# YuanchenBei/ColdRec

Hardware: AMD Instinct MI355X
Metric: ranked items/sec (full-catalogue eval) (higher is better)
Workload: dtype f32; 1 GPU; configs[3] full-catalogue eval: 1000000-row user table x 10000000 items, d=128, k=20, f32 tables, user block 131072 per step, rated CSR (mean ~50) + 20% cold-item bitmap ('warm' setting), item table row-sharded over 1 GPU(s); items=10000000, dim=128, k=20, parallelism=single GPU

## Files before the change

coldrec_amd/_lib.py:

```python
from __future__ import annotations

import ctypes
import os
import subprocess

_HERE = os.path.dirname(os.path.abspath(__file__))
LIB_PATH = os.environ.get("CRH_LIB") or os.path.join(_HERE, "lib", "libcoldrec_hip.so")
CSRC = os.path.join(_HERE, "csrc")

PAD_IDX = 0x7FFFFFFF
MASKED_SCORE = -1.0e9
MAX_K = 128

_lib = None

_vp, _i32, _i64, _sz, _f32 = ctypes.c_void_p, ctypes.c_int, ctypes.c_int64, ctypes.c_size_t, ctypes.c_float
_f64 = ctypes.c_double

SIGNATURES = {
    "crh_last_error": (ctypes.c_char_p, []),
    "crh_version": (_i32, []),
    "crh_score_topk_supports_dim": (_i32, [_i32]),
    "crh_score_topk_workspace_bytes": (_sz, [_i64, _i64, _i32, _i32]),
    "crh_score_topk_min_workspace_bytes": (_sz, [_i64, _i32]),
    "crh_score_topk_route": (_i32, [_i32, _i64, _i64, _i32, _i32, _sz, _i32, _i32, _vp, _vp]),
    "crh_score_topk_route_kernel": (ctypes.c_char_p, [_i32]),
    "crh_score_topk_screened": (_i32, [_i32, _i64, _i64, _i32, _i32, _sz, _i32, _i32]),
    "crh_score_topk_uncertified": (_i64, [_vp, _vp]),
    "crh_score_topk_screen_plan": (_i32, [_i64, _i64, _sz, _i32, _vp, _vp]),
    "crh_score_topk_screen_ordered": (_i32, [_i64, _i64, _sz, _i32]),
    "crh_score_topk_screen_map": (_i32, [_vp, _vp, _i64, _i64, _i64, _i32, _vp, _vp, _vp, _vp]),
    "crh_score_topk_f32": (_i32, [_vp, _vp, _i64, _vp, _i64, _i32, _vp, _vp, _vp, _i32, _i64, _vp, _vp,
                                  _vp, _sz, _vp]),
    "crh_score_topk_f32_ex": (_i32, [_vp, _vp, _i64, _vp, _i64, _i32, _vp, _vp, _vp, _i32, _i64, _vp, _vp,
                                     _vp, _sz, _vp, _i32, _vp, _vp]),
    "crh_score_screen_items_bytes": (_sz, [_i64, _i32]),
    "crh_score_screen_items_prepare": (_i32, [_vp, _i64, _i32, _vp, _i64, _i64, _vp, _sz, _vp, _sz, _vp, _vp]),
    "crh_score_screen_items_destroy": (_i32, [_vp]),
    "crh_score_topk_screen_item_preps": (_i64, []),
    "crh_score_topk_f32_prepared": (_i32, [_vp, _vp, _i64, _vp, _i64, _i32, _vp, _vp, _vp, _i32, _i64, _vp, _vp,
                                           _vp, _sz, _vp, _i32, _vp, _vp, _vp]),
    "crh_score_topk_f16_supports_dim": (_i32, [_i32]),
    "crh_score_topk_f16_workspace_bytes": (_sz, [_i64, _i64, _i32, _i32]),
    "crh_score_topk_f16_ex": (_i32, [_vp, _vp, _i64, _vp, _i64, _i32, _vp, _vp, _vp, _i32, _i64, _vp, _vp,
                                     _vp, _sz, _vp, _i32, _vp, _vp]),
    "crh_mask_topk_f32": (_i32, [_vp, _i64, _i64, _i64, _vp, _vp, _vp, _i32, _i64, _i32, _vp, _vp, _vp]),
    "crh_merge_topk": (_i32, [_vp, _vp, _i32, _i64, _i32, _i32, _vp, _vp, _vp]),
    "crh_bpr_workspace_bytes": (_sz, [_i64]),
    "crh_bpr_plan_ints": (_i64, [_i64]),
    "crh_bpr_heavy_threshold": (_i32, []),
    "crh_bpr_plan_build_host": (_i32, [_vp, _vp, _vp, _i64, _i64, _vp]),
    "crh_bpr_plan_build": (_i32, [_vp, _vp, _vp, _i64, _i64, _vp, _vp]),
    "crh_bpr_plan_build_large_workspace_bytes": (_sz, [_i64, _i64]),
    "crh_bpr_plan_build_large": (_i32, [_vp, _vp, _vp, _i64, _i64, _vp, _vp, _sz, _vp]),
    "crh_bpr_fwd_bwd_f32": (_i32, [_vp, _vp, _vp, _i32, _vp, _vp, _vp, _i64, _f32, _vp, _vp, _vp, _vp, _vp, _vp,
                                   _sz, _vp]),
    "crh_bpr_fwd_f32": (_i32, [_vp, _vp, _vp, _i32, _vp, _vp, _vp, _i64, _vp, _vp, _sz, _vp]),
    "crh_bpr_bwd_f32": (_i32, [_vp, _vp, _vp, _i32, _vp, _vp, _vp, _i64, _i64, _f32, _vp, _vp, _vp, _vp, _vp, _vp,
                               _vp, _sz, _vp]),
    "crh_bpr_bwd_owned_f32": (_i32, [_vp, _vp, _i32, _vp, _vp, _vp, _i64, _f32, _vp, _vp, _vp, _vp, _vp, _i32, _i32, _vp, _sz, _vp]),
    "crh_rows_pack_cap": (_i64, [_i64, _i32]),
    "crh_rows_pack_f32": (_i32, [_vp, _vp, _i64, _i64, _i32, _i32, _i32, _vp, _vp, _vp]),
    "crh_rows_unpack_f32": (_i32, [_vp, _vp, _vp, _i64, _i32, _vp]),
    "crh_adam_dense_f32": (_i32, [_vp, _vp, _vp, _vp, _i64, _vp, _vp, _vp, _vp, _i64, _f64, _f64, _f64, _f64,
                                  _i64, _i32, _vp, _vp]),
    "crh_adam_rows_f32": (_i32, [_vp, _vp, _vp, _vp, _vp, _i64, _i32, _vp, _i64, _i64, _i64, _vp, _f64, _f64, _f64,
                                 _i32, _vp]),
    "crh_adam_step_scalars_host": (None, [_f64, _f64, _f64, _i64, _vp]),
    "crh_adam_step_scalars_range_host": (None, [_f64, _f64, _f64, _i64, _i64, _vp]),
    "crh_spmm_segment_edges": (_i32, []),
    "crh_spmm_lane_group": (_i32, [_i64, _i32, _i64]),
    "crh_spmm_workspace_bytes": (_sz, [_vp, _i32]),
    "crh_spmm_csr_adam_f32": (_i32, [_vp, _vp, _vp, _i64, _vp, _i32, _vp, _f32, _vp, _f32, _vp, _vp, _vp, _vp,
                                     _f64, _f64, _f64, _f64, _i64, _vp, _i32, _vp]),
    "crh_spmm_csr_f32": (_i32, [_vp, _vp, _vp, _i64, _vp, _i32, _vp, _vp, _f32, _vp, _f32, _vp, _vp, _sz, _vp]),
    "crh_bpr_fwd_parts": (_i32, [_i64, _i32]),
    "crh_mf_step_parts": (_i32, [_i64, _i32]),
    "crh_mf_step_tables": (_i32, [_vp, _vp, _vp, _vp, _i64, _i64, _i64, _i64, _vp, _vp, _vp, _vp]),
    "crh_mf_step_f32": (_i32, [_vp, _vp, _vp, _vp, _i64, _i64, _i32, _i64, _f32, _vp, _vp, _vp, _vp,
                               _vp, _i32, _vp, _vp, _i64, _vp, _f64, _f64, _f64, _vp, _vp]),
    "crh_mf_step_finish": (_i32, [_vp, _i32, _i64, _vp, _vp]),
    "crh_mf_step_sgd_f32": (_i32, [_vp, _vp, _i64, _i64, _i32, _i64, _f32, _vp, _vp, _vp, _vp, _vp, _i32, _vp, _vp,
                                   _i64, _vp, _f64, _vp]),
    "crh_sgd_dense_f32": (_i32, [_vp, _vp, _i64, _f64, _i32, _vp]),
    "crh_sgd_rows_f32": (_i32, [_vp, _vp, _i32, _vp, _i64, _i64, _f64, _vp]),
    "crh_spmm_csr_sgd_f32": (_i32, [_vp, _vp, _vp, _i64, _vp, _i32, _vp, _f32, _vp, _f32, _vp, _vp, _f64, _i32, _vp]),
    "crh_l2_workspace_bytes": (_sz, []),
    "crh_l2_norm_f32": (_i32, [_vp, _i64, _vp, _vp, _sz, _vp]),
    "crh_l2_reg_bwd_f32": (_i32, [_vp, _i64, _i64, _f32, _vp, _vp, _vp, _i32, _vp]),
    "crh_infonce_workspace_bytes": (_sz, [_i64, _i32]),
    "crh_infonce_splits": (_i32, [_i64]),
    "crh_infonce_f32": (_i32, [_vp, _vp, _vp, _vp, _vp, _i64, _i32, _f32, _i32, _f32, _i32, _vp, _vp, _vp, _vp, _sz, _vp]),
    "crh_table_nce_workspace_bytes": (_sz, [_i64, _i64, _i32]),
    "crh_table_nce_splits": (_i32, [_i64, _i64, _i32]),
    "crh_table_nce_f32": (_i32, [_vp, _vp, _i64, _vp, _vp, _i64, _i32, _f32, _f32, _i32, _vp, _vp, _vp, _vp, _sz, _vp]),
    "crh_clcrec_max_neg": (_i32, []),
    "crh_clcrec_chunk_rows": (_i32, []),
    "crh_clcrec_workspace_bytes": (_sz, [_i64, _i32, _i32, _i64]),
    "crh_clcrec_f32": (_i32, [_vp] * 12 + [_i64] + [_vp] * 3 + [_i64, _i64, _i32, _i32, _i64, _f32, _f32, _f32, _f32,
                              _vp, _vp, _vp, _vp, _vp, _sz, _vp]),
    "crh_ccfcrec_max_rows": (_i32, []),
    "crh_ccfcrec_chunk_rows": (_i32, []),
    "crh_ccfcrec_workspace_bytes": (_sz, [_i64, _i32, _i32, _i32, _i32, _i64, _i64]),
    "crh_ccfcrec_f32": (_i32, [_vp, _i64, _vp, _i64] + [_vp] * 4 + [_i32] * 4 + [_vp] * 5 + [_i64, _i64] + [_vp] * 5 +
                               [_i64, _i64, _i64, _i32, _i32, _i32, _i32, _f32, _f32, _f32, _vp, _vp, _vp, _vp, _vp, _sz,
                                _vp]),
    "crh_aldi_workspace_bytes": (_sz, [_i64, _i32]),
    "crh_aldi_f32": (_i32, [_vp, _i64, _vp, _i64, _vp, _vp, _vp] + [_i32] * 4 + [_vp] * 4 + [_i64, _i32] + [_f32] * 4 +
                            [_vp] * 5 + [_sz, _vp]),
    "crh_gar_chunk_rows": (_i32, []),
    "crh_gar_workspace_bytes": (_sz, [_i64, _i32, _i64, _i64]),
    "crh_gar_f32": (_i32, [_vp, _i64, _vp, _i64] + [_vp] * 4 + [_i32] * 4 + [_vp] * 5 + [_i64, _i64] + [_vp] * 5 +
                           [_i64, _i64, _i64, _i32, _i32] + [_f32] * 4 + [_vp] * 5 + [_sz, _vp]),
    "crh_mtpr_chunk_rows": (_i32, []),
# ... 91 lines not shown
```

coldrec_amd/csrc/score_screen.hip:

```cpp
#include <math.h>

#include "score_topk_common.h"

#include <hipcub/device/device_radix_sort.hpp>

namespace crh_score {
namespace {

constexpr int SD = 128;
constexpr int FB_SCRATCH_SLICES = 64;

__device__ __forceinline__ float up_float(double x) {
    if (!(x <= 3.0e38)) return __builtin_inff();
    float f = (float)x;
    if ((double)f < x) f = __uint_as_float(__float_as_uint(f) + 1u);
    return f;
}

__device__ __forceinline__ int scale_exp(const unsigned* stats, int word) {
    const float m = __uint_as_float(stats[word]);
    if (!(m > 0.0f) || !(m <= 3.4e38f)) return 0;
    int E;
    frexpf(m, &E);
    return 15 - E;
// ... 73 lines not shown
    const double B = (double)un * R + (double)udn * Nh + gd * (double)un * N + gp * (double)uhn * Nh + 0x1p-126;
    return B * (1.0 + 0x1p-20);
}

__device__ __forceinline__ float up_norm(double s) { return up_float(sqrt(s) * (1.0 + 0x1p-30)); }

constexpr int LIVE_WPB = 256;

__device__ __forceinline__ unsigned live_word(const uint32_t* __restrict__ bitmap, int64_t w, int64_t g0, int64_t g1) {
    const int64_t w0 = g0 >> 5, n_words = ((g1 - 1) >> 5) - w0 + 1;
    if (w >= n_words) return 0u;
    unsigned m = ~bitmap[w0 + w];
    const int64_t lo = (w0 + w) << 5;
    if (lo < g0) m &= ~0u << (int)(g0 - lo);
    if (lo + 32 > g1) m &= ~0u >> (int)(lo + 32 - g1);
    return m;
}

__device__ __forceinline__ unsigned block_excl_sum(unsigned v, unsigned* total) {
    __shared__ unsigned wsum[4];
    const int lane = threadIdx.x & 63, wv = threadIdx.x >> 6;
    unsigned inc = v;
#pragma unroll
    for (int o = 1; o < 64; o <<= 1) {
        const unsigned t = __shfl_up(inc, o);
        if (lane >= o) inc += t;
    }
    if (lane == 63) wsum[wv] = inc;
    __syncthreads();
    unsigned before = 0;
    for (int q = 0; q < wv; ++q) before += wsum[q];
    *total = wsum[0] + wsum[1] + wsum[2] + wsum[3];
    return before + inc - v;
}

__global__ __launch_bounds__(256) void screen_live_count_kernel(const uint32_t* __restrict__ bitmap, int64_t g0, int64_t g1,
                                                                unsigned* __restrict__ blocksum) {
    const unsigned c = __popc(live_word(bitmap, (int64_t)blockIdx.x * LIVE_WPB + threadIdx.x, g0, g1));
    unsigned total;
    block_excl_sum(c, &total);
    if (threadIdx.x == 0) blocksum[blockIdx.x] = total;
}

__global__ __launch_bounds__(256) void screen_live_scan_kernel(unsigned* __restrict__ blocksum, int64_t n_blocks,
                                                               unsigned* __restrict__ n_live) {
    const int64_t per = (n_blocks + 255) / 256;
    const int64_t lo = threadIdx.x * per < n_blocks ? threadIdx.x * per : n_blocks, hi = lo + per < n_blocks ? lo + per : n_blocks;
    unsigned sum = 0;
    for (int64_t q = lo; q < hi; ++q) sum += blocksum[q];
    unsigned total;
    unsigned run = block_excl_sum(sum, &total);
    for (int64_t q = lo; q < hi; ++q) {
        const unsigned c = blocksum[q];
        blocksum[q] = run;
        run += c;
    }
    if (threadIdx.x == 0) *n_live = total;
}

__global__ __launch_bounds__(256) void screen_idmap_kernel(const uint32_t* __restrict__ bitmap, int64_t g0, int64_t g1,
                                                           const unsigned* __restrict__ blocksum, int32_t* __restrict__ idmap) {
    const int64_t w = (int64_t)blockIdx.x * LIVE_WPB + threadIdx.x;
    unsigned m = live_word(bitmap, w, g0, g1);
    unsigned total;
    int64_t pos = (int64_t)blocksum[blockIdx.x] + block_excl_sum(__popc(m), &total);
    const int id0 = (int)(((g0 >> 5) + w) << 5);
    while (m) {
        idmap[pos++] = id0 + __builtin_ctz(m);
        m &= m - 1;
    }
}

__global__ __launch_bounds__(256) void screen_sortkey_kernel(const int32_t* __restrict__ idmap, const uint16_t* __restrict__ rowkeys,
                                                             const unsigned* __restrict__ n_live, int64_t item_base, int64_t n_slots,
                                                             uint16_t* __restrict__ skeys) {
    const int64_t q = (int64_t)blockIdx.x * 256 + threadIdx.x;
    if (q >= n_slots) return;
    skeys[q] = q < (int64_t)*n_live ? (uint16_t)~rowkeys[(int64_t)idmap[q] - item_base] : (uint16_t)0xFFFFu;
}

__global__ __launch_bounds__(256) void screen_mapkeys_kernel(const uint16_t* __restrict__ skeys, int64_t n, int32_t* __restrict__ out) {
    const int64_t q = (int64_t)blockIdx.x * 256 + threadIdx.x;
    if (q < n) out[q] = (int32_t)(uint16_t)~skeys[q];
}

__global__ __launch_bounds__(256) void screen_items_kernel(const float* __restrict__ v, int64_t n_items, const uint32_t* __restrict__ bitmap,
                                                           int64_t item_base, _Float16* __restrict__ packed, unsigned* __restrict__ stats,
                                                           int64_t prefix, const int32_t* __restrict__ idmap) {
    const int e = scale_exp(stats, 0);
    const int64_t TP = prefix >> 5, n_live = idmap ? (int64_t)stats[SCREEN_STAT_LIVE] : 0;
    const int64_t T = idmap ? TP + ((n_live + 31) >> 5) : (n_items + 31) >> 5;
    float mr = 0.0f, mn = 0.0f, mh = 0.0f;
    u32x4* dst = reinterpret_cast<u32x4*>(packed);
    for (int64_t t = blockIdx.x; t < T; t += gridDim.x) {
        for (int p = 0; p < 2; ++p) {
            const int u = threadIdx.x + 256 * p, r = u >> 4, c = u & 15;
            int64_t row = (t << 5) + r;
            bool masked;
            if (idmap != nullptr && t >= TP) {
                const int64_t q = row - prefix;
                masked = q >= n_live;
                row = (int64_t)idmap[masked ? n_live - 1 : q] - item_base;
            } else {
                if (row >= n_items) row = n_items - 1;
                masked = bitmap != nullptr && ((bitmap[(item_base + row) >> 5] >> ((item_base + row) & 31)) & 1u);
            }
            const float* src = v + row * SD + 8 * c;
            const f32x4 x0 = *reinterpret_cast<const f32x4*>(src), x1 = *reinterpret_cast<const f32x4*>(src + 4);
            _Float16 hv[8];
            double sxx, sdd, shh;
            row_sums(x0, x1, hv, e, sxx, sdd, shh);
            u32x4 o = u32x4{0u, 0u, 0u, 0u};
            if (!masked) {
                o = __builtin_bit_cast(u32x4, f16x8{hv[0], hv[1], hv[2], hv[3], hv[4], hv[5], hv[6], hv[7]});
                mr = fmaxf(mr, up_norm(sdd));
                mn = fmaxf(mn, up_norm(sxx));
                mh = fmaxf(mh, up_norm(shh));
                if (sdd != sdd || sxx != sxx) mr = __builtin_inff();
            }
            dst[(t * 8 + (c >> 1)) * 64 + (c & 1) * 32 + r] = o;
        }
    }
    __shared__ float red[3][4];
    mr = wave_max(mr);
    mn = wave_max(mn);
    mh = wave_max(mh);
    if ((threadIdx.x & 63) == 0) {
        red[0][threadIdx.x >> 6] = mr;
        red[1][threadIdx.x >> 6] = mn;
        red[2][threadIdx.x >> 6] = mh;
    }
    __syncthreads();
    if (threadIdx.x < 3) {
        const float b = fmaxf(fmaxf(red[threadIdx.x][0], red[threadIdx.x][1]), fmaxf(red[threadIdx.x][2], red[threadIdx.x][3]));
        if (b > 0.0f) atomicMax(stats + 2 + threadIdx.x, __float_as_uint(b));
    }
}

__global__ __launch_bounds__(256) void screen_users_kernel(const float* __restrict__ uemb, const int32_t* __restrict__ users,
                                                           int64_t n_users, _Float16* __restrict__ uh, float* __restrict__ ustat,
                                                           unsigned* __restrict__ stats) {
    const int e = scale_exp(stats, 1);
    const float R = __uint_as_float(stats[2]), N = __uint_as_float(stats[3]), Nh = __uint_as_float(stats[4]);
    float mb = 0.0f;
    const int64_t n_units = n_users * 16;
    for (int64_t w = (int64_t)blockIdx.x * 256 + threadIdx.x; w < ((n_units + 255) & ~(int64_t)255); w += (int64_t)gridDim.x * 256) {
        const int64_t j = (w < n_units ? w : n_units - 1) >> 4;
        const int c = (int)(w & 15);
        const int64_t row = users ? (int64_t)users[j] : j;
        const float* src = uemb + row * SD + 8 * c;
        const f32x4 x0 = *reinterpret_cast<const f32x4*>(src), x1 = *reinterpret_cast<const f32x4*>(src + 4);
        _Float16 hv[8];
        double sxx, sdd, shh;
        row_sums(x0, x1, hv, e, sxx, sdd, shh);
        if (w < n_units) {
            reinterpret_cast<u32x4*>(uh)[j * 16 + c] = __builtin_bit_cast(u32x4, f16x8{hv[0], hv[1], hv[2], hv[3], hv[4], hv[5], hv[6], hv[7]});
            if (c == 0) {
                const bool bad = sxx != sxx || sdd != sdd;
                const float un = bad ? __builtin_inff() : up_norm(sxx), uhn = bad ? __builtin_inff() : up_norm(shh);
                const float udn = bad ? __builtin_inff() : up_norm(sdd);
                ustat[3 * j + 0] = un;
                ustat[3 * j + 1] = uhn;
                ustat[3 * j + 2] = udn;
                mb = fmaxf(mb, up_float(screen_bound(un, uhn, udn, R, N, Nh)));
            }
        }
// ... 181 lines not shown
    __shared__ int cnth[4];
    const int lane = threadIdx.x & 63, wv = threadIdx.x >> 6;
    const int K = s.k;
    const int64_t count = s.stats[5];
    const int S = fb_slices(s, count);
    const int last = S <= FB_FANIN ? 0 : 1;
    if (level > last) return;
    const int stride = level == 0 ? 1 : FB_FANIN;
    const int span = stride * FB_FANIN;
    const int G = (S + span - 1) / span;
    float* ls = lsh[wv];
    int* li = lih[wv];
    int* cnt = &cnth[wv];
    for (int64_t w = (int64_t)blockIdx.x * 4 + wv; w < count * G; w += (int64_t)gridDim.x * 4) {
        const int64_t f = w / G;
        const int z0 = (int)(w % G) * span;
        if (lane == 0) *cnt = 0;
        for (int z = z0; z < z0 + span && z < S; z += stride) {
            const int64_t o = (f * S + z) * K;
            const float es = lane < K ? s.part_score[o + lane] : CRH_NEG_INF;
            const int ei = lane < K ? s.part_idx[o + lane] : CRH_PAD_IDX;
            unsigned long long m = __ballot(lane < K && ei != CRH_PAD_IDX);
            while (m) {
                const int L = __builtin_ctzll(m);
                m &= m - 1;
                const float sc = __shfl(es, L);
                const int g = __shfl(ei, L);
                const int n = __builtin_amdgcn_readfirstlane(*cnt);
                if (n >= K && !crh_better(sc, g, ls[K - 1], li[K - 1])) break;
                wave_list_insert(ls, li, cnt, K, sc, g, lane);
            }
        }
        const int n = __builtin_amdgcn_readfirstlane(*cnt);
        if (level == last) {
            const int64_t slot = s.fail_list[f];
            wave_list_store(ls, li, n, K, s.out_score + slot * K, s.out_idx + slot * K, lane);
        } else {
            const int64_t o = (f * S + z0) * K;
            wave_list_store(ls, li, n, K, s.part_score + o, s.part_idx + o, lane);
        }
    }
}

}

int screen_fallback_slices(int64_t n_items) {
    const int64_t s = n_items / 4096;
    return (int)(s < 1 ? 1 : (s > FB_SCRATCH_SLICES ? FB_SCRATCH_SLICES : s));
}

size_t screen_scan_bytes(int64_t n_main) { return (size_t)((n_main + 31) / 32 / LIVE_WPB + 2) * sizeof(unsigned); }

int64_t screen_map_slots(int64_t n_main) { return ((n_main + 31) / 32 + 1) * 32; }

size_t screen_sort_bytes(int64_t n_slots) { return (size_t)n_slots * 8 + ((size_t)1 << 20); }

int launch_screen_map(const uint32_t* bitmap, int64_t item_base, int64_t n_items, int64_t prefix, unsigned* n_live, unsigned* scan,
                      int32_t* idmap, const ScreenOrder* ord, hipStream_t st) {
    const int64_t g0 = item_base + prefix, g1 = item_base + n_items;
    const int64_t n_words = ((g1 - 1) >> 5) - (g0 >> 5) + 1, nb = (n_words + LIVE_WPB - 1) / LIVE_WPB;
    hipLaunchKernelGGL(screen_live_count_kernel, dim3((unsigned)nb), dim3(256), 0, st, bitmap, g0, g1, scan);
    CRH_HIP(hipGetLastError());
    hipLaunchKernelGGL(screen_live_scan_kernel, dim3(1), dim3(256), 0, st, scan, nb, n_live);
    CRH_HIP(hipGetLastError());
    hipLaunchKernelGGL(screen_idmap_kernel, dim3((unsigned)nb), dim3(256), 0, st, bitmap, g0, g1, scan, idmap);
    CRH_HIP(hipGetLastError());
    if (ord == nullptr) return CRH_OK;
    const int64_t n_slots = screen_map_slots(n_items - prefix);
    hipLaunchKernelGGL(screen_sortkey_kernel, dim3((unsigned)((n_slots + 255) / 256)), dim3(256), 0, st, idmap, ord->rowkeys, n_live,
                       item_base, n_slots, ord->skeys_in);
    CRH_HIP(hipGetLastError());
    size_t need = 0;
    CRH_HIP(hipcub::DeviceRadixSort::SortPairs(nullptr, need, ord->skeys_in, ord->skeys_out, idmap, ord->idmap, (int)n_slots, 0, 16, st));
    if (need > ord->sort_tmp_bytes) {
        crh_set_error("screened route: the ordered map's sort asks for %zu bytes of temporary storage, %zu are reserved", need,
                      ord->sort_tmp_bytes);
        return CRH_ERR_WS;
    }
    need = ord->sort_tmp_bytes;
    CRH_HIP(hipcub::DeviceRadixSort::SortPairs(ord->sort_tmp, need, ord->skeys_in, ord->skeys_out, idmap, ord->idmap, (int)n_slots, 0, 16, st));
    return CRH_OK;
}

int launch_screen_prep_items(const ScreenArgs& s, unsigned* stats, _Float16* packed, int64_t prefix, int32_t* idmap, unsigned* scan,
                             const ScreenOrder* ord, hipStream_t st) {
    const int64_t T = (s.n_items + 31) / 32;
    if (ord != nullptr)
        hipLaunchKernelGGL(screen_maxabs_kernel<true>, dim3(2048), dim3(256), 0, st, s.item_emb, nullptr, s.n_items, stats, 0, ord->rowkeys);
    else
        hipLaunchKernelGGL(screen_maxabs_kernel<false>, dim3(2048), dim3(256), 0, st, s.item_emb, nullptr, s.n_items, stats, 0, nullptr);
    CRH_HIP(hipGetLastError());
    if (idmap != nullptr) {
        const int rc = launch_screen_map(s.bitmap, s.item_base, s.n_items, prefix, stats + SCREEN_STAT_LIVE, scan, idmap, ord, st);
        if (rc != CRH_OK) return rc;
        if (ord != nullptr) idmap = ord->idmap;
    }
    hipLaunchKernelGGL(screen_items_kernel, dim3((unsigned)(T < 4096 ? T : 4096)), dim3(256), 0, st, s.item_emb, s.n_items, s.bitmap,
                       s.item_base, packed, stats, prefix, idmap);
    CRH_HIP(hipGetLastError());
    return CRH_OK;
}

int launch_screen_prep_users(const ScreenArgs& s, _Float16* uh, int margin_on, hipStream_t st) {
    hipLaunchKernelGGL(screen_maxabs_kernel<false>, dim3(256), dim3(256), 0, st, s.user_emb, s.users, s.n_users, s.stats, 1, nullptr);
    CRH_HIP(hipGetLastError());
    const int64_t ub = (s.n_users * 16 + 255) / 256;
    hipLaunchKernelGGL(screen_users_kernel, dim3((unsigned)(ub < 2048 ? ub : 2048)), dim3(256), 0, st, s.user_emb, s.users, s.n_users,
                       uh, s.ustat, s.stats);
    CRH_HIP(hipGetLastError());
    hipLaunchKernelGGL(screen_margin_kernel, dim3(1), dim3(1), 0, st, s.stats, margin_on);
    CRH_HIP(hipGetLastError());
    return CRH_OK;
}

int screen_map_only(const uint32_t* bitmap, const float* item_emb, int64_t n_items, int64_t item_base, int64_t prefix, int ordered,
                    int32_t* map_out, int32_t* keys_out, int64_t* count, hipStream_t st) {
    auto al = [](size_t x) { return (x + 255) & ~(size_t)255; };
    const int64_t n_main = n_items - prefix, n_slots = screen_map_slots(n_main);
    const size_t o_scan = 256, o_map = o_scan + al(screen_scan_bytes(n_main)), o_rk = o_map + al((size_t)n_slots * 4),
                 o_k0 = o_rk + al((size_t)n_items * 2), o_k1 = o_k0 + al((size_t)n_slots * 2), o_m1 = o_k1 + al((size_t)n_slots * 2),
                 o_tmp = o_m1 + al((size_t)n_slots * 4), total = o_tmp + screen_sort_bytes(n_slots);
    char* buf = nullptr;
    CRH_HIP(hipMalloc(reinterpret_cast<void**>(&buf), total));
    ScreenOrder ord;
    ord.rowkeys = reinterpret_cast<uint16_t*>(buf + o_rk);
    ord.skeys_in = reinterpret_cast<uint16_t*>(buf + o_k0);
    ord.skeys_out = reinterpret_cast<uint16_t*>(buf + o_k1);
    ord.idmap = reinterpret_cast<int32_t*>(buf + o_m1);
    ord.sort_tmp = buf + o_tmp;
    ord.sort_tmp_bytes = screen_sort_bytes(n_slots);
    unsigned* stats = reinterpret_cast<unsigned*>(buf);
    int32_t* idmap = reinterpret_cast<int32_t*>(buf + o_map);
    int rc = CRH_OK;
    unsigned live = 0;
    hipError_t e = hipMemsetAsync(buf, 0, 256, st);
    if (e == hipSuccess) {
        hipLaunchKernelGGL(screen_maxabs_kernel<true>, dim3(2048), dim3(256), 0, st, item_emb, nullptr, n_items, stats, 0, ord.rowkeys);
        e = hipGetLastError();
    }
    if (e == hipSuccess) rc = launch_screen_map(bitmap, item_base, n_items, prefix, stats + SCREEN_STAT_LIVE, reinterpret_cast<unsigned*>(buf + o_scan), idmap, &ord, st);
    if (e == hipSuccess && rc == CRH_OK) {
        hipLaunchKernelGGL(screen_mapkeys_kernel, dim3((unsigned)((n_main + 255) / 256)), dim3(256), 0, st,
                           ordered ? ord.skeys_out : ord.skeys_in, n_main, keys_out);
        e = hipGetLastError();
    }
    if (e == hipSuccess && rc == CRH_OK)
        e = hipMemcpyAsync(map_out, ordered ? ord.idmap : idmap, (size_t)n_main * 4, hipMemcpyDeviceToDevice, st);
    if (e == hipSuccess && rc == CRH_OK) e = hipMemcpyAsync(&live, stats + SCREEN_STAT_LIVE, 4, hipMemcpyDeviceToHost, st);
    if (e == hipSuccess) e = hipStreamSynchronize(st);
    (void)hipFree(buf);
    CRH_HIP(e);
    if (rc == CRH_OK) *count = (int64_t)live;
    return rc;
}

int launch_screen_certify(const ScreenArgs& s, hipStream_t st) {
    hipLaunchKernelGGL(screen_certify_kernel, dim3((unsigned)((s.n_users + 3) / 4)), dim3(256), 0, st, s);
    CRH_HIP(hipGetLastError());
    hipLaunchKernelGGL(screen_fallback_kernel, dim3((unsigned)(FB_WAVES / 4)), dim3(256), 0, st, s);
    CRH_HIP(hipGetLastError());
    for (int level = 0; level < 2; ++level) {
        hipLaunchKernelGGL(screen_fallback_merge_kernel, dim3(512), dim3(256), 0, st, s, level);
        CRH_HIP(hipGetLastError());
    }
    return CRH_OK;
}

}
```

coldrec_amd/csrc/score_topk.hip:

```cpp
#include <math.h>
#include <stdarg.h>
#include <stdlib.h>

#include <algorithm>
#include <atomic>
#include <vector>

#include "score_topk_common.h"

using namespace crh_score;

namespace {

__device__ __forceinline__ bool pack_row_masked(const uint32_t* bitmap, int64_t gid) {
    return bitmap != nullptr && ((bitmap[gid >> 5] >> (gid & 31)) & 1u);
}

template <int D>
__global__ __launch_bounds__(256) void pack_items_kernel(const float* __restrict__ v, int64_t n_items,
                                                         float* __restrict__ packed, const uint32_t* __restrict__ bitmap,
                                                         int64_t item_base) {
    constexpr int NCH = D / 8;
    __shared__ float tile[32][D + 4];
    const int64_t t = blockIdx.x;
// ... 674 lines not shown
    const int dma_mode = getenv("CRH_SCORE_DMA") ? atoi(getenv("CRH_SCORE_DMA")) : 1;
    const size_t tb_off = lists_bytes(n_users, k) + packed_bytes(n_items, d, esz) + sync_bytes(n_items);
    const bool dma_rows = esz == 2 ? d == 256 : (d == 128 || d == 64);
    const int dma_form = dma_mode == 2 || dma_mode == 3 ? dma_mode : (esz == 4 && d == 128 && n_items < FP32_DMA_FLAG_MAX_ITEMS ? 2 : 3);
    const bool dma_shape = dma_mode && dma_rows && score_dma_ring_slots(esz, d, k, dma_form) > 0 &&
                           (!has_bitmap || workspace_bytes >= tb_off + tbits_bytes(n_items));
    const bool wg_shape = esz == 2 ? (d == 64 || d == 128 || d == 256) : ((d == 128 && wg_waves == 8) || (d == 64 && dma_shape));
    const int64_t n_wg64 = ((n_users + 63) / 64 + wg_waves - 1) / wg_waves;
    const int64_t fp32_min_items = !dma_shape ? FP32_WG_MIN_ITEMS : (d == 64 ? FP32_DMA_MIN_ITEMS_D64 : FP32_DMA_MIN_ITEMS_D128);
    const bool fp32_wg_ok = n_items >= fp32_min_items && (double)n_wg64 / (double)(((n_wg64 + 255) / 256) * 256) >= 0.9;
    const bool use_wg = wg_mode && can_pack && wg_shape && (dma_shape || wg_waves == 8 || 2 * wg4_lds <= 160 * 1024) &&
                        (n_users + 63) / 64 >= 512 && (esz == 2 || fp32_wg_ok || wg_mode == 2);
    const bool use_dma = use_wg && dma_shape;
    const int wg_waves_l = use_dma ? 4 : wg_waves;
    const int wg_slots_l = use_dma ? 256 : wg_slots;
    const int upw = use_dma ? 128 : (use_wg ? wg_upw : users_per_wave(esz, d));
    static const int variant = CRH_TUNE_ENV("CRH_SCORE_OCC") ? atoi(CRH_TUNE_ENV("CRH_SCORE_OCC")) : 2;
    const int occ = esz == 2 ? 2 : ((variant == 2 && d == 128) ? 2 : 1);
    static const int dense_mode = CRH_TUNE_ENV("CRH_SCORE_DENSE") ? atoi(CRH_TUNE_ENV("CRH_SCORE_DENSE")) : 1;
    const size_t dense_b = dense_block_bytes(n_users, n_items);
    r.dense = dense_mode && n_splits == 0 && !seeded && dense_b && has_workspace && workspace_bytes >= dense_b;
    r.use_wg = use_wg;
    r.use_dma = use_dma;
    r.dma_mode = dma_form;
    r.can_pack = can_pack;
    r.wg_waves_l = wg_waves_l;
    r.wg_slots_l = wg_slots_l;
    r.upw = upw;
    r.occ = occ;
    r.dense_b = dense_b;
    r.tb_off = tb_off;
    r.no_pack = no_pack;
    return r;
}

int plan_splits(const RoutePlan& r, int esz, int64_t n_users, int64_t n_items, int k, int n_splits, bool seeded) {
    const int64_t T = (n_items + 31) / 32;
    const int64_t n_ug = (n_users + r.upw - 1) / r.upw;
    int s = n_splits > 0 ? n_splits
            : seeded     ? pick_splits_seeded(r.use_wg ? (n_ug + r.wg_waves_l - 1) / r.wg_waves_l : n_ug, n_items,
                                              r.use_wg ? (double)r.wg_slots_l : 1024.0 * r.occ)
            : r.use_wg   ? pick_splits_wg((n_ug + r.wg_waves_l - 1) / r.wg_waves_l, n_items, k, r.wg_slots_l,
                                          esz == 2 ? 18750.0 : 5700.0)
                         : pick_splits(n_ug, n_items, r.occ);
    if (s > T) s = (int)T;
    return s;
}

int score_topk_impl(int esz, const void* user_emb, const int32_t* users, int64_t n_users, const void* item_emb,
                    int64_t n_items, int d, const int64_t* rated_rowptr, const int32_t* rated_col,
                    const uint32_t* cand_bitmap, int k, int64_t item_base, float* out_score, int32_t* out_idx,
                    void* workspace, size_t workspace_bytes, void* stream, int n_splits, void* ev_kernel_start,
                    void* ev_kernel_stop, const char* who, const float* seed_score, const int32_t* seed_idx);

int64_t seed_route(int esz, int64_t n_users, int64_t n_items, int d) {
    const char* sm = getenv("CRH_SCORE_SEED");
    const int seed_mode = sm ? atoi(sm) : 1;
    int64_t P = seed_prefix_items(n_items, n_users);
    if (!seed_mode || P <= 0 || n_users <= 0) return 0;
    const int upw = users_per_wave(esz, d);
    const int64_t n_ug = (n_users + upw - 1) / upw;
    const int occ_pw = esz == 2 || d == 128 ? 2 : 1;
    const bool cuts = pick_splits(n_ug, n_items, occ_pw) > 1;
    const char* smi = getenv("CRH_SCORE_SEED_MAX_ITEMS");
    const int64_t f32_stream_min = d == 64 ? FP32_DMA_MIN_ITEMS_D64 : FP32_WG_MIN_ITEMS;
    const bool small_cat = !cuts && esz == 4 && n_items <= (smi ? atoll(smi) : f32_stream_min - 1);
    const bool f16_stream = !cuts && esz == 2 && d == 256 && n_users >= 32768 && n_items >= ((int64_t)1 << 20);
    const bool f32_stream = !cuts && esz == 4 && (d == 128 || d == 64) && n_users >= 32768 && n_items >= f32_stream_min;
    if ((small_cat || f16_stream) && !CRH_TUNE_ENV("CRH_SCORE_SEED_ITEMS") && P > 4096) P = 4096;
    if (f32_stream && !small_cat && !CRH_TUNE_ENV("CRH_SCORE_SEED_ITEMS") && P > 8192) P = 8192;
    if (!(cuts || small_cat || f16_stream || f32_stream || seed_mode == 2) || dense_block_bytes(n_users, P) == 0) return 0;
    return P;
}

constexpr int64_t SCREEN_SEED_ITEMS = 8192;
int64_t screen_prefix(int64_t n_items) { return n_items >= 8 * SCREEN_SEED_ITEMS ? SCREEN_SEED_ITEMS : 0; }
int screen_splits(int64_t n_users, int64_t n_main, bool seeded) {
    const int64_t n_wg = ((n_users + 127) / 128 + 3) / 4, T = (n_main + 31) / 32;
    int s = seeded ? pick_splits_seeded(n_wg, n_main, 256.0) : pick_splits_wg(n_wg, n_main, SCREEN_KP, 256, 18750.0);
    if (s > T) s = (int)T;
    return s;
}
struct ScreenLayout {
    size_t stats, ustat, fail, uh, seed, cand, packed, tbits, sync, idmap, scan, rowkeys, skeys, idmap2, sorttmp, scratch, need;
};
ScreenLayout screen_layout(int64_t n_users, int64_t n_items, int64_t P, bool compact = false, bool ordered = false) {
    auto al = [](size_t x) { return (x + 255) & ~(size_t)255; };
    ScreenLayout L;
    L.stats = 0;
    L.ustat = 256;
    L.fail = L.ustat + al((size_t)n_users * 3 * sizeof(float));
    L.uh = L.fail + al((size_t)n_users * sizeof(int32_t));
    L.seed = L.uh + al((size_t)n_users * 128 * 2);
    L.cand = L.seed + al((size_t)n_users * SCREEN_KP * 8);
    L.packed = L.cand + al((size_t)n_users * SCREEN_KP * 8);
    L.tbits = L.packed + packed_bytes(n_items, 128, 2);
    L.sync = L.tbits + tbits_bytes(n_items);
    L.idmap = L.sync + sync_bytes(n_items);
    const size_t slots = (size_t)screen_map_slots(n_items - P);
    L.scan = L.idmap + (compact ? al(slots * sizeof(int32_t)) : 0);
    L.rowkeys = L.scan + (compact ? al(screen_scan_bytes(n_items - P)) : 0);
    ordered = ordered && compact;
    L.skeys = L.rowkeys + (ordered ? al((size_t)n_items * sizeof(uint16_t)) : 0);
    L.idmap2 = L.skeys + (ordered ? 2 * al(slots * sizeof(uint16_t)) : 0);
    L.sorttmp = L.idmap2 + (ordered ? al(slots * sizeof(int32_t)) : 0);
    L.scratch = L.sorttmp + (ordered ? al(screen_sort_bytes((int64_t)slots)) : 0);
    const int S = screen_splits(n_users, n_items - P, P > 0);
    const size_t lists = S > 1 ? (size_t)S * n_users * SCREEN_KP * 8 : 0;
    const size_t dense = P > 0 ? (size_t)64 * (size_t)P * sizeof(float) : 0;
    const size_t part = (size_t)n_users * screen_fallback_slices(n_items) * 20 * 8;
    L.need = L.scratch + std::max(lists, std::max(dense, part));
    return L;
}

int screen_mode() {
    const char* e = getenv("CRH_SCORE_SCREEN");
    return e ? atoi(e) : 1;
}
bool screen_compact(int64_t n_users, int64_t n_items, size_t workspace_bytes, bool has_bitmap) {
    const char* e = getenv("CRH_SCORE_SCREEN_COMPACT");
    if (!has_bitmap || (e && atoi(e) == 0)) return false;
    return workspace_bytes >= screen_layout(n_users, n_items, screen_prefix(n_items), true).need;
}
bool screen_ordered(int64_t n_users, int64_t n_items, size_t workspace_bytes, bool has_bitmap) {
    const char* e = getenv("CRH_SCORE_SCREEN_ORDER");
    if ((e && atoi(e) == 0) || !screen_compact(n_users, n_items, workspace_bytes, has_bitmap)) return false;
    const int64_t P = screen_prefix(n_items);
    if (screen_splits(n_users, n_items - P, P > 0) != 1) return false;
    return workspace_bytes >= screen_layout(n_users, n_items, P, true, true).need;
}
bool screen_route(int esz, int64_t n_users, int64_t n_items, int d, int k, size_t workspace_bytes, bool has_bitmap, int n_splits) {
    const int mode = screen_mode();
    if (mode <= 0 || mode > 3 || esz != 4 || d != 128 || k < 1 || k > 20 || n_splits != 0 || n_users <= 0 || n_items <= 0 ||
        workspace_bytes == 0)
        return false;
    if (workspace_bytes < screen_layout(n_users, n_items, screen_prefix(n_items)).need) return false;
    if (mode >= 2) return true;
    if (n_items < FP32_DMA_FLAG_MAX_ITEMS) return false;
    int64_t P = seed_route(esz, n_users, n_items, d);
    size_t ws = workspace_bytes;
    if (P > 0) {
        const size_t sb = seed_bytes(n_users, k);
        const size_t stage1 = dense_block_bytes(n_users, P) + packed_bytes(P, d, esz);
        const size_t stage2 = lists_bytes(n_users, k) + packed_bytes(n_items - P, d, esz);
        if (workspace_bytes >= sb + std::max(stage1, stage2)) ws = workspace_bytes - sb;
        else P = 0;
    }
    const RoutePlan r = plan_route(esz, n_users, n_items - P, d, k, true, ws, has_bitmap, 0, P > 0);
    return !r.dense && r.use_dma && r.dma_mode == 3;
}

constexpr uint32_t SCREEN_ITEMS_MAGIC = 0x43524849u;
struct ScreenItems {
    uint32_t magic;
    const float* item_emb;
    int64_t n_items, item_base, prefix;
    int d;
    const uint32_t* bitmap;
    bool compact, ordered;
    hipStream_t stream;
    char* buf;
};
struct ScreenItemsLayout {
    size_t stats, packed, tbits, map, need;
};
ScreenItemsLayout screen_items_layout(int64_t n_items, bool has_bitmap) {
    ScreenItemsLayout L;
    L.stats = 0;
    L.packed = 256;
    L.tbits = L.packed + packed_bytes(n_items, 128, 2);
    L.map = L.tbits + (has_bitmap ? tbits_bytes(n_items) : 0);
    const size_t slots = (size_t)screen_map_slots(n_items);
    L.need = L.map + (has_bitmap ? (slots * sizeof(int32_t) + 255) & ~(size_t)255 : 0);
    return L;
}
bool screen_items_match(const ScreenItems* p, const float* item_emb, int64_t n_items, int64_t item_base, const uint32_t* bitmap,
                        int64_t prefix, bool compact, bool ordered, hipStream_t st) {
    if (p == nullptr || p->magic != SCREEN_ITEMS_MAGIC) return false;
    const char* e = getenv("CRH_SCORE_SCREEN_PREPARED");
    if (e && atoi(e) == 0) return false;
    return p->item_emb == item_emb && p->n_items == n_items && p->d == 128 && p->item_base == item_base && p->bitmap == bitmap &&
           p->prefix == prefix && p->compact == compact && p->ordered == ordered && p->stream == st;
}
std::atomic<int64_t> screen_item_preps{0};

int score_topk_screened(const float* user_emb, const int32_t* users, int64_t n_users, const float* item_emb, int64_t n_items,
                        const int64_t* rated_rowptr, const int32_t* rated_col, const uint32_t* cand_bitmap, int k, int64_t item_base,
                        float* out_score, int32_t* out_idx, void* workspace, size_t workspace_bytes, void* stream,
                        void* ev_kernel_start, void* ev_kernel_stop, const char* who, const ScreenItems* prepared);

int score_topk_any(int esz, const void* user_emb, const int32_t* users, int64_t n_users, const void* item_emb,
                   int64_t n_items, int d, const int64_t* rated_rowptr, const int32_t* rated_col,
                   const uint32_t* cand_bitmap, int k, int64_t item_base, float* out_score, int32_t* out_idx,
                   void* workspace, size_t workspace_bytes, void* stream, int n_splits, void* ev_kernel_start,
                   void* ev_kernel_stop, const char* who, const ScreenItems* prepared = nullptr) {
    if (user_emb && item_emb && out_score && out_idx && workspace &&
        screen_route(esz, n_users, n_items, d, k, workspace_bytes, cand_bitmap != nullptr, n_splits))
        return score_topk_screened(reinterpret_cast<const float*>(user_emb), users, n_users, reinterpret_cast<const float*>(item_emb),
                                   n_items, rated_rowptr, rated_col, cand_bitmap, k, item_base, out_score, out_idx, workspace,
                                   workspace_bytes, stream, ev_kernel_start, ev_kernel_stop, who, prepared);
    const int64_t P = n_splits == 0 ? seed_route(esz, n_users, n_items, d) : 0;
    if (P > 0 && user_emb && item_emb && out_score && out_idx && n_users > 0 && k >= 1 && k <= CRH_MAX_K && workspace) {
        const size_t sb = seed_bytes(n_users, k);
        const size_t stage1 = dense_block_bytes(n_users, P) + packed_bytes(P, d, esz);
        const size_t stage2 = lists_bytes(n_users, k) + packed_bytes(n_items - P, d, esz);
        if (workspace_bytes >= sb + std::max(stage1, stage2)) {
            float* seed_s = reinterpret_cast<float*>(workspace);
            int32_t* seed_i = reinterpret_cast<int32_t*>(seed_s + (size_t)n_users * k);
            void* ws2 = reinterpret_cast<char*>(workspace) + sb;
            hipStream_t st = reinterpret_cast<hipStream_t>(stream);
            if (ev_kernel_start) CRH_HIP(hipEventRecord(reinterpret_cast<hipEvent_t>(ev_kernel_start), st));
            int rc = score_topk_impl(esz, user_emb, users, n_users, item_emb, P, d, rated_rowptr, rated_col, cand_bitmap, k,
                                     item_base, seed_s, seed_i, ws2, workspace_bytes - sb, stream, 0, nullptr, nullptr, who,
                                     nullptr, nullptr);
            if (rc != CRH_OK) return rc;
            rc = score_topk_impl(esz, user_emb, users, n_users,
                                 reinterpret_cast<const char*>(item_emb) + (size_t)P * d * esz, n_items - P, d, rated_rowptr,
                                 rated_col, cand_bitmap, k, item_base + P, out_score, out_idx, ws2, workspace_bytes - sb, stream,
                                 0, nullptr, nullptr, who, seed_s, seed_i);
            if (rc != CRH_OK) return rc;
            if (ev_kernel_stop) CRH_HIP(hipEventRecord(reinterpret_cast<hipEvent_t>(ev_kernel_stop), st));
            return CRH_OK;
        }
    }
    return score_topk_impl(esz, user_emb, users, n_users, item_emb, n_items, d, rated_rowptr, rated_col, cand_bitmap, k,
                           item_base, out_score, out_idx, workspace, workspace_bytes, stream, n_splits, ev_kernel_start,
                           ev_kernel_stop, who, nullptr, nullptr);
}

#ifdef CRH_PROFILE
int print_wave_timing(unsigned long long* dev, int64_t n_waves, int timing, hipStream_t st) {
        CRH_HIP(hipStreamSynchronize(st));
        std::vector<unsigned long long> h((size_t)n_waves * 6);
        CRH_HIP(hipMemcpy(h.data(), dev, h.size() * 8, hipMemcpyDeviceToHost));
        CRH_HIP(hipFree(dev));
        if (timing == 2)
            if (FILE* f = fopen("/tmp/crh_wave_clock.bin", "wb")) { fwrite(h.data(), 8, h.size(), f); fclose(f); }
        unsigned long long t0 = ~0ull, t1 = 0;
        for (int64_t wv = 0; wv < n_waves; ++wv) { t0 = std::min(t0, h[2 * wv]); t1 = std::max(t1, h[2 * wv + 1]); }
        std::vector<double> st_(n_waves), en_(n_waves);
        for (int64_t wv = 0; wv < n_waves; ++wv) { st_[wv] = (double)(h[2 * wv] - t0); en_[wv] = (double)(h[2 * wv + 1] - t0); }
        std::sort(st_.begin(), st_.end());
        std::sort(en_.begin(), en_.end());
        const double tot = (double)(t1 - t0);
        fprintf(stderr, "[crh timing] waves=%lld span=%.0f ticks; start quantiles 0/25/50/75/100%%: %.3f %.3f %.3f %.3f %.3f; "
                        "end quantiles 0/10/25/50/75/90/100%%: %.3f %.3f %.3f %.3f %.3f %.3f %.3f (fraction of span)\n",
                (long long)n_waves, tot, st_[0] / tot, st_[n_waves / 4] / tot, st_[n_waves / 2] / tot,
                st_[3 * n_waves / 4] / tot, st_[n_waves - 1] / tot, en_[0] / tot, en_[n_waves / 10] / tot,
                en_[n_waves / 4] / tot, en_[n_waves / 2] / tot, en_[3 * n_waves / 4] / tot, en_[9 * n_waves / 10] / tot,
                en_[n_waves - 1] / tot);
        std::vector<double> in_(n_waves), lp_(n_waves), so_(n_waves);
        double ev_ticks = 0, ev = 0, lp_sum = 0;
        for (int64_t wv = 0; wv < n_waves; ++wv) {
            in_[wv] = (double)(h[2 * n_waves + 2 * wv] - h[2 * wv]);
            lp_[wv] = (double)(h[2 * n_waves + 2 * wv + 1] - h[2 * n_waves + 2 * wv]);
            so_[wv] = (double)(h[2 * wv + 1] - h[2 * n_waves + 2 * wv + 1]);
            ev_ticks += (double)h[4 * n_waves + 2 * wv];
            ev += (double)h[4 * n_waves + 2 * wv + 1];
            lp_sum += lp_[wv];
        }
        std::sort(in_.begin(), in_.end());
        std::sort(lp_.begin(), lp_.end());
        std::sort(so_.begin(), so_.end());
        fprintf(stderr, "[crh timing] median ticks: list setup %.0f, tile loop %.0f, list store %.0f; %.0f slow-path events per wave, "
                        "%.0f ticks each = %.3f of the loop\n",
                in_[n_waves / 2], lp_[n_waves / 2], so_[n_waves / 2], ev / (double)n_waves, ev > 0 ? ev_ticks / ev : 0.0,
                lp_sum > 0 ? ev_ticks / lp_sum : 0.0);
    return CRH_OK;
}
int dma_timing_begin(ScoreArgs& a, hipStream_t st) {
    CRH_HIP(hipMalloc(&a.wave_clock, (size_t)16 * 4 * 66 * 8));
    CRH_HIP(hipMemsetAsync(a.wave_clock, 0, (size_t)16 * 4 * 66 * 8, st));
    return CRH_OK;
}
int dma_timing_report(ScoreArgs& a, int esz, int d, hipStream_t st) {
    CRH_HIP(hipStreamSynchronize(st));
    std::vector<unsigned long long> h((size_t)16 * 4 * 66);
    CRH_HIP(hipMemcpy(h.data(), a.wave_clock, h.size() * 8, hipMemcpyDeviceToHost));
    CRH_HIP(hipFree(a.wave_clock));
    {
        unsigned long long tk = 0, ne = 0;
        for (int q = 0; q < 64; ++q) { tk += h[(size_t)16 * 4 * 64 + 2 * q]; ne += h[(size_t)16 * 4 * 64 + 2 * q + 1]; }
        fprintf(stderr, "[crh dma timing] events: %.0f per wave, %.0f cycles each (tiles with at least one candidate; 64 waves)\n",
                (double)ne / 64.0, ne ? (double)tk / (double)ne : 0.0);
    }
    for (int wv = 0; wv < 4; ++wv) {
        unsigned long long tot = 0, wsum = 0;
        std::vector<unsigned long long> b(64, 0);
        for (int blk = 0; blk < 16; ++blk)
            for (int q = 0; q < 64; ++q) b[q] += h[((size_t)blk * 4 + wv) * 64 + q];
        const unsigned long long bw = (esz == 4 ? 512 : 128) >> (d * esz == 256 ? 1 : 0);
        for (int q = 0; q < 64; ++q) { tot += b[q]; wsum += b[q] * (q * bw + bw / 2); }
        fprintf(stderr, "[crh dma timing] wave %d: %llu tiles, mean %.0f cycles; histogram (%llu-cycle buckets from 0):", wv, tot,
                tot ? (double)wsum / (double)tot : 0.0, bw);
        for (int q = 0; q < 64; ++q) fprintf(stderr, " %llu", b[q]);
        fprintf(stderr, "\n");
    }
    a.wave_clock = nullptr;
    return CRH_OK;
}
#endif

int score_topk_impl(int esz, const void* user_emb, const int32_t* users, int64_t n_users, const void* item_emb,
                    int64_t n_items, int d, const int64_t* rated_rowptr, const int32_t* rated_col,
                    const uint32_t* cand_bitmap, int k, int64_t item_base, float* out_score, int32_t* out_idx,
                    void* workspace, size_t workspace_bytes, void* stream, int n_splits, void* ev_kernel_start,
                    void* ev_kernel_stop, const char* who, const float* seed_score, const int32_t* seed_idx) {
    CRH_CHECK_ARG(user_emb && item_emb && out_score && out_idx, "%s: NULL table/output pointer", who);
    CRH_CHECK_ARG(n_users > 0 && n_items > 0, "%s: empty block (n_users=%lld, n_items=%lld)", who,
                  (long long)n_users, (long long)n_items);
    CRH_CHECK_ARG(k >= 1 && k <= CRH_MAX_K, "%s: k=%d outside 1..%d", who, k, CRH_MAX_K);
    CRH_CHECK_ARG(esz == 4 ? crh_score_topk_supports_dim(d) : crh_score_topk_f16_supports_dim(d),
                  "%s: d=%d unsupported (pad the tables to %s16/32/64/128/256)", who, d, esz == 4 ? "8/" : "");
    CRH_CHECK_ARG(((uintptr_t)user_emb & 15) == 0 && ((uintptr_t)item_emb & 15) == 0,
                  "%s: tables must be 16-byte aligned", who);
    CRH_CHECK_ARG((rated_rowptr == nullptr) == (rated_col == nullptr) || rated_rowptr != nullptr,
                  "%s: rated_col given without rated_rowptr", who);
    CRH_CHECK_ARG(item_base >= 0 && item_base + n_items < (int64_t)CRH_PAD_IDX, "%s: item ids exceed int32", who);
    CRH_CHECK_ARG(n_splits >= 0 && n_splits <= 64, "%s: n_splits=%d outside 0..64", who, n_splits);

    const RoutePlan rp = plan_route(esz, n_users, n_items, d, k, workspace != nullptr, workspace_bytes, cand_bitmap != nullptr,
                                    n_splits, seed_score != nullptr);
    const bool use_wg = rp.use_wg, use_dma = rp.use_dma, can_pack = rp.can_pack;
    const int wg_waves_l = rp.wg_waves_l, upw = rp.upw, occ = rp.occ, no_pack = rp.no_pack;
    const size_t tb_off = rp.tb_off, dense_b = rp.dense_b;
    ScoreArgs a;
    a.user_emb = user_emb;
    a.users = users;
    a.n_users = n_users;
    a.item_emb = item_emb;
    a.n_items = n_items;
    a.rated_rowptr = rated_rowptr;
    a.rated_col = rated_col;
    a.bitmap = cand_bitmap;
    a.k = k;
    a.item_base = item_base;
    a.n_ugroups = (n_users + upw - 1) / upw;
    static const int ablate = CRH_PROFILE_ENV("CRH_SCORE_ABLATE");
    a.ablate = ablate;
    a.dense = nullptr;
    a.dense_stride = 0;
    a.user_base = 0;
    a.seed_score = seed_score;
    a.seed_idx = seed_idx;
    a.margin = nullptr;
    a.screen_k = 0;
    const int64_t T = (n_items + 31) / 32;
    hipStream_t st = reinterpret_cast<hipStream_t>(stream);

    if (rp.dense) {
        const int64_t stride = T * 32;
        const int upw_pw = users_per_wave(esz, d);
        int64_t chunk = (int64_t)(dense_b / ((size_t)stride * sizeof(float)));
        if (chunk > n_users) chunk = n_users;
        a.packed = nullptr;
        if (!no_pack && workspace_bytes >= dense_b + packed_bytes(n_items, d, esz)) {
            void* pk = reinterpret_cast<char*>(workspace) + dense_b;
            const int prc = pack_items(esz, item_emb, n_items, d, pk, st, cand_bitmap, item_base);
            if (prc != CRH_OK) return prc;
            a.packed = pk;
        }
        a.n_splits = 1;
        a.xcd_sync = nullptr;
        a.sync_window = 0;
        a.sync_stride = 0;
        a.wave_clock = nullptr;
#ifdef CRH_PROFILE
        static const int timing_d = CRH_PROFILE_ENV("CRH_SCORE_TIMING");
#endif
        a.out_score = out_score;
        a.out_idx = out_idx;
        a.dense = reinterpret_cast<float*>(workspace);
        CRH_CHECK_ARG(stride < ((int64_t)1 << 25), "%s: dense block rows of %lld scores exceed the kernel's 32-bit lane offsets", who, (long long)stride);
        a.dense_stride = stride;
        if (ev_kernel_start) CRH_HIP(hipEventRecord(reinterpret_cast<hipEvent_t>(ev_kernel_start), st));
        for (int64_t u0 = 0; u0 < n_users; u0 += chunk) {
            const int64_t cu = std::min(chunk, n_users - u0);
            a.users = users ? users + u0 : nullptr;
            a.user_base = u0;
            a.n_users = cu;
            a.n_ugroups = (cu + upw_pw - 1) / upw_pw;
            a.n_splits = (int)std::max<int64_t>(1, std::min<int64_t>(T, (1024 * occ) / a.n_ugroups));
            a.rated_rowptr = rated_rowptr ? rated_rowptr + u0 : nullptr;
#ifdef CRH_PROFILE
            if (timing_d) {
                CRH_HIP(hipMalloc(&a.wave_clock, (size_t)a.n_ugroups * a.n_splits * 48));
                CRH_HIP(hipMemsetAsync(a.wave_clock, 0, (size_t)a.n_ugroups * a.n_splits * 48, st));
            }
#endif
            const int rc1 = launch_score_per_wave(esz, d, occ, a, st);
            if (rc1 != CRH_OK) return rc1;
#ifdef CRH_PROFILE
            if (timing_d) {
                const int trc = print_wave_timing(a.wave_clock, a.n_ugroups * a.n_splits, timing_d, st);
                if (trc != CRH_OK) return trc;
            }
#endif
            const int rc2 = crh_mask_topk_f32(a.dense, cu, n_items, stride, a.rated_rowptr, rated_col, cand_bitmap, k,
                                              item_base, 0, out_score + u0 * k, out_idx + u0 * k, stream);
            if (rc2 != CRH_OK) return rc2;
        }
        if (ev_kernel_stop) CRH_HIP(hipEventRecord(reinterpret_cast<hipEvent_t>(ev_kernel_stop), st));
        return CRH_OK;
    }

    a.n_splits = plan_splits(rp, esz, n_users, n_items, k, n_splits, seed_score != nullptr);

    if (a.n_splits == 1) {
        a.out_score = out_score;
        a.out_idx = out_idx;
    } else {
        const size_t need = (size_t)a.n_splits * n_users * k * 8;
        if (!workspace || workspace_bytes < need) {
            crh_set_error("%s: workspace %zu < %zu bytes", who, workspace_bytes, need);
            return CRH_ERR_WS;
        }
        a.out_score = reinterpret_cast<float*>(workspace);
        a.out_idx = reinterpret_cast<int32_t*>(a.out_score + (size_t)a.n_splits * n_users * k);
    }
    a.packed = nullptr;
    if (can_pack) {
        void* pk = reinterpret_cast<char*>(workspace) + lists_bytes(n_users, k);
        const int prc = pack_items(esz, item_emb, n_items, d, pk, st, cand_bitmap, item_base);
        if (prc != CRH_OK) return prc;
        a.packed = pk;
    }
    int rc;
    static const int sync_win_raw = CRH_TUNE_ENV("CRH_SCORE_SYNC_WINDOW") ? atoi(CRH_TUNE_ENV("CRH_SCORE_SYNC_WINDOW")) : 128;
    static const int sync_win = sync_win_raw <= 0 ? 0 : std::max(2, sync_win_raw & ~1);
// ... 8 lines not shown
        const int64_t n_win = (T / a.n_splits + 1 + sync_win - 1) / sync_win + 1;
        const size_t need = lists_bytes(n_users, k) + packed_bytes(n_items, d, esz) + sync_bytes(n_items);
        if (workspace_bytes >= need && (size_t)(n_win + 1) * 8 * sizeof(unsigned) <= sync_bytes(n_items)) {
            a.sync_stride = n_win + 1;
            a.xcd_sync = reinterpret_cast<unsigned*>(reinterpret_cast<char*>(workspace) + lists_bytes(n_users, k) +
                                                     packed_bytes(n_items, d, esz));
            CRH_HIP(hipMemsetAsync(a.xcd_sync, 0, (size_t)a.sync_stride * 8 * sizeof(unsigned), st));
        }
    }
    a.tile_bits = reinterpret_cast<const uint32_t*>(a.packed);
    a.idmap = nullptr;
    a.n_live = nullptr;
    if (use_dma && cand_bitmap) {
        uint32_t* tb = reinterpret_cast<uint32_t*>(reinterpret_cast<char*>(workspace) + tb_off);
        hipLaunchKernelGGL(tile_bits_kernel, dim3((unsigned)((T + 255) / 256)), dim3(256), 0, st, cand_bitmap, item_base, n_items, T, tb);
        CRH_HIP(hipGetLastError());
        a.tile_bits = tb;
    }
    a.wave_clock = nullptr;
#ifdef CRH_PROFILE
    static const int timing = CRH_PROFILE_ENV("CRH_SCORE_TIMING");
    const int64_t n_waves = a.n_ugroups * a.n_splits;
    if (timing && !use_wg) CRH_HIP(hipMalloc(&a.wave_clock, (size_t)n_waves * 48));
    if (timing && use_dma) {
        rc = dma_timing_begin(a, st);
        if (rc != CRH_OK) return rc;
    }
#endif
    if (ev_kernel_start) CRH_HIP(hipEventRecord(reinterpret_cast<hipEvent_t>(ev_kernel_start), st));
    if (use_dma) {
        rc = launch_score_dma(esz, d, rp.dma_mode, a, st);
    } else if (esz == 4 && use_wg) {
        rc = launch_score_wg<float, 128, 2, 8>(a, st);
    } else if (use_wg) {
        switch (d) {
            case 64: rc = wg_waves_l == 4 ? launch_score_wg<_Float16, 64, 2, 4>(a, st) : launch_score_wg<_Float16, 64, 2, 8>(a, st); break;
            case 128: rc = wg_waves_l == 4 ? launch_score_wg<_Float16, 128, 2, 4>(a, st) : launch_score_wg<_Float16, 128, 2, 8>(a, st); break;
            default: rc = wg_waves_l == 4 ? launch_score_wg<_Float16, 256, 2, 4>(a, st) : launch_score_wg<_Float16, 256, 2, 8>(a, st); break;
        }
    } else {
        rc = launch_score_per_wave(esz, d, occ, a, st);
    }
    if (rc != CRH_OK) return rc;
    if (ev_kernel_stop) CRH_HIP(hipEventRecord(reinterpret_cast<hipEvent_t>(ev_kernel_stop), st));
#ifdef CRH_PROFILE
    if (timing && use_dma) {
        rc = dma_timing_report(a, esz, d, st);
        if (rc != CRH_OK) return rc;
    }
    if (timing && !use_wg) {
        const int trc = print_wave_timing(a.wave_clock, n_waves, timing, st);
        if (trc != CRH_OK) return trc;
    }
#endif
    if (a.n_splits > 1)
        return crh_merge_topk(a.out_score, a.out_idx, a.n_splits, n_users, k, k, out_score, out_idx, stream);
    return CRH_OK;
}

int screen_items_build(const ScreenArgs& s, unsigned* stats, _Float16* pk, int64_t P, int32_t* idmap, unsigned* scan,
                       const ScreenOrder* ord, uint32_t* tbits, hipStream_t st) {
    screen_item_preps.fetch_add(1, std::memory_order_relaxed);
    const int rc = launch_screen_prep_items(s, stats, pk, P, idmap, scan, ord, st);
    if (rc != CRH_OK) return rc;
    if (tbits != nullptr) {
        const int64_t n_main = s.n_items - P, T = (n_main + 31) / 32;
        hipLaunchKernelGGL(tile_bits_kernel, dim3((unsigned)((T + 255) / 256)), dim3(256), 0, st, s.bitmap, s.item_base + P, n_main, T, tbits);
        CRH_HIP(hipGetLastError());
    }
    return CRH_OK;
}

int score_topk_screened(const float* user_emb, const int32_t* users, int64_t n_users, const float* item_emb, int64_t n_items,
                        const int64_t* rated_rowptr, const int32_t* rated_col, const uint32_t* cand_bitmap, int k, int64_t item_base,
                        float* out_score, int32_t* out_idx, void* workspace, size_t workspace_bytes, void* stream,
                        void* ev_kernel_start, void* ev_kernel_stop, const char* who, const ScreenItems* prepared) {
    CRH_CHECK_ARG(((uintptr_t)user_emb & 15) == 0 && ((uintptr_t)item_emb & 15) == 0, "%s: tables must be 16-byte aligned", who);
    CRH_CHECK_ARG(rated_rowptr != nullptr || rated_col == nullptr, "%s: rated_col given without rated_rowptr", who);
    CRH_CHECK_ARG(item_base >= 0 && item_base + n_items < (int64_t)CRH_PAD_IDX, "%s: item ids exceed int32", who);
    constexpr int KP = SCREEN_KP, D = 128;
    const int64_t P = screen_prefix(n_items);
    const bool compact = screen_compact(n_users, n_items, workspace_bytes, cand_bitmap != nullptr);
    const bool ordered = screen_ordered(n_users, n_items, workspace_bytes, cand_bitmap != nullptr);
    const ScreenLayout L = screen_layout(n_users, n_items, P, compact, ordered);
    CRH_CHECK_ARG(workspace_bytes >= L.need, "%s: workspace %zu < %zu bytes (screened route)", who, workspace_bytes, L.need);
    int32_t* idmap = compact ? reinterpret_cast<int32_t*>(reinterpret_cast<char*>(workspace) + L.idmap) : nullptr;
    hipStream_t st = reinterpret_cast<hipStream_t>(stream);
    char* ws = reinterpret_cast<char*>(workspace);
    ScreenOrder ord;
    if (ordered) {
        const size_t slots = (size_t)screen_map_slots(n_items - P);
        ord.rowkeys = reinterpret_cast<uint16_t*>(ws + L.rowkeys);
        ord.skeys_in = reinterpret_cast<uint16_t*>(ws + L.skeys);
        ord.skeys_out = reinterpret_cast<uint16_t*>(ws + L.skeys + (L.idmap2 - L.skeys) / 2);
        ord.idmap = reinterpret_cast<int32_t*>(ws + L.idmap2);
        ord.sort_tmp = ws + L.sorttmp;
        ord.sort_tmp_bytes = screen_sort_bytes((int64_t)slots);
    }
    const bool reuse = screen_items_match(prepared, item_emb, n_items, item_base, cand_bitmap, P, compact, ordered, st);
    const ScreenItemsLayout PL = screen_items_layout(n_items, cand_bitmap != nullptr);
    _Float16* pk = reinterpret_cast<_Float16*>(reuse ? prepared->buf + PL.packed : ws + L.packed);
    uint32_t* tbits = cand_bitmap && !compact ? reinterpret_cast<uint32_t*>(reuse ? prepared->buf + PL.tbits : ws + L.tbits) : nullptr;
    const int32_t* stream_map = nullptr;
    if (compact) stream_map = reuse ? reinterpret_cast<const int32_t*>(prepared->buf + PL.map) : (ordered ? ord.idmap : idmap);
    _Float16* uh = reinterpret_cast<_Float16*>(ws + L.uh);
    float* seed_s = reinterpret_cast<float*>(ws + L.seed);
    int32_t* seed_i = reinterpret_cast<int32_t*>(seed_s + (size_t)n_users * KP);
    float* cand_s = reinterpret_cast<float*>(ws + L.cand);
    int32_t* cand_i = reinterpret_cast<int32_t*>(cand_s + (size_t)n_users * KP);
    char* scratch = ws + L.scratch;
    const size_t scratch_b = workspace_bytes - L.scratch;

    ScreenArgs s;
    s.user_emb = user_emb;
    s.users = users;
    s.n_users = n_users;
    s.item_emb = item_emb;
    s.n_items = n_items;
    s.item_base = item_base;
    s.rated_rowptr = rated_rowptr;
    s.rated_col = rated_col;
    s.bitmap = cand_bitmap;
    s.k = k;
    s.kp = KP;
    s.mode = screen_mode();
    s.cand_score = cand_s;
    s.cand_idx = cand_i;
    s.stats = reinterpret_cast<unsigned*>(ws + L.stats);
    s.ustat = reinterpret_cast<float*>(ws + L.ustat);
    s.fail_list = reinterpret_cast<int32_t*>(ws + L.fail);
    s.n_slices = screen_fallback_slices(n_items);
    s.part_score = reinterpret_cast<float*>(scratch);
    s.part_idx = reinterpret_cast<int32_t*>(s.part_score + (size_t)n_users * s.n_slices * k);
    s.out_score = out_score;
    s.out_idx = out_idx;

    int rc = CRH_OK;
    if (reuse) {
        CRH_HIP(hipMemcpyAsync(s.stats, prepared->buf + PL.stats, 256, hipMemcpyDeviceToDevice, st));
    } else {
        CRH_HIP(hipMemsetAsync(s.stats, 0, 256, st));
        rc = screen_items_build(s, s.stats, pk, P, idmap, reinterpret_cast<unsigned*>(ws + L.scan), ordered ? &ord : nullptr, tbits, st);
        if (rc != CRH_OK) return rc;
    }
    const char* margin_env = getenv("CRH_SCORE_SCREEN_MARGIN");
    rc = launch_screen_prep_users(s, uh, !(margin_env && atoi(margin_env) == 0), st);
    if (rc != CRH_OK) return rc;
    if (ev_kernel_start) CRH_HIP(hipEventRecord(reinterpret_cast<hipEvent_t>(ev_kernel_start), st));

    ScoreArgs a;
    a.user_emb = uh;
    a.users = nullptr;
    a.n_users = n_users;
    a.item_emb = nullptr;
    a.rated_rowptr = rated_rowptr;
    a.rated_col = rated_col;
    a.bitmap = cand_bitmap;
    a.k = KP;
    a.ablate = 0;
    a.wave_clock = nullptr;
    a.xcd_sync = nullptr;
    a.sync_window = 0;
    a.sync_stride = 0;
    a.dense = nullptr;
    a.dense_stride = 0;
    a.user_base = 0;
    a.seed_score = nullptr;
    a.seed_idx = nullptr;
    a.tile_bits = reinterpret_cast<const uint32_t*>(pk);
    a.idmap = nullptr;
    a.n_live = nullptr;
    a.margin = nullptr;
    a.screen_k = 0;
    if (P > 0) {
        const int64_t stride = P;
        const int upw_pw = users_per_wave(2, D);
        int64_t chunk = (int64_t)(scratch_b / ((size_t)stride * sizeof(float))) & ~(int64_t)63;
        if (chunk > n_users) chunk = n_users;
        a.packed = pk;
        a.n_items = P;
        a.item_base = item_base;
        a.dense = reinterpret_cast<float*>(scratch);
        a.dense_stride = stride;
        for (int64_t u0 = 0; u0 < n_users; u0 += chunk) {
            const int64_t cu = std::min(chunk, n_users - u0);
            a.user_base = u0;
            a.n_users = cu;
            a.n_ugroups = (cu + upw_pw - 1) / upw_pw;
            a.n_splits = (int)std::max<int64_t>(1, std::min<int64_t>(P / 32, 2048 / a.n_ugroups));
            a.rated_rowptr = rated_rowptr ? rated_rowptr + u0 : nullptr;
            rc = launch_score_per_wave(2, D, 2, a, st);
            if (rc != CRH_OK) return rc;
            rc = crh_mask_topk_f32(a.dense, cu, P, stride, a.rated_rowptr, rated_col, cand_bitmap, KP, item_base, 0,
                                   seed_s + u0 * KP, seed_i + u0 * KP, stream);
            if (rc != CRH_OK) return rc;
        }
        a.dense = nullptr;
        a.dense_stride = 0;
        a.user_base = 0;
        a.n_users = n_users;
        a.rated_rowptr = rated_rowptr;
        a.seed_score = seed_s;
        a.seed_idx = seed_i;
    }
    const int64_t n_main = n_items - P, T = (n_main + 31) / 32;
    a.packed = reinterpret_cast<const char*>(pk) + (size_t)(P / 32) * 32 * D * 2;
    a.n_items = n_main;
    a.item_base = item_base + P;
    a.n_ugroups = (n_users + 127) / 128;
    const int64_t n_wg = (a.n_ugroups + 3) / 4;
    a.n_splits = screen_splits(n_users, n_main, P > 0);
    a.margin = reinterpret_cast<const float*>(s.stats + SCREEN_STAT_MARGIN);
    a.screen_k = k;
    if (a.n_splits == 1) {
        a.out_score = cand_s;
        a.out_idx = cand_i;
    } else {
        a.out_score = reinterpret_cast<float*>(scratch);
        a.out_idx = reinterpret_cast<int32_t*>(a.out_score + (size_t)a.n_splits * n_users * KP);
    }
    static const int sync_win_raw = CRH_TUNE_ENV("CRH_SCORE_SYNC_WINDOW") ? atoi(CRH_TUNE_ENV("CRH_SCORE_SYNC_WINDOW")) : 128;
    static const int sync_win = sync_win_raw <= 0 ? 0 : std::max(2, sync_win_raw & ~1);
    if (sync_win > 0 && a.n_splits == 1 && n_wg <= 256 && n_wg > 8) {
        const int64_t n_win = (T + 1 + sync_win - 1) / sync_win + 1;
        if ((size_t)(n_win + 1) * 8 * sizeof(unsigned) <= sync_bytes(n_items)) {
            a.sync_window = sync_win;
            a.sync_stride = n_win + 1;
            a.xcd_sync = reinterpret_cast<unsigned*>(ws + L.sync);
            CRH_HIP(hipMemsetAsync(a.xcd_sync, 0, (size_t)a.sync_stride * 8 * sizeof(unsigned), st));
        }
    }
    if (compact) {
        a.idmap = stream_map;
        a.n_live = s.stats + SCREEN_STAT_LIVE;
    } else if (cand_bitmap) {
        a.tile_bits = tbits;
    }
#ifdef CRH_PROFILE
    static const int timing = CRH_PROFILE_ENV("CRH_SCORE_TIMING");
    if (timing) {
        rc = dma_timing_begin(a, st);
        if (rc != CRH_OK) return rc;
    }
#endif
    rc = launch_score_dma(2, D, 3, a, st);
    if (rc != CRH_OK) return rc;
#ifdef CRH_PROFILE
    if (timing) {
        rc = dma_timing_report(a, 2, D, st);
        if (rc != CRH_OK) return rc;
    }
#endif
    if (a.n_splits > 1) {
        rc = crh_merge_topk(a.out_score, a.out_idx, a.n_splits, n_users, KP, KP, cand_s, cand_i, stream);
        if (rc != CRH_OK) return rc;
    }

    rc = launch_screen_certify(s, st);
    if (rc != CRH_OK) return rc;
    if (ev_kernel_stop) CRH_HIP(hipEventRecord(reinterpret_cast<hipEvent_t>(ev_kernel_stop), st));
    return CRH_OK;
}
}

namespace {
size_t full_workspace_bytes(int64_t n_users, int64_t n_items, int d, int k, int esz, bool dim_ok) {
    if (n_users <= 0 || k <= 0) return 0;
    const size_t tail = dim_ok && n_items > 0 ? packed_bytes(n_items, d, esz) + sync_bytes(n_items) + tbits_bytes(n_items) : 0;
    size_t need = std::max(lists_bytes(n_users, k), dense_block_bytes(n_users, n_items)) + tail;
    const int64_t P = dim_ok ? seed_route(esz, n_users, n_items, d) : 0;
    if (P > 0)
        need = std::max(need, std::max(dense_block_bytes(n_users, P) + packed_bytes(P, d, esz), lists_bytes(n_users, k) + tail)) +
               seed_bytes(n_users, k);
    return need;
}
}

extern "C" size_t crh_score_topk_workspace_bytes(int64_t n_users, int64_t n_items, int d, int k) {
    return full_workspace_bytes(n_users, n_items, d, k, 4, crh_score_topk_supports_dim(d) != 0);
}

extern "C" size_t crh_score_topk_f16_workspace_bytes(int64_t n_users, int64_t n_items, int d, int k) {
    return full_workspace_bytes(n_users, n_items, d, k, 2, crh_score_topk_f16_supports_dim(d) != 0);
}

extern "C" size_t crh_score_topk_min_workspace_bytes(int64_t n_users, int k) {
    if (n_users <= 0 || k <= 0) return 0;
    return lists_bytes(n_users, k);
}

extern "C" int crh_score_topk_route(int elem_bytes, int64_t n_users, int64_t n_items, int d, int k, size_t workspace_bytes,
                                    int has_bitmap, int n_splits, int64_t* prefix_items, int* picked_splits) {
    CRH_CHECK_ARG(elem_bytes == 4 || elem_bytes == 2, "crh_score_topk_route: elem_bytes=%d (4 = fp32 tables, 2 = fp16)", elem_bytes);
    CRH_CHECK_ARG(n_users > 0 && n_items > 0 && k >= 1 && k <= CRH_MAX_K, "crh_score_topk_route: empty block or k outside 1..%d",
                  CRH_MAX_K);
    CRH_CHECK_ARG(elem_bytes == 4 ? crh_score_topk_supports_dim(d) : crh_score_topk_f16_supports_dim(d),
                  "crh_score_topk_route: d=%d unsupported", d);
    CRH_CHECK_ARG(n_splits >= 0 && n_splits <= 64, "crh_score_topk_route: n_splits=%d outside 0..64", n_splits);
    const bool has_ws = workspace_bytes > 0;
    int64_t P = n_splits == 0 && has_ws ? seed_route(elem_bytes, n_users, n_items, d) : 0;
    size_t ws = workspace_bytes;
    if (P > 0) {
        const size_t sb = seed_bytes(n_users, k);
        const size_t stage1 = dense_block_bytes(n_users, P) + packed_bytes(P, d, elem_bytes);
        const size_t stage2 = lists_bytes(n_users, k) + packed_bytes(n_items - P, d, elem_bytes);
        if (workspace_bytes >= sb + std::max(stage1, stage2)) ws = workspace_bytes - sb;
        else P = 0;
    }
    const int64_t n_main = n_items - P;
    const RoutePlan r = plan_route(elem_bytes, n_users, n_main, d, k, has_ws, ws, has_bitmap != 0, n_splits, P > 0);
    int route = r.dense ? CRH_ROUTE_DENSE : (r.use_dma ? CRH_ROUTE_FUSED_DMA : (r.use_wg ? CRH_ROUTE_FUSED_WG : CRH_ROUTE_FUSED_WAVE));
    if (P > 0) route |= CRH_ROUTE_SEEDED;
    if (r.use_dma && !r.dense && r.dma_mode == 2) route |= CRH_ROUTE_DMA_FLAGS;
    if (prefix_items) *prefix_items = P;
    if (picked_splits) *picked_splits = r.dense ? 1 : plan_splits(r, elem_bytes, n_users, n_main, k, n_splits, P > 0);
    return route;
}

extern "C" int crh_score_topk_screened(int elem_bytes, int64_t n_users, int64_t n_items, int d, int k, size_t workspace_bytes,
                                       int has_bitmap, int n_splits) {
    return screen_route(elem_bytes, n_users, n_items, d, k, workspace_bytes, has_bitmap != 0, n_splits) ? 1 : 0;
}

extern "C" int crh_score_topk_screen_plan(int64_t n_users, int64_t n_items, size_t workspace_bytes, int has_bitmap, int* cuts,
                                          int* compact) {
    CRH_CHECK_ARG(n_users > 0 && n_items > 0, "crh_score_topk_screen_plan: empty block");
    const int64_t P = screen_prefix(n_items);
    if (cuts) *cuts = screen_splits(n_users, n_items - P, P > 0);
    if (compact) *compact = screen_compact(n_users, n_items, workspace_bytes, has_bitmap != 0) ? 1 : 0;
    return CRH_OK;
}

extern "C" int crh_score_topk_screen_ordered(int64_t n_users, int64_t n_items, size_t workspace_bytes, int has_bitmap) {
    if (n_users <= 0 || n_items <= 0) return 0;
    return screen_ordered(n_users, n_items, workspace_bytes, has_bitmap != 0) ? 1 : 0;
}

extern "C" int crh_score_topk_screen_map(const uint32_t* bitmap, const float* item_emb, int64_t n_items, int64_t item_base,
                                         int64_t prefix, int ordered, int32_t* map_out, int32_t* keys_out, int64_t* count,
                                         void* stream) {
    CRH_CHECK_ARG(bitmap && item_emb && map_out && keys_out && count, "crh_score_topk_screen_map: NULL argument");
    CRH_CHECK_ARG(prefix >= 0 && (prefix & 31) == 0 && n_items > prefix, "crh_score_topk_screen_map: prefix %lld of %lld items",
                  (long long)prefix, (long long)n_items);
    CRH_CHECK_ARG(((uintptr_t)item_emb & 15) == 0, "crh_score_topk_screen_map: table must be 16-byte aligned");
    CRH_CHECK_ARG(item_base >= 0 && item_base + n_items < (int64_t)CRH_PAD_IDX, "crh_score_topk_screen_map: item ids exceed int32");
    return screen_map_only(bitmap, item_emb, n_items, item_base, prefix, ordered, map_out, keys_out, count,
                           reinterpret_cast<hipStream_t>(stream));
}

extern "C" size_t crh_score_screen_items_bytes(int64_t n_items, int has_bitmap) {
    if (n_items <= 0) return 0;
    return screen_items_layout(n_items, has_bitmap != 0).need;
}

extern "C" int crh_score_screen_items_prepare(const float* item_emb, int64_t n_items, int d, const uint32_t* cand_bitmap,
                                              int64_t item_base, int64_t n_users, void* items_buf, size_t items_bytes,
                                              void* workspace, size_t workspace_bytes, void* stream, void** handle) {
    const char* who = "crh_score_screen_items_prepare";
    CRH_CHECK_ARG(item_emb && items_buf && workspace && handle, "%s: NULL argument", who);
    CRH_CHECK_ARG(d == 128, "%s: d=%d (the screened route ranks d=128 tables)", who, d);
    CRH_CHECK_ARG(n_users > 0 && n_items > 0, "%s: empty block", who);
    CRH_CHECK_ARG(((uintptr_t)item_emb & 15) == 0 && ((uintptr_t)items_buf & 255) == 0, "%s: table must be 16-byte, buffer 256-byte aligned", who);
    CRH_CHECK_ARG(item_base >= 0 && item_base + n_items < (int64_t)CRH_PAD_IDX, "%s: item ids exceed int32", who);
    const bool has_bitmap = cand_bitmap != nullptr;
    const ScreenItemsLayout PL = screen_items_layout(n_items, has_bitmap);
    CRH_CHECK_ARG(items_bytes >= PL.need, "%s: buffer %zu < %zu bytes", who, items_bytes, PL.need);
    const int64_t P = screen_prefix(n_items);
    const bool compact = screen_compact(n_users, n_items, workspace_bytes, has_bitmap);
    const bool ordered = screen_ordered(n_users, n_items, workspace_bytes, has_bitmap);
    const ScreenLayout L = screen_layout(n_users, n_items, P, compact, ordered);
    CRH_CHECK_ARG(workspace_bytes >= L.need, "%s: workspace %zu < %zu bytes (screened route)", who, workspace_bytes, L.need);
    hipStream_t st = reinterpret_cast<hipStream_t>(stream);
    char* ws = reinterpret_cast<char*>(workspace);
    char* buf = reinterpret_cast<char*>(items_buf);
    int32_t* own_map = reinterpret_cast<int32_t*>(buf + PL.map);
    ScreenOrder ord;
    if (ordered) {
        const size_t slots = (size_t)screen_map_slots(n_items - P);
        ord.rowkeys = reinterpret_cast<uint16_t*>(ws + L.rowkeys);
        ord.skeys_in = reinterpret_cast<uint16_t*>(ws + L.skeys);
        ord.skeys_out = reinterpret_cast<uint16_t*>(ws + L.skeys + (L.idmap2 - L.skeys) / 2);
        ord.idmap = own_map;
        ord.sort_tmp = ws + L.sorttmp;
        ord.sort_tmp_bytes = screen_sort_bytes((int64_t)slots);
    }
    int32_t* idmap = compact ? (ordered ? reinterpret_cast<int32_t*>(ws + L.idmap) : own_map) : nullptr;
    ScreenArgs s = {};
    s.item_emb = item_emb;
    s.n_items = n_items;
    s.item_base = item_base;
    s.bitmap = cand_bitmap;
    unsigned* stats = reinterpret_cast<unsigned*>(buf + PL.stats);
    CRH_HIP(hipMemsetAsync(stats, 0, 256, st));
    const int rc = screen_items_build(s, stats, reinterpret_cast<_Float16*>(buf + PL.packed), P, idmap, reinterpret_cast<unsigned*>(ws + L.scan),
                                      ordered ? &ord : nullptr, has_bitmap && !compact ? reinterpret_cast<uint32_t*>(buf + PL.tbits) : nullptr, st);
    if (rc != CRH_OK) return rc;
    ScreenItems* p = new ScreenItems;
    p->magic = SCREEN_ITEMS_MAGIC;
    p->item_emb = item_emb;
    p->n_items = n_items;
    p->item_base = item_base;
    p->prefix = P;
    p->d = d;
    p->bitmap = cand_bitmap;
    p->compact = compact;
    p->ordered = ordered;
    p->stream = st;
    p->buf = buf;
    *handle = p;
    return CRH_OK;
}

extern "C" int crh_score_screen_items_destroy(void* handle) {
    if (handle == nullptr) return CRH_OK;
    ScreenItems* p = reinterpret_cast<ScreenItems*>(handle);
    CRH_CHECK_ARG(p->magic == SCREEN_ITEMS_MAGIC, "crh_score_screen_items_destroy: not a prepared-items handle");
    p->magic = 0;
    delete p;
// ... 71 lines not shown
```

coldrec_amd/csrc/score_topk_common.h:

```cpp
#pragma once
#include <math.h>

#include "crh_common.h"
#include "topk_list.h"

namespace crh_score {

struct ScoreArgs {
    const void* user_emb;
    const int32_t* users;
    int64_t n_users;
    const void* item_emb;
    const void* packed;
    int64_t n_items;
    const int64_t* rated_rowptr;
    const int32_t* rated_col;
    const uint32_t* bitmap;
    int k;
    int64_t item_base;
    int n_splits;
    int64_t n_ugroups;
    float* out_score;
    int32_t* out_idx;
    int ablate;
    unsigned long long* wave_clock;
    unsigned* xcd_sync;
    int sync_window;
    int64_t sync_stride;
    float* dense;
    int64_t dense_stride;
    int64_t user_base;
    const float* seed_score;
    const int32_t* seed_idx;
    const uint32_t* tile_bits;
    const int32_t* idmap;
    const unsigned* n_live;
    const float* margin;
    int screen_k;
};

__device__ __forceinline__ void chunk_swap(f32x4& cf) {
    u32x4 c = __builtin_bit_cast(u32x4, cf);
    const u32x2 r0 = __builtin_amdgcn_permlane32_swap(c.x, c.y, false, false);
    const u32x2 r1 = __builtin_amdgcn_permlane32_swap(c.z, c.w, false, false);
    u32x4 o;
    o.x = r0[0];
    o.y = r0[1];
    o.z = r1[0];
    o.w = r1[1];
    cf = __builtin_bit_cast(f32x4, o);
}

__device__ __forceinline__ f32x4 load16(const char* p) { return *reinterpret_cast<const f32x4*>(p); }

typedef _Float16 f16x8 __attribute__((ext_vector_type(8)));

template <typename T>
struct Elem;
template <>
struct Elem<float> {
    static constexpr bool kSwap = true;
    template <int UW>
    static __device__ __forceinline__ void mma(f32x16 (&acc)[UW], const f32x4& c, const f32x4 (&b)[UW]) {
#pragma unroll
        for (int u = 0; u < UW; ++u) acc[u] = __builtin_amdgcn_mfma_f32_32x32x2f32(c.x, b[u].x, acc[u], 0, 0, 0);
#pragma unroll
        for (int u = 0; u < UW; ++u) acc[u] = __builtin_amdgcn_mfma_f32_32x32x2f32(c.z, b[u].z, acc[u], 0, 0, 0);
#pragma unroll
        for (int u = 0; u < UW; ++u) acc[u] = __builtin_amdgcn_mfma_f32_32x32x2f32(c.y, b[u].y, acc[u], 0, 0, 0);
#pragma unroll
        for (int u = 0; u < UW; ++u) acc[u] = __builtin_amdgcn_mfma_f32_32x32x2f32(c.w, b[u].w, acc[u], 0, 0, 0);
    }
};
template <>
struct Elem<_Float16> {
    static constexpr bool kSwap = false;
    template <int UW>
    static __device__ __forceinline__ void mma(f32x16 (&acc)[UW], const f32x4& c, const f32x4 (&b)[UW]) {
        const f16x8 ca = __builtin_bit_cast(f16x8, c);
#pragma unroll
        for (int u = 0; u < UW; ++u)
            acc[u] = __builtin_amdgcn_mfma_f32_32x32x16_f16(ca, __builtin_bit_cast(f16x8, b[u]), acc[u], 0, 0, 0);
    }
};

template <int UPW>
struct WaveLds {
    float* ls;
    int* li;
    int* cnt;
    int64_t* rlo;
    int64_t* rhi;
    unsigned* rfilter;
};

template <int UPW>
__host__ __device__ constexpr size_t wave_lds_bytes(int K) {
    return (size_t)UPW * K * 8 + (size_t)UPW * 4 + (size_t)UPW * 16 + (size_t)UPW * 32;
}

template <int UPW>
__device__ __forceinline__ void wave_lds_carve(WaveLds<UPW>& w, char* base, int K) {
    w.ls = reinterpret_cast<float*>(base);
    w.li = reinterpret_cast<int*>(w.ls + UPW * K);
    w.cnt = w.li + UPW * K;
    w.rlo = reinterpret_cast<int64_t*>(w.cnt + UPW);
    w.rhi = w.rlo + UPW;
    w.rfilter = reinterpret_cast<unsigned*>(w.rhi + UPW);
}

__device__ __forceinline__ unsigned rated_hash(int gi) { return ((unsigned)gi * 2654435761u) >> 24; }

template <int UPW>
__device__ __forceinline__ void wave_lds_init(const WaveLds<UPW>& w, const ScoreArgs& a, int64_t slot0, int id0, int id1,
                                              bool filter, int lane) {
    for (int j = lane; j < UPW; j += 64) {
        w.cnt[j] = 0;
        const int64_t slot = slot0 + j;
        const bool has = a.rated_rowptr && slot < a.n_users;
        w.rlo[j] = has ? a.rated_rowptr[slot] : 0;
        w.rhi[j] = has ? a.rated_rowptr[slot + 1] : 0;
    }
// ... 162 lines not shown
                    lsu[p] = sc;
                    liu[p] = gi;
                    w.cnt[ul] = n2;
                }
                if (n2 >= K) {
                    const int q = K >= 2 ? K - 2 : 0;
                    const float prev = __builtin_bit_cast(float, q < 64 ? __builtin_amdgcn_readlane(__builtin_bit_cast(int, es), q)
                                                                        : __builtin_amdgcn_readlane(__builtin_bit_cast(int, es2), q - 64));
                    const float kth = (p == K - 1) ? sc : prev;
                    if ((lane & 31) == jl) tau_reg = kth >= CRH_MASKED_SCORE ? kth : CRH_NEG_INF;
                }
            }
        }
    }
}

__device__ __forceinline__ bool xcd_window_sync(unsigned* cnt, int64_t win, int lane) {
    bool ok = true;
    if (lane == 0) {
        if (win >= 1) __hip_atomic_fetch_add(cnt + 1 + (win - 1), 1u, __ATOMIC_RELAXED, __HIP_MEMORY_SCOPE_AGENT);
        if (win >= 2) {
            int spins = 0;
            while (__hip_atomic_load(cnt + 1 + (win - 2), __ATOMIC_RELAXED, __HIP_MEMORY_SCOPE_AGENT) <
                   __hip_atomic_load(cnt, __ATOMIC_RELAXED, __HIP_MEMORY_SCOPE_AGENT)) {
                __builtin_amdgcn_s_sleep(32);
                if (++spins > 200000) { ok = false; break; }
            }
        }
    }
    return __builtin_amdgcn_readfirstlane((int)ok) != 0;
}

constexpr int WG_RING = 3;

constexpr int SCREEN_KP = 28;
__attribute__((visibility("hidden"))) int launch_score_dma(int esz, int d, int mode, const ScoreArgs& a, hipStream_t stream);
__attribute__((visibility("hidden"))) size_t score_dma_lds_bytes(int row_bytes, int k, int ring_slots, bool flags, bool compact = false);
__attribute__((visibility("hidden"))) int score_dma_ring_slots(int esz, int d, int k, int mode);

struct ScreenArgs {
    const float* user_emb;
    const int32_t* users;
    int64_t n_users;
    const float* item_emb;
    int64_t n_items;
    int64_t item_base;
    const int64_t* rated_rowptr;
    const int32_t* rated_col;
    const uint32_t* bitmap;
    int k;
    int kp;
    int mode;
    const float* cand_score;
    const int32_t* cand_idx;
    unsigned* stats;
    float* ustat;
    int32_t* fail_list;
    float* part_score;
    int32_t* part_idx;
    int n_slices;
    float* out_score;
    int32_t* out_idx;
};
__attribute__((visibility("hidden"))) int screen_fallback_slices(int64_t n_items);
constexpr int SCREEN_STAT_LIVE = 6;
constexpr int SCREEN_STAT_MAXB = 7;
constexpr int SCREEN_STAT_MARGIN = 8;
__attribute__((visibility("hidden"))) size_t screen_scan_bytes(int64_t n_main);
struct ScreenOrder {
    uint16_t* rowkeys;
    uint16_t* skeys_in;
    uint16_t* skeys_out;
    int32_t* idmap;
    void* sort_tmp;
    size_t sort_tmp_bytes;
};
__attribute__((visibility("hidden"))) int64_t screen_map_slots(int64_t n_main);
__attribute__((visibility("hidden"))) size_t screen_sort_bytes(int64_t n_slots);
__attribute__((visibility("hidden"))) int launch_screen_prep_items(const ScreenArgs& s, unsigned* stats, _Float16* packed, int64_t prefix,
                                                                   int32_t* idmap, unsigned* scan, const ScreenOrder* ord, hipStream_t st);
__attribute__((visibility("hidden"))) int launch_screen_prep_users(const ScreenArgs& s, _Float16* uh, int margin_on, hipStream_t st);
__attribute__((visibility("hidden"))) int screen_map_only(const uint32_t* bitmap, const float* item_emb, int64_t n_items,
                                                          int64_t item_base, int64_t prefix, int ordered, int32_t* map_out,
                                                          int32_t* keys_out, int64_t* count, hipStream_t st);
__attribute__((visibility("hidden"))) int launch_screen_certify(const ScreenArgs& s, hipStream_t st);

}
```

coldrec_amd/csrc/score_topk_dma.hip:

```cpp
#include <type_traits>
#include <utility>

#include "score_topk_common.h"

namespace crh_score {
namespace {

constexpr int DMA_NW = 4;
constexpr int DMA_UPW = 128;
constexpr int TBITS_B = 2 * 64 * 4;
constexpr int FLAGS_B = 64;
constexpr int IDS_SLOTS = 8;
constexpr int IDS_B = (IDS_SLOTS + 1) * 32 * 4;

constexpr int DMA_FW = 6;
__host__ __device__ constexpr size_t dma_wave_lds_bytes(int K) {
    return (size_t)DMA_UPW * K * 8 + (size_t)DMA_UPW * 4 + (size_t)DMA_UPW * DMA_FW * 4;
}
__device__ __forceinline__ unsigned rated_hash192(int gi) { return ((((unsigned)gi * 2654435761u) >> 16) * (32u * DMA_FW)) >> 16; }

template <int K>
__device__ __forceinline__ float f4_comp(const f32x4& v) {
    if constexpr (K == 0) return v.x;
    else if constexpr (K == 1) return v.z;
    else if constexpr (K == 2) return v.y;
    else return v.w;
}
template <int UW, int BASE, typename H>
__device__ __forceinline__ void mma_f32_hooked(f32x16 (&acc)[UW], const f32x4& c, const f32x4 (&b)[UW], H&& hook) {
    [&]<int... I>(std::integer_sequence<int, I...>) __attribute__((always_inline)) {
        ((acc[I % UW] = __builtin_amdgcn_mfma_f32_32x32x2f32(f4_comp<I / UW>(c), f4_comp<I / UW>(b[I % UW]), acc[I % UW], 0, 0, 0),
          hook(std::integral_constant<int, BASE + I>{})),
         ...);
    }(std::make_integer_sequence<int, 4 * UW>{});
}

#ifdef CRH_DMA_TWO_TRIP
constexpr bool DMA_ONE_TRIP_F32 = false;
#else
constexpr bool DMA_ONE_TRIP_F32 = true;
#endif
template <bool MG>
__device__ __forceinline__ float dma_new_tau(float tail, float es, float sc, int kc, float m) {
    float t = tail >= CRH_MASKED_SCORE ? tail : CRH_NEG_INF;
    if constexpr (MG) {
        const float e1 = __builtin_bit_cast(float, __builtin_amdgcn_readlane(__builtin_bit_cast(int, es), kc - 1));
        const float e2 = __builtin_bit_cast(float, __builtin_amdgcn_readlane(__builtin_bit_cast(int, es), kc - 2));
        const float lk = __builtin_amdgcn_fmed3f(sc, e1, e2);
        t = __builtin_amdgcn_fmed3f(t, tail > CRH_MASKED_SCORE ? lk - m : CRH_NEG_INF, __builtin_inff());
    }
    return t;
}

template <bool ONE_TRIP, bool LANE_READ = false, bool MG = false>
__device__ __forceinline__ void dma_candidate(float sc, int gi, bool bm_masked, int ul, int64_t slot, float* ls, int* li, int* cnt, int K,
                                              const ScoreArgs& a, int lane, const unsigned* rfilter, bool mine, float& tau_reg,
                                              float margin = 0.0f) {
    float* lsu = ls + ul * K;
    int* liu = li + ul * K;
    const unsigned hsh = rated_hash192(gi);
    const int n_raw = cnt[ul];
    const int le = ONE_TRIP ? (LANE_READ ? lane : (lane < K ? lane : K - 1)) : K - 1;
    const float ks_raw = lsu[le];
    const int ki_raw = liu[le];
    const unsigned fw_raw = a.rated_rowptr ? rfilter[ul * DMA_FW + (hsh >> 5)] : 0u;
    const int n = __builtin_amdgcn_readfirstlane(n_raw);
    if (n >= K) {
        const float ks = ONE_TRIP ? __builtin_bit_cast(float, __builtin_amdgcn_readlane(__builtin_bit_cast(int, ks_raw), K - 1))
                                  : __builtin_bit_cast(float, __builtin_amdgcn_readfirstlane(__builtin_bit_cast(int, ks_raw)));
        const int ki = ONE_TRIP ? __builtin_amdgcn_readlane(ki_raw, K - 1) : __builtin_amdgcn_readfirstlane(ki_raw);
        if (!crh_better(fmaxf(sc, CRH_MASKED_SCORE), gi, ks, ki)) return;
    }
    bool masked = bm_masked;
    if (!masked && ((__builtin_amdgcn_readfirstlane(fw_raw) >> (hsh & 31)) & 1u)) {
        const int64_t lo = a.rated_rowptr[slot], hi = a.rated_rowptr[slot + 1];
        masked = wave_is_masked_at(gi, lo, hi, a.rated_col, nullptr, lane);
        __builtin_amdgcn_s_waitcnt(0x0f70);
    }
    if (masked) sc = CRH_MASKED_SCORE;
    float es = CRH_NEG_INF;
    int ei = CRH_PAD_IDX;
    if constexpr (ONE_TRIP && LANE_READ) {
        es = ks_raw;
        ei = ki_raw;
    } else if constexpr (ONE_TRIP) {
        if (lane < n) {
            es = ks_raw;
            ei = ki_raw;
        }
    } else {
        if (lane < n) {
            es = lsu[lane];
            ei = liu[lane];
        }
    }
    const int p = __popcll(__ballot(lane < n && crh_better(es, ei, sc, gi)));
    if (p < K) {
        if (lane >= p && lane < n && lane + 1 < K) {
            lsu[lane + 1] = es;
            liu[lane + 1] = ei;
        }
        const int n2 = n < K ? n + 1 : K;
        if (lane == 0) {
            lsu[p] = sc;
            liu[p] = gi;
            cnt[ul] = n2;
        }
        if (n2 >= K) {
            const float prev = __builtin_bit_cast(float, __builtin_amdgcn_readlane(__builtin_bit_cast(int, es), K >= 2 ? K - 2 : 0));
            const float kth = (p == K - 1) ? sc : prev;
            const float t = dma_new_tau<MG>(kth, es, sc, a.screen_k < 2 ? 2 : a.screen_k, margin);
            if (mine) tau_reg = t;
        }
    }
}

#ifdef CRH_DMA_EVENT_REBALLOT
constexpr bool DMA_EVENT_REBALLOT = true;
#else
constexpr bool DMA_EVENT_REBALLOT = false;
#endif
#ifdef CRH_DMA_SCREEN_TWO_TRIP
constexpr bool DMA_SCREEN_ONE_TRIP = false;
#else
constexpr bool DMA_SCREEN_ONE_TRIP = true;
#endif
#ifdef CRH_DMA_SCREEN_MFMA32
constexpr bool DMA_SCREEN_M16 = false;
#else
constexpr bool DMA_SCREEN_M16 = true;
#endif
#ifdef CRH_DMA_M16_BODY_OLD
constexpr bool DMA_M16_HOOKED = false;
#else
constexpr bool DMA_M16_HOOKED = true;
#endif
#ifdef CRH_DMA_EVENT_RUNTIME_K
constexpr int DMA_EVENT_KC = 0;
#else
constexpr int DMA_EVENT_KC = SCREEN_KP;
#endif
#ifdef CRH_DMA_EVENT_SLOT_TEST
constexpr bool DMA_EVENT_SLOT_TEST = true;
#else
constexpr bool DMA_EVENT_SLOT_TEST = false;
#endif
#ifdef CRH_DMA_EVENT_TAIL64
constexpr bool DMA_EVENT_TAIL64 = true;
#else
constexpr bool DMA_EVENT_TAIL64 = false;
#endif
#ifdef CRH_DMA_EVENT_MASK8_SPLIT
[[maybe_unused]] constexpr bool DMA_EVENT_MASK8_SPLIT = true;
#else
[[maybe_unused]] constexpr bool DMA_EVENT_MASK8_SPLIT = false;
#endif
#ifdef CRH_DMA_EVENT_NO_FULL
constexpr bool DMA_EVENT_FULL = false;
#else
constexpr bool DMA_EVENT_FULL = DMA_EVENT_KC != 0 && DMA_SCREEN_ONE_TRIP;
#endif
#ifdef CRH_DMA_EVENT_NO_STRAIGHT
constexpr bool DMA_EVENT_STRAIGHT = false;
#else
constexpr bool DMA_EVENT_STRAIGHT = true;
#endif
template <int K>
__device__ __forceinline__ void dma_candidate_full(float sc, int gi, bool bm_masked, int ul, int64_t slot, float* ls, int* li,
                                                   const ScoreArgs& a, int lane, const unsigned* rfilter, bool mine, float& tau_reg,
                                                   float margin) {
    static_assert(K >= 2 && K < 64, "one entry per lane");
    constexpr unsigned long long LIST = (1ull << K) - 1ull;
    float* lsu = ls + ul * K;
    int* liu = li + ul * K;
    const unsigned hsh = rated_hash192(gi);
    const float es = lsu[lane];
    const int ei = liu[lane];
    const unsigned fw_raw = a.rated_rowptr ? rfilter[ul * DMA_FW + (hsh >> 5)] : 0u;
    const float ks = __builtin_bit_cast(float, __builtin_amdgcn_readlane(__builtin_bit_cast(int, es), K - 1));
    const int ki = __builtin_amdgcn_readlane(ei, K - 1);
    if (!crh_better(fmaxf(sc, CRH_MASKED_SCORE), gi, ks, ki)) return;
    bool masked = bm_masked;
    if (!masked && ((__builtin_amdgcn_readfirstlane(fw_raw) >> (hsh & 31)) & 1u)) {
        const int64_t lo = a.rated_rowptr[slot], hi = a.rated_rowptr[slot + 1];
        masked = wave_is_masked_at(gi, lo, hi, a.rated_col, nullptr, lane);
        __builtin_amdgcn_s_waitcnt(0x0f70);
    }
    if (masked) sc = CRH_MASKED_SCORE;
    const int p = __popcll(__ballot(crh_better(es, ei, sc, gi)) & LIST);
    if (p < K) {
        if (lane >= p && lane + 1 < K) {
            lsu[lane + 1] = es;
            liu[lane + 1] = ei;
        }
        if (lane == 0) {
            lsu[p] = sc;
            liu[p] = gi;
        }
        const float prev = __builtin_bit_cast(float, __builtin_amdgcn_readlane(__builtin_bit_cast(int, es), K - 2));
        const float kth = (p == K - 1) ? sc : prev;
        const float t = dma_new_tau<true>(kth, es, sc, a.screen_k < 2 ? 2 : a.screen_k, margin);
        if (mine) tau_reg = t;
    }
}

template <bool ONE_TRIP, bool CM, bool MG = false>
__device__ __forceinline__ void tile_slow_path_dma(const f32x16& acc, float& tau_reg, float* ls, int* li, int* cnt, int K,
                                                   int ucol0, int64_t slot0, const ScoreArgs& a, int64_t item0,
                                                   int64_t split_end, int lane, unsigned tb, const unsigned* rfilter, int idv,
                                                   float margin = 0.0f) {
    unsigned cm = gt_mask16(acc, tau_reg);
    unsigned m16 = 0u;
    if (tb != 0u && __ballot(tau_reg < 0.0f) != 0ull) {
        const unsigned x = tb >> (4 * (lane >> 5));
        m16 = (x & 0xFu) | ((x >> 4) & 0xF0u) | ((x >> 8) & 0xF00u) | ((x >> 12) & 0xF000u);
        if (tau_reg > CRH_NEG_INF) cm &= ~m16;
    }
    const unsigned bm = cm & m16;
    unsigned long long lanes = __ballot(cm != 0u);
    while (lanes) {
        const int L = __builtin_ctzll(lanes);
        lanes &= lanes - 1;
        unsigned cmL = __builtin_amdgcn_readlane(cm, L);
        const unsigned bmL = __builtin_amdgcn_readlane(bm, L);
        const int jl = L & 31, hh = L >> 5;
        const int64_t slot = slot0 + jl;
        if (slot >= a.n_users) continue;
        const int ul = ucol0 + jl;
        while (cmL) {
            const int r = __builtin_ctz(cmL);
            cmL &= cmL - 1;
            const int64_t il = item0 + (r & 3) + 8 * (r >> 2) + 4 * hh;
            if (il >= split_end) continue;
            const float sc = __builtin_bit_cast(float, __builtin_amdgcn_readlane(__builtin_bit_cast(int, pick16u(acc, r)), L));
            int gi;
            if constexpr (CM) gi = __builtin_amdgcn_readlane(idv, (r & 3) + 8 * (r >> 2) + 4 * hh);
            else gi = (int)(a.item_base + il);
            dma_candidate<ONE_TRIP, false, MG>(sc, gi, (bmL >> r) & 1u, ul, slot, ls, li, cnt, K, a, lane, rfilter, (lane & 31) == jl, tau_reg, margin);
        }
    }
}

typedef float f32x8 __attribute__((ext_vector_type(8)));
__device__ __forceinline__ float max8(const f32x8& v) {
#if defined(__HIP_DEVICE_COMPILE__)
    float a0, a1, a2, r;
    asm("v_max3_f32 %0, %1, %2, %3" : "=v"(a0) : "v"(v[0]), "v"(v[1]), "v"(v[2]));
    asm("v_max3_f32 %0, %1, %2, %3" : "=v"(a1) : "v"(v[3]), "v"(v[4]), "v"(v[5]));
    asm("v_max3_f32 %0, %1, %2, %3" : "=v"(a2) : "v"(v[6]), "v"(v[7]), "v"(a0));
    asm("v_max_f32 %0, %1, %2" : "=v"(r) : "v"(a1), "v"(a2));
    return r;
#else
    return fmaxf(fmaxf(fmaxf(v[0], v[1]), fmaxf(v[2], v[3])), fmaxf(fmaxf(v[4], v[5]), fmaxf(v[6], v[7])));
#endif
}
__device__ __forceinline__ float acc_max(const f32x8& v) { return max8(v); }
__device__ __forceinline__ float acc_max(const f32x16& v) { return max16(v); }
__device__ __forceinline__ unsigned gt_mask8(const f32x8& v, float t) {
    unsigned m = 0;
#if defined(__HIP_DEVICE_COMPILE__)
    if constexpr (DMA_EVENT_MASK8_SPLIT) {
#pragma unroll
        for (int r = 7; r >= 0; --r)
            asm("v_cmp_gt_f32 vcc, %1, %2\n\tv_addc_co_u32 %0, vcc, %0, %0, vcc" : "+v"(m) : "v"(v[r]), "v"(t) : "vcc");
    } else {
#define CRH_GT8(R) "v_cmp_gt_f32 vcc, %" #R ", %9\n\tv_addc_co_u32 %0, vcc, %0, %0, vcc\n\t"
        asm(CRH_GT8(8) CRH_GT8(7) CRH_GT8(6) CRH_GT8(5) CRH_GT8(4) CRH_GT8(3) CRH_GT8(2) "v_cmp_gt_f32 vcc, %1, %9\n\tv_addc_co_u32 %0, vcc, %0, %0, vcc"
            : "+v"(m)
            : "v"(v[0]), "v"(v[1]), "v"(v[2]), "v"(v[3]), "v"(v[4]), "v"(v[5]), "v"(v[6]), "v"(v[7]), "v"(t)
            : "vcc");
#undef CRH_GT8
    }
#endif
    return m;
}
__device__ __forceinline__ float pick8u(const f32x8& v, int r) {
    const bool b0 = r & 1, b1 = r & 2, b2 = r & 4;
    const float p0 = b0 ? v[1] : v[0], p1 = b0 ? v[3] : v[2], p2 = b0 ? v[5] : v[4], p3 = b0 ? v[7] : v[6];
    const float q0 = b1 ? p1 : p0, q1 = b1 ? p3 : p2;
    return b2 ? q1 : q0;
}
template <bool CM, int KC, bool FULL = false>
__device__ __forceinline__ void tile_slow_path_dma16(const f32x8& acc, float& tau_reg, float* ls, int* li, int* cnt, int Krt, int ucol0,
                                                     int64_t slot0, const ScoreArgs& a, int64_t item0, int64_t split_end, int rows_left,
                                                     int gi0, int lane, unsigned tb, const unsigned* rfilter, int idv, float margin) {
    static_assert(!FULL || KC != 0, "the full-list form is compiled for K'");
    const int K = KC ? KC : Krt;
    unsigned cm = gt_mask8(acc, tau_reg);
    unsigned m8 = 0u;
    if (tb != 0u && __ballot(tau_reg < 0.0f) != 0ull) {
        const int g4 = 4 * (lane >> 4);
        m8 = ((tb >> g4) & 0xFu) | (((tb >> (16 + g4)) & 0xFu) << 4);
        if (tau_reg > CRH_NEG_INF) cm &= ~m8;
    }
    const unsigned bm = cm & m8;
    unsigned long long lanes = __ballot(cm != 0u);
    auto candidate = [&](int L, int r, unsigned bmL) __attribute__((always_inline)) {
        const int jl = L & 15, g = L >> 4;
        const int64_t slot = slot0 + jl;
        const int ul = ucol0 + jl;
        const int row = 16 * (r >> 2) + 4 * g + (r & 3);
        const int64_t il = item0 + row;
        if constexpr (DMA_EVENT_TAIL64) {
            if (il >= split_end) return;
        } else {
            if (row >= rows_left) return;
        }
        const float sc = __builtin_bit_cast(float, __builtin_amdgcn_readlane(__builtin_bit_cast(int, pick8u(acc, r)), L));
        int gi;
        if constexpr (CM) gi = __builtin_amdgcn_readlane(idv, row);
        else if constexpr (DMA_EVENT_TAIL64) gi = (int)(a.item_base + il);
        else gi = gi0 + row;
        if constexpr (FULL)
            dma_candidate_full<KC>(sc, gi, (bmL >> r) & 1u, ul, slot, ls, li, a, lane, rfilter, (lane & 15) == jl, tau_reg, margin);
        else
            dma_candidate<DMA_SCREEN_ONE_TRIP, true, true>(sc, gi, (bmL >> r) & 1u, ul, slot, ls, li, cnt, K, a, lane, rfilter, (lane & 15) == jl, tau_reg, margin);
    };
    if constexpr (FULL && DMA_EVENT_STRAIGHT && !DMA_EVENT_SLOT_TEST) {
        if (__popcll(lanes) == 1) {
            const int L = __builtin_ctzll(lanes);
            const unsigned cmL = __builtin_amdgcn_readlane(cm, L);
            if ((cmL & (cmL - 1)) == 0u) {
                candidate(L, __builtin_ctz(cmL), __builtin_amdgcn_readlane(bm, L));
                return;
            }
        }
    }
    while (lanes) {
        const int L = __builtin_ctzll(lanes);
        lanes &= lanes - 1;
        unsigned cmL = __builtin_amdgcn_readlane(cm, L);
        const unsigned bmL = __builtin_amdgcn_readlane(bm, L);
        if constexpr (DMA_EVENT_SLOT_TEST) {
            if (slot0 + (L & 15) >= a.n_users) continue;
        }
        while (cmL) {
            const int r = __builtin_ctz(cmL);
            cmL &= cmL - 1;
            candidate(L, r, bmL);
        }
    }
}


template <typename T, int D, int R, bool FL, bool CM = false, bool M16 = false>
__global__ __launch_bounds__(256, 1) void score_topk_dma_kernel(ScoreArgs a) {
    constexpr int NW = DMA_NW, UW = 4, UPW = DMA_UPW;
    static_assert(!M16 || (std::is_same<T, _Float16>::value && D == 128 && !FL), "the 16x16x32 form is the fp16 d=128 screen's");
    constexpr int UB = M16 ? 16 : 32, NU = UPW / UB, NR = M16 ? 8 : 16;
    using AccT = std::conditional_t<M16, f32x8, f32x16>;
    constexpr int PF = FL ? 2 : 3;
    static_assert(R == 4 && (!FL || sizeof(T) == 4) && !(CM && FL), "ring shape");
    constexpr int SIDE_B = CM ? IDS_B : TBITS_B;
    constexpr int ROWB = D * (int)sizeof(T);
    constexpr int NCH = ROWB / 32;
    constexpr int TILE_B = NCH * 1024;
    constexpr int CPW = NCH / NW;
    constexpr int GR = 2, NG = NCH / GR;
    constexpr int BG = NG / 2 - 1;
    constexpr int TG = M16 ? 2 : 1;
    static_assert(NCH % NW == 0 && NG % 4 == 0 && BG + 2 < NG, "row width not supported by the DMA kernel");
    extern __shared__ __attribute__((aligned(16))) char smem[];

    const int lane = threadIdx.x & 63;
    const int wave = __builtin_amdgcn_readfirstlane((int)(threadIdx.x >> 6));
    const int S = a.n_splits;
    const int split = (int)(blockIdx.x % S);
    const int64_t ug_raw = (int64_t)(blockIdx.x / S) * NW + wave;
    const bool live = ug_raw < a.n_ugroups;
    const int64_t ug = live ? ug_raw : a.n_ugroups - 1;
    constexpr int KC = M16 ? DMA_EVENT_KC : 0;
    const int K = KC ? KC : a.k;
    const int i = lane & (M16 ? 15 : 31), h = lane >> (M16 ? 4 : 5);
    constexpr bool MG = std::is_same<T, _Float16>::value && D == 128;

    char* ring = smem;
    unsigned* tbits = reinterpret_cast<unsigned*>(smem + R * TILE_B);
    unsigned* flags = tbits + SIDE_B / 4;
    if constexpr (FL) {
        if (threadIdx.x < 16) flags[threadIdx.x] = threadIdx.x < PF - 1 ? (unsigned)NW : 0u;
    }
    int64_t n_rows = a.n_items;
    if constexpr (CM) n_rows = (int64_t)__builtin_amdgcn_readfirstlane((int)*a.n_live);
    const int64_t NT = (n_rows + 31) >> 5;
    const int64_t t0 = NT * split / S, t1 = NT * (split + 1) / S;
    const int64_t split_end = (t1 << 5) < n_rows ? (t1 << 5) : n_rows;
    const int64_t slot0w = ug * UPW;
    auto cut_ids = [&](int& lo, int& hi) __attribute__((always_inline)) {
        if constexpr (CM) {
            const int id_end = (int)(a.item_base + a.n_items);
            if (S == 1) {
                lo = (int)a.item_base;
                hi = id_end;
            } else {
                lo = (t0 << 5) < n_rows ? a.idmap[t0 << 5] : id_end;
                hi = (t1 << 5) < n_rows ? a.idmap[t1 << 5] : id_end;
            }
        } else {
            lo = (int)(a.item_base + (t0 << 5));
            hi = (int)(a.item_base + split_end);
        }
    };

    char* wl = smem + R * TILE_B + SIDE_B + (FL ? FLAGS_B : 0) + (size_t)wave * dma_wave_lds_bytes(K);
    float* ls = reinterpret_cast<float*>(wl);
    int* li = reinterpret_cast<int*>(ls + UPW * K);
    int* cnt = li + UPW * K;
    for (int j = lane; j < UPW; j += 64) cnt[j] = 0;
    [[maybe_unused]] float margin = __builtin_inff();
    if constexpr (MG) {
        if (a.margin != nullptr) margin = *a.margin;
    }
    constexpr bool FULL_FORM = M16 && KC != 0 && DMA_EVENT_FULL;
    [[maybe_unused]] int lists_full = FULL_FORM && a.seed_score != nullptr ? 1 : 0;
    if (a.seed_score) {
        for (int j = 0; j < UPW; ++j) {
            const int64_t slot = slot0w + j;
            if (slot >= a.n_users) break;
            int n = 0;
            for (int e0 = 0; e0 < K; e0 += 64) {
                const int e = e0 + lane;
                int gi = CRH_PAD_IDX;
                if (e < K) {
                    gi = a.seed_idx[slot * K + e];
                    ls[j * K + e] = a.seed_score[slot * K + e];
                    li[j * K + e] = gi;
                }
                n += __popcll(__ballot(gi != CRH_PAD_IDX));
            }
            if (lane == 0) cnt[j] = n;
            if constexpr (FULL_FORM) lists_full &= n == K ? 1 : 0;
        }
    }
    unsigned* rfilter = reinterpret_cast<unsigned*>(cnt + UPW);
    for (int j = lane; j < UPW * DMA_FW; j += 64) rfilter[j] = 0u;
    if (live && a.rated_rowptr) {
        int id0, id1;
        cut_ids(id0, id1);
        const int64_t s1 = slot0w + UPW < a.n_users ? slot0w + UPW : a.n_users;
        const int64_t e0 = a.rated_rowptr[slot0w], e1 = a.rated_rowptr[s1];
        int64_t nxt = a.rated_rowptr[slot0w + 1];
        int u = 0;
        for (int64_t base = e0; base < e1; base += 64) {
            const int64_t e = base + lane;
            if (e < e1) {
                const int v = a.rated_col[e];
                while (e >= nxt) { ++u; nxt = a.rated_rowptr[slot0w + u + 1]; }
                if (v >= id0 && v < id1) {
                    const unsigned hsh = rated_hash192(v);
                    atomicOr(&rfilter[u * DMA_FW + (hsh >> 5)], 1u << (hsh & 31));
                }
            }
        }
    }

    constexpr int BQ = M16 ? ROWB / 64 : NCH;
    f32x4 b[BQ][NU];
    float tau[NU];
#pragma unroll
    for (int u = 0; u < NU; ++u) {
        int64_t slot = slot0w + UB * u + i;
        tau[u] = slot < a.n_users ? CRH_NEG_INF : __builtin_inff();
        if (a.seed_score && slot < a.n_users) {
            tau[u] = wave_list_tau(ls + (UB * u + i) * K, cnt[UB * u + i], K);
            if constexpr (MG) {
                if (cnt[UB * u + i] >= K && ls[(UB * u + i) * K + K - 1] > CRH_MASKED_SCORE)
                    tau[u] = fmaxf(tau[u], ls[(UB * u + i) * K + (a.screen_k < 2 ? 2 : a.screen_k) - 1] - margin);
            }
        }
        if (slot >= a.n_users) slot = a.n_users - 1;
        const int64_t row = a.users ? (int64_t)a.users[slot] : a.user_base + slot;
        const char* up = reinterpret_cast<const char*>(a.user_emb) + row * ROWB + 16 * h;
#pragma unroll
        for (int q = 0; q < BQ; ++q) {
            b[q][u] = load16(up + (M16 ? 64 : 32) * q);
            if constexpr (Elem<T>::kSwap) chunk_swap(b[q][u]);
        }
    }
    if constexpr (M16 && DMA_M16_HOOKED) {
        if (!live) {
#pragma unroll
            for (int u = 0; u < NU; ++u) tau[u] = __builtin_inff();
        }
    }
#if defined(__HIP_DEVICE_COMPILE__)
#pragma unroll
    for (int q = 0; q < BQ; ++q)
#pragma unroll
        for (int u = 0; u < NU; ++u) {
            if constexpr (sizeof(T) == 4) {
                asm volatile("" : "+a"(b[q][u].x));
                asm volatile("" : "+a"(b[q][u].y));
                asm volatile("" : "+a"(b[q][u].z));
                asm volatile("" : "+a"(b[q][u].w));
            } else {
                asm volatile("" : "+a"(b[q][u]));
            }
        }
#endif

    const char* packed = reinterpret_cast<const char*>(a.packed);
    const int n_steps = (int)(t1 - t0);
    const char* my_pieces = packed + (wave * CPW) * 1024 + lane * 16;
    const int n_tiles32 = (int)NT;
    auto dma_tile = [&](int j, int slot) __attribute__((always_inline)) {
        int t = (int)t0 + j;
        t = t < n_tiles32 ? t : n_tiles32 - 1;
        if (CRH_ABLATE(a.ablate) & 2) t = 0;
        const char* g = my_pieces + (int64_t)t * TILE_B;
        char* l = ring + slot * TILE_B + (wave * CPW) * 1024;
#define CRH_DMA_PIECE(CQ)                                                                                              \
    if constexpr (CQ < CPW)                                                                                            \
        __builtin_amdgcn_global_load_lds((const __attribute__((address_space(1))) void*)g,                             \
                                         (__attribute__((address_space(3))) void*)l, 16, (CQ) * 1024, 0)
        CRH_DMA_PIECE(0); CRH_DMA_PIECE(1); CRH_DMA_PIECE(2); CRH_DMA_PIECE(3);
#undef CRH_DMA_PIECE
        static_assert(CPW <= 4, "pieces beyond the immediate offset range");
    };
    auto dma_tbits = [&](int64_t blk) __attribute__((always_inline)) {
        int t = ((int)blk << 6) + lane;
        t = t < n_tiles32 ? t : n_tiles32 - 1;
        __builtin_amdgcn_global_load_lds((const __attribute__((address_space(1))) void*)(a.tile_bits + (unsigned)t),
                                         (__attribute__((address_space(3))) void*)(tbits + (blk & 1) * 64), 4, 0, 0);
    };
    auto dma_ids = [&](int j) __attribute__((always_inline)) {
        int t = (int)t0 + j;
        t = t < n_tiles32 ? t : n_tiles32 - 1;
        unsigned e = ((unsigned)t << 5) + (unsigned)lane;
        const unsigned e_max = ((unsigned)n_tiles32 << 5) - 1u;
        e = e < e_max ? e : e_max;
        __builtin_amdgcn_global_load_lds((const __attribute__((address_space(1))) void*)(a.idmap + e),
                                         (__attribute__((address_space(3))) void*)(tbits + (j & (IDS_SLOTS - 1)) * 32), 4, 0, 0);
    };
    const bool has_bits = !CM && a.bitmap != nullptr;
    auto dma_wait_all = [&]() __attribute__((always_inline)) {
#if defined(__HIP_DEVICE_COMPILE__)
        asm volatile("s_waitcnt vmcnt(0)" ::: "memory");
#endif
    };
    auto dma_wait_but_newest_tile = [&]() __attribute__((always_inline)) {
#if defined(__HIP_DEVICE_COMPILE__)
        if (CRH_ABLATE(a.ablate) & 16) return;
        asm volatile("s_waitcnt vmcnt(%0)" ::"i"(CPW + 1) : "memory");
#endif
    };

    AccT acc[2][NU];
#pragma unroll
    for (int p = 0; p < 2; ++p)
#pragma unroll
        for (int u = 0; u < NU; ++u)
#pragma unroll
            for (int r = 0; r < NR; ++r) acc[p][u][r] = 0.0f;
    f32x4 c[4][GR];
    const uint32_t ring_lds = (uint32_t)(uintptr_t)(__attribute__((address_space(3))) char*)ring +
                              (M16 ? (lane >> 5) * 1024 + ((lane >> 4) & 1) * 512 + (lane & 15) * 16 : lane * 16);
    auto lds_group = [&](f32x4(&dst)[GR], uint32_t addr, auto Gc) __attribute__((always_inline)) {
#if defined(__HIP_DEVICE_COMPILE__)
        asm volatile("ds_read_b128 %0, %1 offset:%2" : "=v"(dst[0]) : "v"(addr), "i"((decltype(Gc)::value * GR + 0) * 1024));
        asm volatile("ds_read_b128 %0, %1 offset:%2" : "=v"(dst[1]) : "v"(addr), "i"(M16 ? decltype(Gc)::value * GR * 1024 + 256 : (decltype(Gc)::value * GR + 1) * 1024));
#endif
    };
    auto lds_wait = [&](f32x4(&x)[GR], auto Nc) __attribute__((always_inline)) {
#if defined(__HIP_DEVICE_COMPILE__)
        if (CRH_ABLATE(a.ablate) & 8) {
            asm volatile("" : "+v"(x[0]), "+v"(x[1]));
            return;
        }
        asm volatile("s_waitcnt lgkmcnt(%2)" : "+v"(x[0]), "+v"(x[1]) : "i"(decltype(Nc)::value));
#endif
    };
    static_assert(GR == 2, "lds_group / lds_wait are written for two chunks per group");
    const uint32_t flags_lds = (uint32_t)(uintptr_t)(__attribute__((address_space(3))) unsigned*)flags;
    unsigned rflag = 0, dflag = 0;
    auto flag_read = [&](unsigned& dst, int word) __attribute__((always_inline)) {
#if defined(__HIP_DEVICE_COMPILE__)
        asm volatile("ds_read_b32 %0, %1" : "=v"(dst) : "v"(flags_lds + 4u * (unsigned)word));
#endif
    };
    const unsigned bump_val = lane == 0 ? 1u : 0u;
    auto flag_bump = [&](int word) __attribute__((always_inline)) {
#if defined(__HIP_DEVICE_COMPILE__)
        asm volatile("ds_add_u32 %0, %1" ::"v"(flags_lds + 4u * (unsigned)word), "v"(bump_val) : "memory");
#endif
    };
    auto flag_land = [&](unsigned& f) __attribute__((always_inline)) {
#if defined(__HIP_DEVICE_COMPILE__)
        asm volatile("s_waitcnt lgkmcnt(0)" : "+v"(f));
#endif
    };
    auto lds_wait_fl = [&](f32x4(&x)[GR], unsigned& f0, unsigned& f1) __attribute__((always_inline)) {
#if defined(__HIP_DEVICE_COMPILE__)
        asm volatile("s_waitcnt lgkmcnt(%4)" : "+v"(x[0]), "+v"(x[1]), "+v"(f0), "+v"(f1) : "i"(GR));
#endif
    };
    auto flag_spin = [&](unsigned have, int word, unsigned want) __attribute__((always_inline)) {
        unsigned v = __builtin_amdgcn_readfirstlane(have);
        if (__builtin_expect(v >= want, 1) || (CRH_ABLATE(a.ablate) & 4)) return;
        unsigned spins = 0;
        do {
            __builtin_amdgcn_s_sleep(1);
            unsigned t;
#if defined(__HIP_DEVICE_COMPILE__)
            asm volatile("ds_read_b32 %0, %1\n\ts_waitcnt lgkmcnt(0)" : "=v"(t) : "v"(flags_lds + 4u * (unsigned)word) : "memory");
#endif
            v = __builtin_amdgcn_readfirstlane(t);
            if (++spins > (1u << 24)) __builtin_trap();
        } while (v < want);
    };

#ifdef CRH_PROFILE
    unsigned long long ev_ticks = 0, ev_count = 0;
#endif
    auto event16 = [&](const AccT& v, float& tau_u, int u, int64_t ts, int rows_left, int gi0, unsigned tb, int idv) __attribute__((always_inline)) {
        if constexpr (M16) {
            if constexpr (FULL_FORM) {
                if (lists_full) {
                    tile_slow_path_dma16<CM, KC, true>(v, tau_u, ls, li, cnt, K, UB * u, slot0w + UB * u, a, ts << 5, split_end, rows_left, gi0,
                                                       lane, tb, rfilter, idv, margin);
                    return;
                }
            }
            tile_slow_path_dma16<CM, KC>(v, tau_u, ls, li, cnt, K, UB * u, slot0w + UB * u, a, ts << 5, split_end, rows_left, gi0, lane, tb,
                                         rfilter, idv, margin);
        }
    };
    auto body = [&](auto Pc, int j, int s_cur, int s_nxt, int s_fill) __attribute__((always_inline)) {
        constexpr int P = decltype(Pc)::value, Q = 1 - P;
        const uint32_t src = ring_lds + s_cur * TILE_B, srcn = ring_lds + s_nxt * TILE_B;
        float m[NU];
        auto group = [&](auto Gc) __attribute__((always_inline)) {
            constexpr int g = decltype(Gc)::value;
            if constexpr (g + 2 < NG) lds_group(c[(g + 2) & 3], src, std::integral_constant<int, g + 2>{});
            else lds_group(c[(g + 2) & 3], srcn, std::integral_constant<int, g + 2 - NG>{});
            if constexpr (!FL && g == BG) {
                dma_wait_but_newest_tile();
                if (!(CRH_ABLATE(a.ablate) & 4)) __builtin_amdgcn_s_barrier();
            }
            __builtin_amdgcn_sched_barrier(0);
            if constexpr (FL) {
                lds_wait_fl(c[g & 3], rflag, dflag);
            } else {
                lds_wait(c[g & 3], std::integral_constant<int, 2 * GR>{});
            }
            if constexpr (!FL && g == BG) {
                if constexpr (CM) dma_ids(j + 3);
                else dma_tbits((t0 + j + 32) >> 6);
                dma_tile(j + 3, s_fill);
#pragma unroll
                for (int q = 0; q < (M16 ? 16 : 8); ++q) {
                    __builtin_amdgcn_sched_group_barrier(0x008, 1, 0);
                    __builtin_amdgcn_sched_group_barrier(0x004, M16 ? 1 : 2, 0);
                    __builtin_amdgcn_sched_group_barrier(0x002, 1, 0);
                    if constexpr (!M16) __builtin_amdgcn_sched_group_barrier(0x020, 1, 0);
                }
            }
            if constexpr (FL) {
                auto hook = [&](auto Nc) __attribute__((always_inline)) {
                    constexpr int n = decltype(Nc)::value;
                    constexpr bool any = (g == 0 && n <= 3) || (g == NG - 3 && (n == 0 || n == 8 || n == 9)) || (g == NG - 2 && n == 0) ||
                                         (g == NG - 1 && (n == 0 || n == 8));
                    if constexpr (any) __builtin_amdgcn_sched_barrier(0);
                    if constexpr (g == 0 && n == 0) {
                        dma_wait_all();
                        flag_bump((j + PF - 1) & (R - 1));
                    }
                    if constexpr (g == 0 && n == 1) flag_spin(dflag, 8 + s_fill, (unsigned)NW * (unsigned)((j + PF) / R));
                    if constexpr (g == 0 && n == 2) dma_tbits((t0 + j + 32) >> 6);
                    if constexpr (g == 0 && n == 3) dma_tile(j + PF, s_fill);
                    if constexpr (g == NG - 3 && n == 0) flag_read(rflag, s_nxt);
                    if constexpr (g == NG - 3 && n == 8) flag_land(rflag);
                    if constexpr (g == NG - 3 && n == 9) flag_spin(rflag, s_nxt, (unsigned)NW * (unsigned)((j + 1) / R + 1));
                    if constexpr (g == NG - 2 && n == 0) flag_bump(8 + s_cur);
                    if constexpr (g == NG - 1 && n == 0) flag_read(dflag, 8 + ((j + 1 + PF) & (R - 1)));
                    if constexpr (g == NG - 1 && n == 8) flag_land(dflag);
                    if constexpr (any) __builtin_amdgcn_sched_barrier(0);
                };
                if constexpr (g == 0) {
#pragma unroll
                    for (int u = 0; u < UW; ++u)
#pragma unroll
                        for (int r = 0; r < 16; ++r) acc[P][u][r] = 0.0f;
                }
                if constexpr (sizeof(T) == 4) {
                    [&]<int... JJ>(std::integer_sequence<int, JJ...>) __attribute__((always_inline)) {
                        (mma_f32_hooked<UW, JJ * 4 * UW>(acc[P], c[g & 3][JJ], b[g * GR + JJ], hook), ...);
                    }(std::make_integer_sequence<int, GR>{});
                }
            } else if constexpr (M16) {
                if constexpr (g == 0) {
#pragma unroll
                    for (int u = 0; u < NU; ++u)
#pragma unroll
                        for (int r = 0; r < NR; ++r) acc[P][u][r] = 0.0f;
                }
#pragma unroll
                for (int mb = 0; mb < 2; ++mb) {
                    const f16x8 ca = __builtin_bit_cast(f16x8, c[g & 3][mb]);
#pragma unroll
                    for (int u = 0; u < NU; ++u) {
                        AccT& x = acc[P][u];
                        f32x4 t = mb ? f32x4{x[4], x[5], x[6], x[7]} : f32x4{x[0], x[1], x[2], x[3]};
                        t = __builtin_amdgcn_mfma_f32_16x16x32_f16(ca, __builtin_bit_cast(f16x8, b[g][u]), t, 0, 0, 0);
#pragma unroll
                        for (int r = 0; r < 4; ++r) x[4 * mb + r] = t[r];
                    }
                }
            } else {
#pragma unroll
                for (int jj = 0; jj < GR; ++jj) {
                    if constexpr (g == 0) {
                        if (jj == 0) {
#pragma unroll
                            for (int u = 0; u < UW; ++u)
#pragma unroll
                                for (int r = 0; r < 16; ++r) acc[P][u][r] = 0.0f;
                        }
                    }
                    Elem<T>::template mma<UW>(acc[P], c[g & 3][jj], b[g * GR + jj]);
                }
            }
            if constexpr (M16 && g == 0) {
#pragma unroll
                for (int u = 0; u < NU; ++u) m[u] = acc_max(acc[Q][u]);
#pragma unroll
                for (int q = 0; q < 16; ++q) {
                    __builtin_amdgcn_sched_group_barrier(0x008, 1, 0);
                    __builtin_amdgcn_sched_group_barrier(0x002, 2, 0);
                }
            }
            if constexpr (!M16 && g == 1) {
#pragma unroll
                for (int u = 0; u < UW; ++u) m[u] = acc_max(acc[Q][u]);
            }
            unsigned long long hitm = 0ull;
            unsigned long long hitb[NU];
            if constexpr (M16 && g == TG) {
#pragma unroll
                for (int u = 0; u < NU; ++u) {
                    hitb[u] = __ballot(m[u] > tau[u]);
                    hitm |= hitb[u];
                }
#pragma unroll
                for (int q = 0; q < NU; ++q) {
                    __builtin_amdgcn_sched_group_barrier(0x008, 1, 0);
                    __builtin_amdgcn_sched_group_barrier(0x002, 1, 0);
                    __builtin_amdgcn_sched_group_barrier(0x004, 1, 0);
                }
            }
            __builtin_amdgcn_sched_barrier(0);
            if constexpr (g == TG) {
                if constexpr (!M16) {
#pragma unroll
                    for (int u = 0; u < UW; ++u) hitm |= __ballot(m[u] > tau[u]);
                }
                if (hitm != 0ull && live && j > 0 && !(CRH_ABLATE(a.ablate) & 1)) {
#ifdef CRH_PROFILE
                    const unsigned long long ev_t0 = a.wave_clock != nullptr ? __builtin_amdgcn_s_memtime() : 0ull;
#endif
                    const int64_t ts = t0 + j - 1;
                    const unsigned tb = has_bits ? tbits[((ts >> 6) & 1) * 64 + (ts & 63)] : 0u;
                    int idv = 0;
                    if constexpr (CM) idv = (int)tbits[((j - 1) & (IDS_SLOTS - 1)) * 32 + (lane & 31)];
                    const int64_t rl64 = split_end - (ts << 5);
                    const int rows_left = rl64 < 32 ? (int)rl64 : 32;
                    const int gi0 = (int)(a.item_base + (ts << 5));
#pragma unroll
                    for (int u = 0; u < NU; ++u)
                        if ((M16 && !DMA_EVENT_REBALLOT) ? hitb[u] != 0ull : __ballot(m[u] > tau[u]) != 0ull) {
                            if constexpr (M16)
                                event16(acc[Q][u], tau[u], u, ts, rows_left, gi0, tb, idv);
                            else
                                tile_slow_path_dma<sizeof(T) == 4 && DMA_ONE_TRIP_F32, CM, MG>(acc[Q][u], tau[u], ls, li, cnt, K, 32 * u, slot0w + 32 * u, a,
                                                                                                ts << 5, split_end, lane, tb, rfilter, idv, margin);
                        }
                    __builtin_amdgcn_s_waitcnt(0xc07f);
#ifdef CRH_PROFILE
                    if (a.wave_clock != nullptr) {
                        ev_ticks += __builtin_amdgcn_s_memtime() - ev_t0;
                        ev_count += 1;
                    }
#endif
                }
            }
        };
        [&]<int... Gs>(std::integer_sequence<int, Gs...>) __attribute__((always_inline)) {
            (group(std::integral_constant<int, Gs>{}), ...);
        }(std::make_integer_sequence<int, NG>{});
    };

    uint32_t ring_a = ring_lds;
    int next_sync = 0;
    bool sync_due = false;
    auto lds_read1 = [&](f32x4& dst, uint32_t addr, auto Oc) __attribute__((always_inline)) {
#if defined(__HIP_DEVICE_COMPILE__)
        asm volatile("ds_read_b128 %0, %1 offset:%2" : "=v"(dst) : "v"(addr), "i"(decltype(Oc)::value));
#endif
    };
    auto body16 = [&](auto Pc, auto Fc, int j) __attribute__((always_inline)) {
        constexpr int P = decltype(Pc)::value, Q = 1 - P;
        constexpr bool FIRST = decltype(Fc)::value;
        constexpr int LA = P ? 0 : TILE_B;
        static_assert(CPW == 2 || !M16, "two pieces per wave");
        float m[NU], a0[NU], a1[NU], a2[NU];
        unsigned long long hitm = 0ull;
        unsigned long long hitb[NU];
        int tc = 0, tf = 0;
        const unsigned* side = nullptr;
        const char* gt = nullptr;
        auto hook = [&](auto Gc, auto Nc) __attribute__((always_inline)) {
            constexpr int g = decltype(Gc)::value, n = decltype(Nc)::value;
            if constexpr (g == 0 && !FIRST) {
#if defined(__HIP_DEVICE_COMPILE__)
                constexpr int u = n >> 1;
                const AccT& v = acc[Q][u];
                if constexpr ((n & 1) == 0) {
                    asm volatile("v_max3_f32 %0, %1, %2, %3" : "=v"(a0[u]) : "v"(v[0]), "v"(v[1]), "v"(v[2]));
                    asm volatile("v_max3_f32 %0, %1, %2, %3" : "=v"(a1[u]) : "v"(v[3]), "v"(v[4]), "v"(v[5]));
                } else {
                    asm volatile("v_max3_f32 %0, %1, %2, %3" : "=v"(a2[u]) : "v"(v[6]), "v"(v[7]), "v"(a0[u]));
                    asm volatile("v_max_f32 %0, %1, %2" : "=v"(m[u]) : "v"(a1[u]), "v"(a2[u]));
                }
#endif
            }
            if constexpr (g == BG) {
                if constexpr (n == 0) {
                    tc = (int)t0 + j + 3;
                    tc = tc < n_tiles32 ? tc : n_tiles32 - 1;
                    tf = (CRH_ABLATE(a.ablate) & 2) ? 0 : tc;
                }
                if constexpr (n == 1) {
                    if constexpr (CM) {
                        unsigned e = ((unsigned)tc << 5) + (unsigned)lane;
                        const unsigned e_max = ((unsigned)n_tiles32 << 5) - 1u;
                        e = e < e_max ? e : e_max;
                        side = reinterpret_cast<const unsigned*>(a.idmap) + e;
                    } else {
                        int t = ((int)((t0 + j + 32) >> 6) << 6) + lane;
                        t = t < n_tiles32 ? t : n_tiles32 - 1;
                        side = reinterpret_cast<const unsigned*>(a.tile_bits) + (unsigned)t;
                    }
                }
                if constexpr (n == 2) {
                    unsigned* dst = CM ? tbits + ((j + 3) & (IDS_SLOTS - 1)) * 32 : tbits + (((t0 + j + 32) >> 6) & 1) * 64;
                    __builtin_amdgcn_global_load_lds((const __attribute__((address_space(1))) void*)side,
                                                     (__attribute__((address_space(3))) void*)dst, 4, 0, 0);
                }
                if constexpr (n == 3) gt = my_pieces + (int64_t)tf * TILE_B;
                if constexpr (n == 4 || n == 5) {
                    char* l = ring + ((j + 3) & (R - 1)) * TILE_B + (wave * CPW) * 1024;
                    __builtin_amdgcn_global_load_lds((const __attribute__((address_space(1))) void*)gt,
                                                     (__attribute__((address_space(3))) void*)l, 16, (n - 4) * 1024, 0);
                }
                if constexpr (n == 8) lds_read1(c[3][0], ring_a, std::integral_constant<int, P * TILE_B + 3 * 2048>{});
                if constexpr (n == 9) lds_read1(c[3][1], ring_a, std::integral_constant<int, P * TILE_B + 3 * 2048 + 256>{});
                if constexpr (n == 10 && P == 1) ring_a = ring_lds + (unsigned)((j + 1) & 2) * TILE_B;
            }
            if constexpr (g == TG) {
                if constexpr (n < NU && !FIRST) {
                    hitb[n] = __ballot(m[n] > tau[n]);
                    hitm |= hitb[n];
                }
                if constexpr (n == 8) lds_read1(c[0][0], ring_a, std::integral_constant<int, LA>{});
                if constexpr (n == 9) lds_read1(c[0][1], ring_a, std::integral_constant<int, LA + 256>{});
            }
            if constexpr (g == 3) {
                if constexpr (n == 0) lds_read1(c[1][0], ring_a, std::integral_constant<int, LA + 2048>{});
                if constexpr (n == 1) lds_read1(c[1][1], ring_a, std::integral_constant<int, LA + 2048 + 256>{});
                if constexpr (n == 6) lds_read1(c[2][0], ring_a, std::integral_constant<int, LA + 2 * 2048>{});
                if constexpr (n == 7) lds_read1(c[2][1], ring_a, std::integral_constant<int, LA + 2 * 2048 + 256>{});
                if constexpr (n == 8 && P == 1) sync_due = (j + 1 >= next_sync) & (j + 1 < n_steps);
            }
        };
        auto group = [&](auto Gc) __attribute__((always_inline)) {
            constexpr int g = decltype(Gc)::value;
            if constexpr (g == BG) {
                dma_wait_but_newest_tile();
                if (!(CRH_ABLATE(a.ablate) & 4)) __builtin_amdgcn_s_barrier();
            }
            __builtin_amdgcn_sched_barrier(0);
            if constexpr (g == 0) lds_wait(c[g], std::integral_constant<int, 4>{});
            else lds_wait(c[g], std::integral_constant<int, 2>{});
            __builtin_amdgcn_sched_barrier(0);
            [&]<int... N>(std::integer_sequence<int, N...>) __attribute__((always_inline)) {
                (([&]() __attribute__((always_inline)) {
                     constexpr int mb = N >> 3, u = N & 7;
                     AccT& x = acc[P][u];
                     f32x4 t = mb ? f32x4{x[4], x[5], x[6], x[7]} : f32x4{x[0], x[1], x[2], x[3]};
                     if constexpr (g == 0) t = f32x4{0.0f, 0.0f, 0.0f, 0.0f};
                     t = __builtin_amdgcn_mfma_f32_16x16x32_f16(__builtin_bit_cast(f16x8, c[g][mb]), __builtin_bit_cast(f16x8, b[g][u]), t, 0, 0, 0);
#pragma unroll
                     for (int r = 0; r < 4; ++r) x[4 * mb + r] = t[r];
                     __builtin_amdgcn_sched_barrier(0);
                     hook(Gc, std::integral_constant<int, N>{});
                     __builtin_amdgcn_sched_barrier(0);
                 }()),
                 ...);
            }(std::make_integer_sequence<int, 16>{});
            if constexpr (g == TG && !FIRST) {
                if (hitm != 0ull && !(CRH_ABLATE(a.ablate) & 1)) {
#ifdef CRH_PROFILE
                    const unsigned long long ev_t0 = a.wave_clock != nullptr ? __builtin_amdgcn_s_memtime() : 0ull;
#endif
                    const int64_t ts = t0 + j - 1;
                    const unsigned tb = has_bits ? tbits[((ts >> 6) & 1) * 64 + (ts & 63)] : 0u;
                    int idv = 0;
                    if constexpr (CM) idv = (int)tbits[((j - 1) & (IDS_SLOTS - 1)) * 32 + (lane & 31)];
                    const int64_t rl64 = split_end - (ts << 5);
                    const int rows_left = rl64 < 32 ? (int)rl64 : 32;
                    const int gi0 = (int)(a.item_base + (ts << 5));
#pragma unroll
                    for (int u = 0; u < NU; ++u)
                        if (!DMA_EVENT_REBALLOT ? hitb[u] != 0ull : __ballot(m[u] > tau[u]) != 0ull)
                            if constexpr (M16)
                                event16(acc[Q][u], tau[u], u, ts, rows_left, gi0, tb, idv);
                    __builtin_amdgcn_s_waitcnt(0xc07f);
#ifdef CRH_PROFILE
                    if (a.wave_clock != nullptr) {
                        ev_ticks += __builtin_amdgcn_s_memtime() - ev_t0;
                        ev_count += 1;
                    }
#endif
                }
            }
        };
        [&]<int... Gs>(std::integer_sequence<int, Gs...>) __attribute__((always_inline)) {
            (group(std::integral_constant<int, Gs>{}), ...);
        }(std::make_integer_sequence<int, NG>{});
    };

    if (n_steps > 0) {
        if constexpr (CM) {
            dma_ids(0);
            dma_ids(2);
        } else {
            dma_tbits(t0 >> 6);
            dma_tbits((t0 >> 6) + 1);
        }
#pragma unroll
        for (int p = 0; p < PF; ++p) dma_tile(p, p);
        dma_wait_all();
        __builtin_amdgcn_s_barrier();
        lds_group(c[0], ring_lds, std::integral_constant<int, 0>{});
        lds_group(c[1], ring_lds, std::integral_constant<int, 1>{});
        if constexpr (FL) flag_read(dflag, 8 + (PF & (R - 1)));
        int s0 = 0;
        unsigned* sync_cnt = nullptr;
        int win_steps = 0;
        next_sync = n_steps + 4;
        if (a.xcd_sync && wave == 0) {
            const unsigned xcc = __builtin_amdgcn_s_getreg(20 | (0 << 6) | (3 << 11)) & 7u;
            sync_cnt = a.xcd_sync + (int64_t)xcc * a.sync_stride;
            if (lane == 0) __hip_atomic_fetch_add(sync_cnt, 1u, __ATOMIC_RELAXED, __HIP_MEMORY_SCOPE_AGENT);
            win_steps = a.sync_window & ~1;
            if (win_steps < 2) win_steps = 2;
            next_sync = 0;
        }
#ifdef CRH_PROFILE
        unsigned long long t_prev = 0;
#endif
        auto trip_head = [&](int j, bool due) __attribute__((always_inline)) {
#ifdef CRH_PROFILE
            if (a.wave_clock != nullptr && blockIdx.x < 16) {
                const unsigned long long t_now = __builtin_amdgcn_s_memtime();
                if (j >= 64 && lane == 0) {
                    unsigned long long dt = (t_now - t_prev) >> ((sizeof(T) == 4 ? 10 : 8) - (ROWB == 256 ? 1 : 0));
                    if (dt > 63) dt = 63;
                    atomicAdd(&a.wave_clock[((size_t)blockIdx.x * 4 + wave) * 64 + dt], 1ull);
                }
                t_prev = t_now;
            }
#endif
            if (due) {
                const int win = j / win_steps;
                if (xcd_window_sync(sync_cnt, win, lane)) {
                    next_sync += win_steps;
                } else {
                    next_sync = n_steps + 4;
                    const int n_win = (n_steps + win_steps - 1) / win_steps;
                    if (lane == 0)
                        for (int wdw = win; wdw < n_win; ++wdw)
                            __hip_atomic_fetch_add(sync_cnt + 1 + wdw, 1u, __ATOMIC_RELAXED, __HIP_MEMORY_SCOPE_AGENT);
                }
            }
        };
        if constexpr (M16 && DMA_M16_HOOKED) {
            lds_group(c[2], ring_lds, std::integral_constant<int, 2>{});
            trip_head(0, 0 >= next_sync);
            body16(std::integral_constant<int, 0>{}, std::true_type{}, 0);
            for (int j = 1;; j += 2) {
                body16(std::integral_constant<int, 1>{}, std::false_type{}, j);
                if (j + 1 > n_steps) break;
                trip_head(j + 1, sync_due);
                body16(std::integral_constant<int, 0>{}, std::false_type{}, j + 1);
                if (j + 2 > n_steps) break;
            }
        } else {
            for (int j = 0; j <= n_steps; j += 2) {
                trip_head(j, j >= next_sync && j < n_steps);
                const int s1 = (s0 + 1) & (R - 1), s2 = (s0 + 2) & (R - 1);
                body(std::integral_constant<int, 0>{}, j, s0, s1, (s0 + PF) & (R - 1));
                if (j + 1 > n_steps) break;
                body(std::integral_constant<int, 1>{}, j + 1, s1, s2, (s1 + PF) & (R - 1));
                s0 = s2;
            }
        }
        dma_wait_all();
#if defined(__HIP_DEVICE_COMPILE__)
        asm volatile("s_waitcnt lgkmcnt(0)" : "+v"(c[0][0]), "+v"(c[0][1]), "+v"(c[1][0]), "+v"(c[1][1]), "+v"(c[2][0]), "+v"(c[2][1]),
                     "+v"(c[3][0]), "+v"(c[3][1]), "+v"(rflag), "+v"(dflag));
#endif
    }

#ifdef CRH_PROFILE
    if (a.wave_clock != nullptr && blockIdx.x < 16 && lane == 0) {
        a.wave_clock[(size_t)16 * 4 * 64 + ((size_t)blockIdx.x * 4 + wave) * 2] = ev_ticks;
        a.wave_clock[(size_t)16 * 4 * 64 + ((size_t)blockIdx.x * 4 + wave) * 2 + 1] = ev_count;
    }
#endif
    if (live) {
        int id_lo, id_hi;
        cut_ids(id_lo, id_hi);
        for (int j = 0; j < UPW; ++j) {
            const int64_t slot = slot0w + j;
            if (slot >= a.n_users) break;
            const int n = __builtin_amdgcn_readfirstlane(cnt[j]);
            const int64_t o = ((int64_t)split * a.n_users + slot) * K;
            if (a.seed_score && S > 1)
                wave_list_store_range(ls + j * K, li + j * K, n, K, a.out_score + o, a.out_idx + o, lane,
                                      split == 0 ? INT32_MIN : id_lo, id_hi);
            else
                wave_list_store(ls + j * K, li + j * K, n, K, a.out_score + o, a.out_idx + o, lane);
        }
    }
}

template <typename T, int D, int R, bool FL, bool CM = false, bool M16 = false>
int launch_score_dma_t(const ScoreArgs& a, hipStream_t stream) {
    const size_t lds = score_dma_lds_bytes(D * (int)sizeof(T), a.k, R, FL, CM);
    auto kern = score_topk_dma_kernel<T, D, R, FL, CM, M16>;
    CRH_HIP(hipFuncSetAttribute(reinterpret_cast<const void*>(kern), hipFuncAttributeMaxDynamicSharedMemorySize,
                                (int)lds));
    const int64_t blocks = ((a.n_ugroups + DMA_NW - 1) / DMA_NW) * a.n_splits;
    hipLaunchKernelGGL(kern, dim3((unsigned)blocks), dim3(64 * DMA_NW), lds, stream, a);
    CRH_HIP(hipGetLastError());
    return CRH_OK;
}

}

size_t score_dma_lds_bytes(int row_bytes, int k, int ring_slots, bool flags, bool compact) {
    return (size_t)ring_slots * (row_bytes / 32) * 1024 + (compact ? IDS_B : TBITS_B) + (flags ? FLAGS_B : 0) + DMA_NW * dma_wave_lds_bytes(k);
}

int score_dma_ring_slots(int esz, int d, int k, int mode) {
    const bool fl = esz == 4 && d == 128 && mode == 2;
    return score_dma_lds_bytes(d * esz, k, 4, fl) <= 160 * 1024 ? 4 : 0;
}

int launch_score_dma(int esz, int d, int mode, const ScoreArgs& a, hipStream_t stream) {
    if (esz == 2 && d == 128 && DMA_SCREEN_M16 && DMA_EVENT_KC != 0 && a.k != DMA_EVENT_KC) return CRH_ERR_ARG;
    if (esz == 2 && d == 128 && (a.margin == nullptr || a.screen_k < 1 || a.screen_k > a.k)) return CRH_ERR_ARG;
    if (esz == 2 && d == 128 && a.idmap != nullptr) {
        if (score_dma_lds_bytes(d * esz, a.k, 4, false, true) > 160 * 1024) return CRH_ERR_ARG;
        return launch_score_dma_t<_Float16, 128, 4, false, true, DMA_SCREEN_M16>(a, stream);
    }
    if (esz == 2) return d == 128 ? launch_score_dma_t<_Float16, 128, 4, false, false, DMA_SCREEN_M16>(a, stream) : launch_score_dma_t<_Float16, 256, 4, false>(a, stream);
    if (d == 64) return launch_score_dma_t<float, 64, 4, false>(a, stream);
    return mode == 2 ? launch_score_dma_t<float, 128, 4, true>(a, stream) : launch_score_dma_t<float, 128, 4, false>(a, stream);
}

}
```

coldrec_amd/ops.py:

```python
from __future__ import annotations

import ctypes
import weakref
import os
from typing import Optional, Tuple

import numpy as np
import torch

from . import _lib

SUPPORTED_DIMS = (8, 16, 32, 64, 128, 256)
SUPPORTED_DIMS_F16 = (16, 32, 64, 128, 256)


def _need_cuda(*ts):
    for t in ts:
        if t is not None and not t.is_cuda:
            raise RuntimeError("coldrec_amd ops need tensors on the MI355X (cuda device); there is no CPU path")


def pad_dim(table: torch.Tensor) -> torch.Tensor:
    d = table.shape[1]
    dims = SUPPORTED_DIMS_F16 if table.dtype == torch.float16 else SUPPORTED_DIMS
# ... 124 lines not shown
            self.handle = h
        return self.handle

    def build(self, n_users: int, k: int) -> "PreparedItems":
        if torch.cuda.current_stream(self.item_emb.device).cuda_stream != self.stream:
            raise RuntimeError("PreparedItems.build: not the stream the state was made on")
        ws_bytes = int(_lib.lib().crh_score_topk_workspace_bytes(int(n_users), self.item_emb.shape[0], 128, int(k)))
        self.handle_for(n_users, _workspace(ws_bytes, self.item_emb.device), ws_bytes)
        return self

    def close(self) -> None:
        h, self.handle = self.handle, None
        if h is not None:
            _lib.lib().crh_score_screen_items_destroy(h)

    def __del__(self):
        try:
            self.close()
        except Exception:
            pass


def prepare_items(item_emb: torch.Tensor, cand_bitmap: Optional[torch.Tensor] = None, item_base: int = 0) -> PreparedItems:
    return PreparedItems(item_emb, cand_bitmap, item_base)


def screen_item_preps() -> int:
    return int(_lib.lib().crh_score_topk_screen_item_preps())


ROUTE_NAMES = {1: "dense", 2: "fused-wave", 3: "fused-wg", 4: "fused-dma"}


def score_topk_route(n_users: int, n_items: int, d: int, k: int, half: bool = False, has_bitmap: bool = True,
                     n_splits: int = 0, pack: bool = True) -> dict:
    import ctypes
    L = _lib.lib()
    d = d if d % 8 == 0 and (L.crh_score_topk_f16_supports_dim(d) if half else L.crh_score_topk_supports_dim(d)) else \
        next(w for w in (8, 16, 32, 64, 128, 256) if w >= d and (w >= 16 or not half))
    full = L.crh_score_topk_f16_workspace_bytes if half else L.crh_score_topk_workspace_bytes
    ws_bytes = full(n_users, n_items, d, k) if pack else L.crh_score_topk_min_workspace_bytes(n_users, k)
    prefix, splits = ctypes.c_int64(0), ctypes.c_int(0)
    code = L.crh_score_topk_route(2 if half else 4, n_users, n_items, d, k, ws_bytes, 1 if has_bitmap else 0, n_splits,
                                  ctypes.byref(prefix), ctypes.byref(splits))
    _lib.check(code if code < 0 else 0, "crh_score_topk_route")
    screened = bool(L.crh_score_topk_screened(2 if half else 4, n_users, n_items, d, k, ws_bytes, 1 if has_bitmap else 0, n_splits))
    return {"route": ROUTE_NAMES[code & 15], "seeded": bool(code & 16), "dma_form": ("flags" if code & 32 else "barrier") if (code & 15) == 4 else None,
            "prefix_items": int(prefix.value),
            "n_splits": int(splits.value), "kernel": L.crh_score_topk_route_kernel(code).decode(), "code": int(code),
            "screened": screened}


def score_topk_screen_plan(n_users: int, n_items: int, d: int, k: int, has_bitmap: bool = True) -> dict:
    import ctypes
    L = _lib.lib()
    ws_bytes = L.crh_score_topk_workspace_bytes(n_users, n_items, d, k)
    cuts, compact = ctypes.c_int32(0), ctypes.c_int32(0)
    _lib.check(L.crh_score_topk_screen_plan(n_users, n_items, ws_bytes, 1 if has_bitmap else 0, ctypes.byref(cuts),
                                            ctypes.byref(compact)), "crh_score_topk_screen_plan")
    return {"cuts": int(cuts.value), "compact": bool(compact.value)}


def score_topk_screen_ordered(n_users: int, n_items: int, d: int, k: int, has_bitmap: bool = True) -> bool:
    L = _lib.lib()
    ws_bytes = L.crh_score_topk_workspace_bytes(n_users, n_items, d, k)
    return bool(L.crh_score_topk_screen_ordered(n_users, n_items, ws_bytes, 1 if has_bitmap else 0))


def score_topk_screen_map(cand_bitmap: torch.Tensor, item_emb: torch.Tensor, item_base: int = 0, prefix: int = 0,
                          ordered: bool = True):
    import ctypes
    _need_cuda(cand_bitmap, item_emb)
    assert cand_bitmap.dtype == torch.int32 and item_emb.dtype == torch.float32 and item_emb.shape[1] == 128
    item_emb = item_emb.contiguous()
    n_main = item_emb.shape[0] - prefix
    out_map = torch.empty(n_main, dtype=torch.int32, device=item_emb.device)
    out_keys = torch.empty(n_main, dtype=torch.int32, device=item_emb.device)
    count = ctypes.c_int64(0)
    rc = _lib.lib().crh_score_topk_screen_map(_lib.ptr(cand_bitmap), _lib.ptr(item_emb), item_emb.shape[0], item_base, prefix,
                                              1 if ordered else 0, _lib.ptr(out_map), _lib.ptr(out_keys), ctypes.byref(count),
                                              _lib.current_stream())
    _lib.check(rc, "crh_score_topk_screen_map")
    return out_map[:count.value], out_keys[:count.value]


def score_topk_uncertified(device=None) -> int:
    dev = torch.device("cuda", torch.cuda.current_device()) if device is None else torch.device(device)
    key = (dev.type, dev.index, torch.cuda.current_stream(dev).cuda_stream)
    buf = _ws_cache.get(key)
    if buf is None:
        raise RuntimeError("score_topk_uncertified: no scoring workspace on this stream")
    n = _lib.lib().crh_score_topk_uncertified(_lib.ptr(buf), _lib.current_stream())
    _lib.check(n if n < 0 else 0, "crh_score_topk_uncertified")
    return int(n)


def mask_topk(scores: torch.Tensor, k: int, rated_rowptr=None, rated_col=None, cand_bitmap=None,
              item_base: int = 0, write_back: bool = True):
    _need_cuda(scores, rated_rowptr, rated_col, cand_bitmap)
    assert scores.dtype == torch.float32 and scores.dim() == 2 and scores.stride(1) == 1
    n_users, n_items = scores.shape
    dev = scores.device
    out = (torch.empty((n_users, k), dtype=torch.float32, device=dev),
           torch.empty((n_users, k), dtype=torch.int32, device=dev))
    rc = _lib.lib().crh_mask_topk_f32(_lib.ptr(scores), n_users, n_items, scores.stride(0),
                                      _lib.ptr(rated_rowptr), _lib.ptr(rated_col), _lib.ptr(cand_bitmap), k,
                                      item_base, 1 if write_back else 0, _lib.ptr(out[0]), _lib.ptr(out[1]),
                                      _lib.current_stream())
    _lib.check(rc, "crh_mask_topk_f32")
    return out


def merge_topk(scores: torch.Tensor, idx: torch.Tensor, k_out: int):
    _need_cuda(scores, idx)
    assert scores.dtype == torch.float32 and idx.dtype == torch.int32
    scores, idx = scores.contiguous(), idx.contiguous()
    n_lists, n_users, k_in = scores.shape
    dev = scores.device
    out = (torch.empty((n_users, k_out), dtype=torch.float32, device=dev),
           torch.empty((n_users, k_out), dtype=torch.int32, device=dev))
    rc = _lib.lib().crh_merge_topk(_lib.ptr(scores), _lib.ptr(idx), n_lists, n_users, k_in, k_out,
                                   _lib.ptr(out[0]), _lib.ptr(out[1]), _lib.current_stream())
    _lib.check(rc, "crh_merge_topk")
    return out


_warmed = set()


def warm_up(device) -> None:
    device = torch.device(device)
    if device.type != 'cuda' or (device.index, ) in _warmed:
        return
    _warmed.add((device.index, ))
    with torch.cuda.device(device):
        f32 = dict(dtype=torch.float32, device=device)
        u, v = torch.zeros((64, 8), **f32), torch.zeros((96, 8), **f32)
        score_topk(u, None, v, 4)
        score_topk(u, None, v, 4, n_splits=2)
        mask_topk(torch.zeros((4, 64), **f32), 4, write_back=False)
        idx = torch.zeros(4, dtype=torch.int32, device=device)
        g, gv = torch.zeros_like(u), torch.zeros_like(v)
        bpr_fwd_bwd(u, v, v, idx, idx, idx, 0.0, g, gv, gv, plan=build_plans_device(idx, idx, idx, 4)[0])
        adam_dense(u.clone(), g, torch.zeros_like(u), torch.zeros_like(u), 1)
        l2_norm(u)
        rp = torch.arange(0, 65, dtype=torch.int64, device=device).clamp_(max=1)
        spmm_csr(rp, torch.zeros(1, dtype=torch.int32, device=device), torch.ones(1, **f32), u, y=torch.empty_like(u))
        dense = torch.zeros((4, 8), dtype=torch.bool, device=device)
        ids = torch.zeros((4, 3), dtype=torch.int32, device=device).long()
        ok = (ids >= 0) & (ids < 8)
        (dense[torch.arange(4, device=device).unsqueeze(1), ids.clamp(0, 7)] & ok).cpu()
        torch.zeros((3, 2), **f32).sum(dim=1).cpu()
        torch.empty(4, dtype=torch.int32, device=device).copy_(torch.zeros(4, dtype=torch.int32).pin_memory(), non_blocking=True)
        torch.cuda.synchronize(device)


def bpr_fwd_bwd(user_table, pos_table, neg_table, user_idx, pos_idx, neg_idx, reg: float,
                grad_user=None, grad_pos=None, grad_neg=None, loss_out: Optional[torch.Tensor] = None,
                plan: Optional[torch.Tensor] = None, workspace: Optional[torch.Tensor] = None):
    _need_cuda(user_table, pos_table, neg_table, user_idx, pos_idx, neg_idx, grad_user, grad_pos, grad_neg)
    d = user_table.shape[1]
    batch = user_idx.shape[0] if user_idx is not None else user_table.shape[0]
    for t in (user_table, pos_table, neg_table):
        assert t.dtype == torch.float32 and t.is_contiguous() and t.shape[1] == d
    for ix in (user_idx, pos_idx, neg_idx):
        assert ix is None or (ix.dtype == torch.int32 and ix.is_contiguous() and ix.shape[0] == batch)
# ... 1067 lines not shown
```

include/coldrec_hip.h:

```cpp
#ifndef COLDREC_HIP_H
#define COLDREC_HIP_H

#include <stddef.h>
#include <stdint.h>

#ifdef __cplusplus
extern "C" {
#endif

#define CRH_OK 0
#define CRH_ERR_ARG (-1)
#define CRH_ERR_HIP (-2)
#define CRH_ERR_WS (-3)
#define CRH_PAD_IDX 0x7fffffff
#define CRH_MASKED_SCORE (-1.0e9f)
#define CRH_MAX_K 128

const char* crh_last_error(void);
int crh_version(void);
int crh_score_topk_supports_dim(int d);

size_t crh_score_topk_workspace_bytes(int64_t n_users, int64_t n_items, int d, int k);
size_t crh_score_topk_min_workspace_bytes(int64_t n_users, int k);

#define CRH_ROUTE_DENSE 1
#define CRH_ROUTE_FUSED_WAVE 2
#define CRH_ROUTE_FUSED_WG 3
#define CRH_ROUTE_FUSED_DMA 4
#define CRH_ROUTE_SEEDED 16
#define CRH_ROUTE_DMA_FLAGS 32
int crh_score_topk_route(int elem_bytes, int64_t n_users, int64_t n_items, int d, int k, size_t workspace_bytes,
                         int has_bitmap, int n_splits, int64_t* prefix_items, int* picked_splits);
const char* crh_score_topk_route_kernel(int route);
int crh_score_topk_screen_plan(int64_t n_users, int64_t n_items, size_t workspace_bytes, int has_bitmap, int* cuts, int* compact);
int crh_score_topk_screen_ordered(int64_t n_users, int64_t n_items, size_t workspace_bytes, int has_bitmap);
int crh_score_topk_screen_map(const uint32_t* bitmap, const float* item_emb, int64_t n_items, int64_t item_base, int64_t prefix,
                              int ordered, int32_t* map_out, int32_t* keys_out, int64_t* count, void* stream);
int crh_score_topk_screened(int elem_bytes, int64_t n_users, int64_t n_items, int d, int k, size_t workspace_bytes,
                            int has_bitmap, int n_splits);
int64_t crh_score_topk_uncertified(const void* workspace, void* stream);
size_t crh_score_screen_items_bytes(int64_t n_items, int has_bitmap);
int crh_score_screen_items_prepare(const float* item_emb, int64_t n_items, int d, const uint32_t* cand_bitmap, int64_t item_base,
                                   int64_t n_users, void* items_buf, size_t items_bytes, void* workspace, size_t workspace_bytes,
                                   void* stream, void** handle);
int crh_score_screen_items_destroy(void* handle);
int64_t crh_score_topk_screen_item_preps(void);
int crh_score_topk_f32_prepared(const float* user_emb, const int32_t* users, int64_t n_users,
                                const float* item_emb, int64_t n_items, int d,
                                const int64_t* rated_rowptr, const int32_t* rated_col,
                                const uint32_t* cand_bitmap, int k, int64_t item_base,
                                float* out_score, int32_t* out_idx, void* workspace,
                                size_t workspace_bytes, void* stream, int n_splits,
                                void* ev_kernel_start, void* ev_kernel_stop, const void* prepared);
int crh_score_topk_f32(const float* user_emb, const int32_t* users, int64_t n_users,
                       const float* item_emb, int64_t n_items, int d,
                       const int64_t* rated_rowptr, const int32_t* rated_col,
                       const uint32_t* cand_bitmap, int k, int64_t item_base,
                       float* out_score, int32_t* out_idx,
                       void* workspace, size_t workspace_bytes, void* stream);

int crh_score_topk_f32_ex(const float* user_emb, const int32_t* users, int64_t n_users,
                          const float* item_emb, int64_t n_items, int d,
                          const int64_t* rated_rowptr, const int32_t* rated_col,
                          const uint32_t* cand_bitmap, int k, int64_t item_base,
                          float* out_score, int32_t* out_idx,
                          void* workspace, size_t workspace_bytes, void* stream, int n_splits,
                          void* ev_kernel_start, void* ev_kernel_stop);

int crh_score_topk_f16_supports_dim(int d);
size_t crh_score_topk_f16_workspace_bytes(int64_t n_users, int64_t n_items, int d, int k);
int crh_score_topk_f16_ex(const void* user_emb, const int32_t* users, int64_t n_users,
                          const void* item_emb, int64_t n_items, int d,
                          const int64_t* rated_rowptr, const int32_t* rated_col,
                          const uint32_t* cand_bitmap, int k, int64_t item_base,
                          float* out_score, int32_t* out_idx,
                          void* workspace, size_t workspace_bytes, void* stream, int n_splits,
                          void* ev_kernel_start, void* ev_kernel_stop);

int crh_mask_topk_f32(float* scores, int64_t n_users, int64_t n_items, int64_t row_stride,
                      const int64_t* rated_rowptr, const int32_t* rated_col,
                      const uint32_t* cand_bitmap, int k, int64_t item_base, int write_back,
                      float* out_score, int32_t* out_idx, void* stream);

int crh_merge_topk(const float* in_score, const int32_t* in_idx, int n_lists, int64_t n_users,
                   int k_in, int k_out, float* out_score, int32_t* out_idx, void* stream);

size_t crh_bpr_workspace_bytes(int64_t batch);
int64_t crh_bpr_plan_ints(int64_t batch);
int crh_bpr_heavy_threshold(void);
int crh_bpr_plan_build_host(const int32_t* user_idx_host, const int32_t* pos_idx_host,
                            const int32_t* neg_idx_host, int64_t batch, int64_t layout_batch,
                            int32_t* plan_out_host);
int crh_bpr_plan_build(const int32_t* user_idx, const int32_t* pos_idx, const int32_t* neg_idx,
                       int64_t n_records, int64_t batch_size, int32_t* plans_out, void* stream);
size_t crh_bpr_plan_build_large_workspace_bytes(int64_t n_records, int64_t batch_size);
int crh_bpr_plan_build_large(const int32_t* user_idx, const int32_t* pos_idx, const int32_t* neg_idx,
                             int64_t n_records, int64_t batch_size, int32_t* plans_out, void* workspace,
                             size_t workspace_bytes, void* stream);
int crh_bpr_fwd_bwd_f32(const float* user_table, const float* pos_table, const float* neg_table, int d,
                        const int32_t* user_idx, const int32_t* pos_idx, const int32_t* neg_idx,
                        int64_t batch, float reg, float* grad_user, float* grad_pos, float* grad_neg,
                        float* loss_out, const int32_t* plan, void* workspace, size_t workspace_bytes,
                        void* stream);

int crh_bpr_fwd_f32(const float* user_table, const float* pos_table, const float* neg_table, int d,
                    const int32_t* user_idx, const int32_t* pos_idx, const int32_t* neg_idx, int64_t batch,
                    float* sums_out, void* workspace, size_t workspace_bytes, void* stream);
int crh_bpr_bwd_f32(const float* user_table, const float* pos_table, const float* neg_table, int d,
                    const int32_t* user_idx, const int32_t* pos_idx, const int32_t* neg_idx, int64_t batch,
                    int64_t global_batch, float reg, const float* sums, float* grad_user, float* grad_pos,
                    float* grad_neg, float* loss_out, const int32_t* plan, void* workspace,
                    size_t workspace_bytes, void* stream);

int crh_bpr_bwd_owned_f32(const float* user_table, const float* item_table, int d, const int32_t* user_idx,
                          const int32_t* pos_idx, const int32_t* neg_idx, int64_t batch, float reg, const float* sums,
                          float* grad_user, float* grad_item, float* loss_out, const int32_t* plan, int own_mod,
                          int own_rem, void* workspace, size_t workspace_bytes, void* stream);
int64_t crh_rows_pack_cap(int64_t batch, int own_mod);
int crh_rows_pack_f32(const float* table, const int32_t* plan, int64_t batch, int64_t user_rows, int d, int own_mod,
                      int own_rem, int32_t* out_ids, float* out_rows, void* stream);
// ... 215 lines not shown
```

Measured before the change: 6744 billion items/s.

## Precompute per-wave rated-item tile flags to skip rated-list lookups in screened route

Adds a prepass that builds an inverse item map and marks, for each group of 128 users (one wave) and each 32-item compacted tile, whether any user in that wave rated a warm item in the tile. The DMA scoring kernel streams these flags into LDS alongside the id windows and passes them to the event path, so tiles with no rated items can skip the per-user rated-list bounds fetch and binary search. It costs an extra memset, an invmap kernel, a scatter kernel with a binary search per rated edge, more workspace and LDS, and extra DMA scheduling inside the tile loop. Profiling counters for memory trips inside events are also added. The feature is on by default and can be disabled with an environment variable.

```diff
diff --git a/coldrec_amd/_lib.py b/coldrec_amd/_lib.py
--- a/coldrec_amd/_lib.py
+++ b/coldrec_amd/_lib.py
@@ -30,6 +30,9 @@
     "crh_score_topk_screen_plan": (_i32, [_i64, _i64, _sz, _i32, _vp, _vp]),
     "crh_score_topk_screen_ordered": (_i32, [_i64, _i64, _sz, _i32]),
     "crh_score_topk_screen_map": (_i32, [_vp, _vp, _i64, _i64, _i64, _i32, _vp, _vp, _vp, _vp]),
+    "crh_score_topk_screen_rated_tiles": (_i32, [_i64, _i64, _sz, _i32, _i32]),
+    "crh_score_topk_screen_flags_bytes": (_sz, [_i64, _i64]),
+    "crh_score_topk_screen_flags": (_i32, [_vp, _vp, _i64, _i64, _i64, _i32, _vp, _vp, _i64, _vp, _vp]),
     "crh_score_topk_f32": (_i32, [_vp, _vp, _i64, _vp, _i64, _i32, _vp, _vp, _vp, _i32, _i64, _vp, _vp,
                                   _vp, _sz, _vp]),
     "crh_score_topk_f32_ex": (_i32, [_vp, _vp, _i64, _vp, _i64, _i32, _vp, _vp, _vp, _i32, _i64, _vp, _vp,
diff --git a/coldrec_amd/csrc/score_screen.hip b/coldrec_amd/csrc/score_screen.hip
--- a/coldrec_amd/csrc/score_screen.hip
+++ b/coldrec_amd/csrc/score_screen.hip
@@ -179,6 +179,31 @@
 __global__ __launch_bounds__(256) void screen_mapkeys_kernel(const uint16_t* __restrict__ skeys, int64_t n, int32_t* __restrict__ out) {
     const int64_t q = (int64_t)blockIdx.x * 256 + threadIdx.x;
     if (q < n) out[q] = (int32_t)(uint16_t)~skeys[q];
+}
+
+__global__ __launch_bounds__(256) void screen_invmap_kernel(const int32_t* __restrict__ map, const unsigned* __restrict__ n_live, int64_t g0,
+                                                            int32_t* __restrict__ inv) {
+    const int64_t q = (int64_t)blockIdx.x * 256 + threadIdx.x;
+    if (q < (int64_t)*n_live) inv[(int64_t)map[q] - g0] = (int32_t)q;
+}
+
+__global__ __launch_bounds__(256) void screen_rated_tiles_kernel(const int64_t* __restrict__ rowptr, const int32_t* __restrict__ col,
+                                                                 int64_t n_users, const uint32_t* __restrict__ bitmap, int64_t g0, int64_t g1,
+                                                                 const int32_t* __restrict__ inv, uint32_t* __restrict__ flags, int64_t nb) {
+    const int64_t e0 = rowptr[0], e1 = rowptr[n_users];
+    for (int64_t e = e0 + (int64_t)blockIdx.x * 256 + threadIdx.x; e < e1; e += (int64_t)gridDim.x * 256) {
+        const int64_t v = col[e];
+        if (v < g0 || v >= g1) continue;
+        if ((bitmap[v >> 5] >> (v & 31)) & 1u) continue;
+        int64_t lo = 0, hi = n_users;
+        while (hi - lo > 1) {
+            const int64_t mid = lo + ((hi - lo) >> 1);
+            if (rowptr[mid] <= e) lo = mid;
+            else hi = mid;
+        }
+        const int64_t wave = lo >> 7, t = (int64_t)inv[v - g0] >> 5;
+        atomicOr(flags + ((wave >> 2) * nb * 64 + (t >> 3)), 1u << (4 * (int)(t & 7) + (int)(wave & 3)));
+    }
 }
 
 __global__ __launch_bounds__(256) void screen_items_kernel(const float* __restrict__ v, int64_t n_items, const uint32_t* __restrict__ bitmap,
@@ -526,6 +551,26 @@
     return CRH_OK;
 }
 
+int launch_screen_invmap(const int32_t* map, const unsigned* n_live, int64_t g0, int64_t n_main, int32_t* inv, hipStream_t st) {
+    hipLaunchKernelGGL(screen_invmap_kernel, dim3((unsigned)((n_main + 255) / 256)), dim3(256), 0, st, map, n_live, g0, inv);
+    CRH_HIP(hipGetLastError());
+    return CRH_OK;
+}
+
+size_t screen_rated_tiles_bytes(int64_t n_users, int64_t n_main) {
+    const int64_t groups = ((n_users + 127) / 128 + 3) / 4;
+    return (size_t)(groups * screen_rated_blocks(n_main)) * 256;
+}
+
+int launch_screen_rated_tiles(const int64_t* rated_rowptr, const int32_t* rated_col, int64_t n_users, const uint32_t* bitmap, int64_t g0,
+                              int64_t g1, const int32_t* inv, uint32_t* flags, hipStream_t st) {
+    CRH_HIP(hipMemsetAsync(flags, 0, screen_rated_tiles_bytes(n_users, g1 - g0), st));
+    hipLaunchKernelGGL(screen_rated_tiles_kernel, dim3(4096), dim3(256), 0, st, rated_rowptr, rated_col, n_users, bitmap, g0, g1, inv, flags,
+                       screen_rated_blocks(g1 - g0));
+    CRH_HIP(hipGetLastError());
+    return CRH_OK;
+}
+
 int launch_screen_prep_items(const ScreenArgs& s, unsigned* stats, _Float16* packed, int64_t prefix, int32_t* idmap, unsigned* scan,
                              const ScreenOrder* ord, hipStream_t st) {
     const int64_t T = (s.n_items + 31) / 32;
@@ -558,12 +603,14 @@
 }
 
 int screen_map_only(const uint32_t* bitmap, const float* item_emb, int64_t n_items, int64_t item_base, int64_t prefix, int ordered,
-                    int32_t* map_out, int32_t* keys_out, int64_t* count, hipStream_t st) {
+                    int32_t* map_out, int32_t* keys_out, int64_t* count, hipStream_t st, const int64_t* rated_rowptr,
+                    const int32_t* rated_col, int64_t n_users, uint32_t* flags_out) {
     auto al = [](size_t x) { return (x + 255) & ~(size_t)255; };
     const int64_t n_main = n_items - prefix, n_slots = screen_map_slots(n_main);
     const size_t o_scan = 256, o_map = o_scan + al(screen_scan_bytes(n_main)), o_rk = o_map + al((size_t)n_slots * 4),
                  o_k0 = o_rk + al((size_t)n_items * 2), o_k1 = o_k0 + al((size_t)n_slots * 2), o_m1 = o_k1 + al((size_t)n_slots * 2),
-                 o_tmp = o_m1 + al((size_t)n_slots * 4), total = o_tmp + screen_sort_bytes(n_slots);
+                 o_tmp = o_m1 + al((size_t)n_slots * 4), o_inv = o_tmp + al(screen_sort_bytes(n_slots)),
+                 total = o_inv + (flags_out ? al((size_t)n_main * 4) : 0);
     char* buf = nullptr;
     CRH_HIP(hipMalloc(reinterpret_cast<void**>(&buf), total));
     ScreenOrder ord;
@@ -590,6 +637,12 @@
     }
     if (e == hipSuccess && rc == CRH_OK)
         e = hipMemcpyAsync(map_out, ordered ? ord.idmap : idmap, (size_t)n_main * 4, hipMemcpyDeviceToDevice, st);
+    if (e == hipSuccess && rc == CRH_OK && flags_out != nullptr) {
+        int32_t* inv = reinterpret_cast<int32_t*>(buf + o_inv);
+        rc = launch_screen_invmap(ordered ? ord.idmap : idmap, stats + SCREEN_STAT_LIVE, item_base + prefix, n_main, inv, st);
+        if (rc == CRH_OK)
+            rc = launch_screen_rated_tiles(rated_rowptr, rated_col, n_users, bitmap, item_base + prefix, item_base + n_items, inv, flags_out, st);
+    }
     if (e == hipSuccess && rc == CRH_OK) e = hipMemcpyAsync(&live, stats + SCREEN_STAT_LIVE, 4, hipMemcpyDeviceToHost, st);
     if (e == hipSuccess) e = hipStreamSynchronize(st);
     (void)hipFree(buf);
diff --git a/coldrec_amd/csrc/score_topk.hip b/coldrec_amd/csrc/score_topk.hip
--- a/coldrec_amd/csrc/score_topk.hip
+++ b/coldrec_amd/csrc/score_topk.hip
@@ -780,9 +780,10 @@
     return s;
 }
 struct ScreenLayout {
-    size_t stats, ustat, fail, uh, seed, cand, packed, tbits, sync, idmap, scan, rowkeys, skeys, idmap2, sorttmp, scratch, need;
+    size_t stats, ustat, fail, uh, seed, cand, packed, tbits, sync, idmap, scan, rowkeys, skeys, idmap2, sorttmp, inv, rtiles, scratch, need;
 };
-ScreenLayout screen_layout(int64_t n_users, int64_t n_items, int64_t P, bool compact = false, bool ordered = false) {
+ScreenLayout screen_layout(int64_t n_users, int64_t n_items, int64_t P, bool compact = false, bool ordered = false,
+                           bool rated_tiles = false) {
     auto al = [](size_t x) { return (x + 255) & ~(size_t)255; };
     ScreenLayout L;
     L.stats = 0;
@@ -802,7 +803,10 @@
     L.skeys = L.rowkeys + (ordered ? al((size_t)n_items * sizeof(uint16_t)) : 0);
     L.idmap2 = L.skeys + (ordered ? 2 * al(slots * sizeof(uint16_t)) : 0);
     L.sorttmp = L.idmap2 + (ordered ? al(slots * sizeof(int32_t)) : 0);
-    L.scratch = L.sorttmp + (ordered ? al(screen_sort_bytes((int64_t)slots)) : 0);
+    rated_tiles = rated_tiles && compact;
+    L.inv = L.sorttmp + (ordered ? al(screen_sort_bytes((int64_t)slots)) : 0);
+    L.rtiles = L.inv + (rated_tiles ? al(slots * sizeof(int32_t)) : 0);
+    L.scratch = L.rtiles + (rated_tiles ? al(screen_rated_tiles_bytes(n_users, n_items - P)) : 0);
     const int S = screen_splits(n_users, n_items - P, P > 0);
     const size_t lists = S > 1 ? (size_t)S * n_users * SCREEN_KP * 8 : 0;
     const size_t dense = P > 0 ? (size_t)64 * (size_t)P * sizeof(float) : 0;
@@ -826,6 +830,12 @@
     const int64_t P = screen_prefix(n_items);
     if (screen_splits(n_users, n_items - P, P > 0) != 1) return false;
     return workspace_bytes >= screen_layout(n_users, n_items, P, true, true).need;
+}
+bool screen_rated_tiles(int64_t n_users, int64_t n_items, size_t workspace_bytes, bool has_bitmap, bool has_rated) {
+    const char* e = getenv("CRH_SCORE_SCREEN_RATED_TILES");
+    if (!has_rated || (e && atoi(e) == 0) || !screen_compact(n_users, n_items, workspace_bytes, has_bitmap)) return false;
+    const bool ordered = screen_ordered(n_users, n_items, workspace_bytes, has_bitmap);
+    return workspace_bytes >= screen_layout(n_users, n_items, screen_prefix(n_items), true, ordered, true).need;
 }
 bool screen_route(int esz, int64_t n_users, int64_t n_items, int d, int k, size_t workspace_bytes, bool has_bitmap, int n_splits) {
     const int mode = screen_mode();
@@ -967,13 +977,13 @@
     return CRH_OK;
 }
 int dma_timing_begin(ScoreArgs& a, hipStream_t st) {
-    CRH_HIP(hipMalloc(&a.wave_clock, (size_t)16 * 4 * 66 * 8));
-    CRH_HIP(hipMemsetAsync(a.wave_clock, 0, (size_t)16 * 4 * 66 * 8, st));
+    CRH_HIP(hipMalloc(&a.wave_clock, (size_t)16 * 4 * 68 * 8));
+    CRH_HIP(hipMemsetAsync(a.wave_clock, 0, (size_t)16 * 4 * 68 * 8, st));
     return CRH_OK;
 }
 int dma_timing_report(ScoreArgs& a, int esz, int d, hipStream_t st) {
     CRH_HIP(hipStreamSynchronize(st));
-    std::vector<unsigned long long> h((size_t)16 * 4 * 66);
+    std::vector<unsigned long long> h((size_t)16 * 4 * 68);
     CRH_HIP(hipMemcpy(h.data(), a.wave_clock, h.size() * 8, hipMemcpyDeviceToHost));
     CRH_HIP(hipFree(a.wave_clock));
     {
@@ -982,6 +992,7 @@
         fprintf(stderr, "[crh dma timing] events: %.0f per wave, %.0f cycles each (tiles with at least one candidate; 64 waves)\n",
                 (double)ne / 64.0, ne ? (double)tk / (double)ne : 0.0);
     }
+    unsigned long long trip_tk = 0, trip_n = 0, loop_cycles = 0;
     for (int wv = 0; wv < 4; ++wv) {
         unsigned long long tot = 0, wsum = 0;
         std::vector<unsigned long long> b(64, 0);
@@ -993,7 +1004,13 @@
                 tot ? (double)wsum / (double)tot : 0.0, bw);
         for (int q = 0; q < 64; ++q) fprintf(stderr, " %llu", b[q]);
         fprintf(stderr, "\n");
-    }
+        loop_cycles += 2 * wsum;
+    }
+    for (int q = 0; q < 64; ++q) { trip_tk += h[(size_t)16 * 4 * 66 + 2 * q]; trip_n += h[(size_t)16 * 4 * 66 + 2 * q + 1]; }
+    fprintf(stderr, "[crh dma timing] memory trips inside events (filter hit -> list bounds + search): %.0f per wave, %.0f cycles each, "
+                    "%.0f cycles per wave = %.4f of the timed tile loop (64 waves)\n",
+            (double)trip_n / 64.0, trip_n ? (double)trip_tk / (double)trip_n : 0.0, (double)trip_tk / 64.0,
+            loop_cycles ? (double)trip_tk / (double)loop_cycles : 0.0);
     a.wave_clock = nullptr;
     return CRH_OK;
 }
@@ -1043,6 +1060,7 @@
     a.seed_idx = seed_idx;
     a.margin = nullptr;
     a.screen_k = 0;
+    a.rated_tiles = nullptr;
     const int64_t T = (n_items + 31) / 32;
     hipStream_t st = reinterpret_cast<hipStream_t>(stream);
 
@@ -1217,7 +1235,8 @@
     const int64_t P = screen_prefix(n_items);
     const bool compact = screen_compact(n_users, n_items, workspace_bytes, cand_bitmap != nullptr);
     const bool ordered = screen_ordered(n_users, n_items, workspace_bytes, cand_bitmap != nullptr);
-    const ScreenLayout L = screen_layout(n_users, n_items, P, compact, ordered);
+    const bool rated_tiles = screen_rated_tiles(n_users, n_items, workspace_bytes, cand_bitmap != nullptr, rated_rowptr != nullptr);
+    const ScreenLayout L = screen_layout(n_users, n_items, P, compact, ordered, rated_tiles);
     CRH_CHECK_ARG(workspace_bytes >= L.need, "%s: workspace %zu < %zu bytes (screened route)", who, workspace_bytes, L.need);
     int32_t* idmap = compact ? reinterpret_cast<int32_t*>(reinterpret_cast<char*>(workspace) + L.idmap) : nullptr;
     hipStream_t st = reinterpret_cast<hipStream_t>(stream);
@@ -1307,6 +1326,7 @@
     a.n_live = nullptr;
     a.margin = nullptr;
     a.screen_k = 0;
+    a.rated_tiles = nullptr;
     if (P > 0) {
         const int64_t stride = P;
         const int upw_pw = users_per_wave(2, D);
@@ -1368,6 +1388,15 @@
     if (compact) {
         a.idmap = stream_map;
         a.n_live = s.stats + SCREEN_STAT_LIVE;
+        if (rated_tiles) {
+            int32_t* inv = reinterpret_cast<int32_t*>(ws + L.inv);
+            uint32_t* rt = reinterpret_cast<uint32_t*>(ws + L.rtiles);
+            rc = launch_screen_invmap(stream_map, a.n_live, item_base + P, n_main, inv, st);
+            if (rc != CRH_OK) return rc;
+            rc = launch_screen_rated_tiles(rated_rowptr, rated_col, n_users, cand_bitmap, item_base + P, item_base + n_items, inv, rt, st);
+            if (rc != CRH_OK) return rc;
+            a.rated_tiles = rt;
+        }
     } else if (cand_bitmap) {
         a.tile_bits = tbits;
     }
@@ -1469,6 +1498,34 @@
 extern "C" int crh_score_topk_screen_ordered(int64_t n_users, int64_t n_items, size_t workspace_bytes, int has_bitmap) {
     if (n_users <= 0 || n_items <= 0) return 0;
     return screen_ordered(n_users, n_items, workspace_bytes, has_bitmap != 0) ? 1 : 0;
+}
+
+extern "C" int crh_score_topk_screen_rated_tiles(int64_t n_users, int64_t n_items, size_t workspace_bytes, int has_bitmap, int has_rated) {
+    if (n_users <= 0 || n_items <= 0) return 0;
+    return screen_rated_tiles(n_users, n_items, workspace_bytes, has_bitmap != 0, has_rated != 0) ? 1 : 0;
+}
+
+extern "C" size_t crh_score_topk_screen_flags_bytes(int64_t n_users, int64_t n_main) {
+    if (n_users <= 0 || n_main <= 0) return 0;
+    return screen_rated_tiles_bytes(n_users, n_main);
+}
+
+extern "C" int crh_score_topk_screen_flags(const uint32_t* bitmap, const float* item_emb, int64_t n_items, int64_t item_base,
+                                           int64_t prefix, int ordered, const int64_t* rated_rowptr, const int32_t* rated_col,
+                                           int64_t n_users, uint32_t* flags_out, void* stream) {
+    CRH_CHECK_ARG(bitmap && item_emb && rated_rowptr && rated_col && flags_out, "crh_score_topk_screen_flags: NULL argument");
+    CRH_CHECK_ARG(n_users > 0 && prefix >= 0 && (prefix & 31) == 0 && n_items > prefix, "crh_score_topk_screen_flags: prefix %lld of %lld items",
+                  (long long)prefix, (long long)n_items);
+    CRH_CHECK_ARG(((uintptr_t)item_emb & 15) == 0, "crh_score_topk_screen_flags: table must be 16-byte aligned");
+    CRH_CHECK_ARG(item_base >= 0 && item_base + n_items < (int64_t)CRH_PAD_IDX, "crh_score_topk_screen_flags: item ids exceed int32");
+    const int64_t n_main = n_items - prefix;
+    int32_t* tmp = nullptr;
+    CRH_HIP(hipMalloc(reinterpret_cast<void**>(&tmp), (size_t)n_main * 8));
+    int64_t count = 0;
+    const int rc = screen_map_only(bitmap, item_emb, n_items, item_base, prefix, ordered, tmp, tmp + n_main, &count,
+                                   reinterpret_cast<hipStream_t>(stream), rated_rowptr, rated_col, n_users, flags_out);
+    (void)hipFree(tmp);
+    return rc;
 }
 
 extern "C" int crh_score_topk_screen_map(const uint32_t* bitmap, const float* item_emb, int64_t n_items, int64_t item_base,
diff --git a/coldrec_amd/csrc/score_topk_common.h b/coldrec_amd/csrc/score_topk_common.h
--- a/coldrec_amd/csrc/score_topk_common.h
+++ b/coldrec_amd/csrc/score_topk_common.h
@@ -37,7 +37,9 @@
     const unsigned* n_live;
     const float* margin;
     int screen_k;
-};
+    const uint32_t* rated_tiles;
+};
+__host__ __device__ constexpr int64_t screen_rated_blocks(int64_t n_rows) { return (((n_rows + 31) >> 5) + 511) >> 9; }
 
 __device__ __forceinline__ void chunk_swap(f32x4& cf) {
     u32x4 c = __builtin_bit_cast(u32x4, cf);
@@ -366,7 +368,15 @@
 __attribute__((visibility("hidden"))) int launch_screen_prep_users(const ScreenArgs& s, _Float16* uh, int margin_on, hipStream_t st);
 __attribute__((visibility("hidden"))) int screen_map_only(const uint32_t* bitmap, const float* item_emb, int64_t n_items,
                                                           int64_t item_base, int64_t prefix, int ordered, int32_t* map_out,
-                                                          int32_t* keys_out, int64_t* count, hipStream_t st);
+                                                          int32_t* keys_out, int64_t* count, hipStream_t st,
+                                                          const int64_t* rated_rowptr = nullptr, const int32_t* rated_col = nullptr,
+                                                          int64_t n_users = 0, uint32_t* flags_out = nullptr);
+__attribute__((visibility("hidden"))) int launch_screen_invmap(const int32_t* map, const unsigned* n_live, int64_t g0, int64_t n_main,
+                                                               int32_t* inv, hipStream_t st);
+__attribute__((visibility("hidden"))) size_t screen_rated_tiles_bytes(int64_t n_users, int64_t n_main);
+__attribute__((visibility("hidden"))) int launch_screen_rated_tiles(const int64_t* rated_rowptr, const int32_t* rated_col, int64_t n_users,
+                                                                    const uint32_t* bitmap, int64_t g0, int64_t g1, const int32_t* inv,
+                                                                    uint32_t* flags, hipStream_t st);
 __attribute__((visibility("hidden"))) int launch_screen_certify(const ScreenArgs& s, hipStream_t st);
 
 }
diff --git a/coldrec_amd/csrc/score_topk_dma.hip b/coldrec_amd/csrc/score_topk_dma.hip
--- a/coldrec_amd/csrc/score_topk_dma.hip
+++ b/coldrec_amd/csrc/score_topk_dma.hip
@@ -12,6 +12,7 @@
 constexpr int FLAGS_B = 64;
 constexpr int IDS_SLOTS = 8;
 constexpr int IDS_B = (IDS_SLOTS + 1) * 32 * 4;
+constexpr int RT_B = 2 * 256;
 
 constexpr int DMA_FW = 6;
 __host__ __device__ constexpr size_t dma_wave_lds_bytes(int K) {
@@ -52,10 +53,27 @@
     return t;
 }
 
-template <bool ONE_TRIP, bool LANE_READ = false, bool MG = false>
+#ifdef CRH_PROFILE
+struct DmaTripProf { unsigned long long ticks, count; };
+#define CRH_TRIP_PARAM , DmaTripProf& tp
+#define CRH_TRIP_ARG , tp
+#define CRH_TRIP_BEGIN const unsigned long long trip_t0 = a.wave_clock != nullptr ? __builtin_amdgcn_s_memtime() : 0ull
+#define CRH_TRIP_END                                                   \
+    if (a.wave_clock != nullptr) {                                     \
+        tp.ticks += __builtin_amdgcn_s_memtime() - trip_t0;            \
+        tp.count += 1;                                                 \
+    }
+#else
+#define CRH_TRIP_PARAM
+#define CRH_TRIP_ARG
+#define CRH_TRIP_BEGIN
+#define CRH_TRIP_END
+#endif
+
+template <bool ONE_TRIP, bool LANE_READ = false, bool MG = false, bool RT = false>
 __device__ __forceinline__ void dma_candidate(float sc, int gi, bool bm_masked, int ul, int64_t slot, float* ls, int* li, int* cnt, int K,
                                               const ScoreArgs& a, int lane, const unsigned* rfilter, bool mine, float& tau_reg,
-                                              float margin = 0.0f) {
+                                              float margin, bool rt CRH_TRIP_PARAM) {
     float* lsu = ls + ul * K;
     int* liu = li + ul * K;
     const unsigned hsh = rated_hash192(gi);
@@ -63,7 +81,7 @@
     const int le = ONE_TRIP ? (LANE_READ ? lane : (lane < K ? lane : K - 1)) : K - 1;
     const float ks_raw = lsu[le];
     const int ki_raw = liu[le];
-    const unsigned fw_raw = a.rated_rowptr ? rfilter[ul * DMA_FW + (hsh >> 5)] : 0u;
+    const unsigned fw_raw = (RT ? rt : a.rated_rowptr != nullptr) ? rfilter[ul * DMA_FW + (hsh >> 5)] : 0u;
     const int n = __builtin_amdgcn_readfirstlane(n_raw);
     if (n >= K) {
         const float ks = ONE_TRIP ? __builtin_bit_cast(float, __builtin_amdgcn_readlane(__builtin_bit_cast(int, ks_raw), K - 1))
@@ -73,9 +91,11 @@
     }
     bool masked = bm_masked;
     if (!masked && ((__builtin_amdgcn_readfirstlane(fw_raw) >> (hsh & 31)) & 1u)) {
+        CRH_TRIP_BEGIN;
         const int64_t lo = a.rated_rowptr[slot], hi = a.rated_rowptr[slot + 1];
         masked = wave_is_masked_at(gi, lo, hi, a.rated_col, nullptr, lane);
         __builtin_amdgcn_s_waitcnt(0x0f70);
+        CRH_TRIP_END
     }
     if (masked) sc = CRH_MASKED_SCORE;
     float es = CRH_NEG_INF;
@@ -165,10 +185,10 @@
 #else
 constexpr bool DMA_EVENT_STRAIGHT = true;
 #endif
-template <int K>
+template <int K, bool RT>
 __device__ __forceinline__ void dma_candidate_full(float sc, int gi, bool bm_masked, int ul, int64_t slot, float* ls, int* li,
                                                    const ScoreArgs& a, int lane, const unsigned* rfilter, bool mine, float& tau_reg,
-                                                   float margin) {
+                                                   float margin, bool rt CRH_TRIP_PARAM) {
     static_assert(K >= 2 && K < 64, "one entry per lane");
     constexpr unsigned long long LIST = (1ull << K) - 1ull;
     float* lsu = ls + ul * K;
@@ -176,15 +196,17 @@
     const unsigned hsh = rated_hash192(gi);
     const float es = lsu[lane];
     const int ei = liu[lane];
-    const unsigned fw_raw = a.rated_rowptr ? rfilter[ul * DMA_FW + (hsh >> 5)] : 0u;
+    const unsigned fw_raw = (RT ? rt : a.rated_rowptr != nullptr) ? rfilter[ul * DMA_FW + (hsh >> 5)] : 0u;
     const float ks = __builtin_bit_cast(float, __builtin_amdgcn_readlane(__builtin_bit_cast(int, es), K - 1));
     const int ki = __builtin_amdgcn_readlane(ei, K - 1);
     if (!crh_better(fmaxf(sc, CRH_MASKED_SCORE), gi, ks, ki)) return;
     bool masked = bm_masked;
     if (!masked && ((__builtin_amdgcn_readfirstlane(fw_raw) >> (hsh & 31)) & 1u)) {
+        CRH_TRIP_BEGIN;
         const int64_t lo = a.rated_rowptr[slot], hi = a.rated_rowptr[slot + 1];
         masked = wave_is_masked_at(gi, lo, hi, a.rated_col, nullptr, lane);
         __builtin_amdgcn_s_waitcnt(0x0f70);
+        CRH_TRIP_END
     }
     if (masked) sc = CRH_MASKED_SCORE;
     const int p = __popcll(__ballot(crh_better(es, ei, sc, gi)) & LIST);
@@ -208,7 +230,7 @@
 __device__ __forceinline__ void tile_slow_path_dma(const f32x16& acc, float& tau_reg, float* ls, int* li, int* cnt, int K,
                                                    int ucol0, int64_t slot0, const ScoreArgs& a, int64_t item0,
                                                    int64_t split_end, int lane, unsigned tb, const unsigned* rfilter, int idv,
-                                                   float margin = 0.0f) {
+                                                   float margin, bool rt CRH_TRIP_PARAM) {
     unsigned cm = gt_mask16(acc, tau_reg);
     unsigned m16 = 0u;
     if (tb != 0u && __ballot(tau_reg < 0.0f) != 0ull) {
@@ -236,7 +258,7 @@
             int gi;
             if constexpr (CM) gi = __builtin_amdgcn_readlane(idv, (r & 3) + 8 * (r >> 2) + 4 * hh);
             else gi = (int)(a.item_base + il);
-            dma_candidate<ONE_TRIP, false, MG>(sc, gi, (bmL >> r) & 1u, ul, slot, ls, li, cnt, K, a, lane, rfilter, (lane & 31) == jl, tau_reg, margin);
+            dma_candidate<ONE_TRIP, false, MG, CM>(sc, gi, (bmL >> r) & 1u, ul, slot, ls, li, cnt, K, a, lane, rfilter, (lane & 31) == jl, tau_reg, margin, rt CRH_TRIP_ARG);
         }
     }
 }
@@ -283,7 +305,7 @@
 template <bool CM, int KC, bool FULL = false>
 __device__ __forceinline__ void tile_slow_path_dma16(const f32x8& acc, float& tau_reg, float* ls, int* li, int* cnt, int Krt, int ucol0,
                                                      int64_t slot0, const ScoreArgs& a, int64_t item0, int64_t split_end, int rows_left,
-                                                     int gi0, int lane, unsigned tb, const unsigned* rfilter, int idv, float margin) {
+                                                     int gi0, int lane, unsigned tb, const unsigned* rfilter, int idv, float margin, bool rt CRH_TRIP_PARAM) {
     static_assert(!FULL || KC != 0, "the full-list form is compiled for K'");
     const int K = KC ? KC : Krt;
     unsigned cm = gt_mask8(acc, tau_reg);
@@ -312,9 +334,9 @@
         else if constexpr (DMA_EVENT_TAIL64) gi = (int)(a.item_base + il);
         else gi = gi0 + row;
         if constexpr (FULL)
-            dma_candidate_full<KC>(sc, gi, (bmL >> r) & 1u, ul, slot, ls, li, a, lane, rfilter, (lane & 15) == jl, tau_reg, margin);
+            dma_candidate_full<KC, CM>(sc, gi, (bmL >> r) & 1u, ul, slot, ls, li, a, lane, rfilter, (lane & 15) == jl, tau_reg, margin, rt CRH_TRIP_ARG);
         else
-            dma_candidate<DMA_SCREEN_ONE_TRIP, true, true>(sc, gi, (bmL >> r) & 1u, ul, slot, ls, li, cnt, K, a, lane, rfilter, (lane & 15) == jl, tau_reg, margin);
+            dma_candidate<DMA_SCREEN_ONE_TRIP, true, true, CM>(sc, gi, (bmL >> r) & 1u, ul, slot, ls, li, cnt, K, a, lane, rfilter, (lane & 15) == jl, tau_reg, margin, rt CRH_TRIP_ARG);
     };
     if constexpr (FULL && DMA_EVENT_STRAIGHT && !DMA_EVENT_SLOT_TEST) {
         if (__popcll(lanes) == 1) {
@@ -351,7 +373,7 @@
     using AccT = std::conditional_t<M16, f32x8, f32x16>;
     constexpr int PF = FL ? 2 : 3;
     static_assert(R == 4 && (!FL || sizeof(T) == 4) && !(CM && FL), "ring shape");
-    constexpr int SIDE_B = CM ? IDS_B : TBITS_B;
+    constexpr int SIDE_B = CM ? IDS_B + RT_B : TBITS_B;
     constexpr int ROWB = D * (int)sizeof(T);
     constexpr int NCH = ROWB / 32;
     constexpr int TILE_B = NCH * 1024;
@@ -376,6 +398,7 @@
 
     char* ring = smem;
     unsigned* tbits = reinterpret_cast<unsigned*>(smem + R * TILE_B);
+    [[maybe_unused]] unsigned* rtiles = tbits + IDS_B / 4;
     unsigned* flags = tbits + SIDE_B / 4;
     if constexpr (FL) {
         if (threadIdx.x < 16) flags[threadIdx.x] = threadIdx.x < PF - 1 ? (unsigned)NW : 0u;
@@ -532,6 +555,13 @@
         __builtin_amdgcn_global_load_lds((const __attribute__((address_space(1))) void*)(a.idmap + e),
                                          (__attribute__((address_space(3))) void*)(tbits + (j & (IDS_SLOTS - 1)) * 32), 4, 0, 0);
     };
+    [[maybe_unused]] const bool rt_fetch = CM && a.rated_tiles != nullptr && a.rated_rowptr != nullptr;
+    [[maybe_unused]] auto dma_rtiles = [&](int64_t blk) __attribute__((always_inline)) {
+        const int64_t nb = screen_rated_blocks(a.n_items);
+        const int64_t bc = blk < nb ? blk : nb - 1;
+        __builtin_amdgcn_global_load_lds((const __attribute__((address_space(1))) void*)(a.rated_tiles + (((int64_t)(blockIdx.x / S) * nb + bc) << 6) + lane),
+                                         (__attribute__((address_space(3))) void*)(rtiles + (blk & 1) * 64), 4, 0, 0);
+    };
     const bool has_bits = !CM && a.bitmap != nullptr;
     auto dma_wait_all = [&]() __attribute__((always_inline)) {
 #if defined(__HIP_DEVICE_COMPILE__)
@@ -611,18 +641,19 @@
 
 #ifdef CRH_PROFILE
     unsigned long long ev_ticks = 0, ev_count = 0;
-#endif
-    auto event16 = [&](const AccT& v, float& tau_u, int u, int64_t ts, int rows_left, int gi0, unsigned tb, int idv) __attribute__((always_inline)) {
+    DmaTripProf tp = {0ull, 0ull};
+#endif
+    auto event16 = [&](const AccT& v, float& tau_u, int u, int64_t ts, int rows_left, int gi0, unsigned tb, int idv, bool rt) __attribute__((always_inline)) {
         if constexpr (M16) {
             if constexpr (FULL_FORM) {
                 if (lists_full) {
                     tile_slow_path_dma16<CM, KC, true>(v, tau_u, ls, li, cnt, K, UB * u, slot0w + UB * u, a, ts << 5, split_end, rows_left, gi0,
-                                                       lane, tb, rfilter, idv, margin);
+                                                       lane, tb, rfilter, idv, margin, rt CRH_TRIP_ARG);
                     return;
                 }
             }
             tile_slow_path_dma16<CM, KC>(v, tau_u, ls, li, cnt, K, UB * u, slot0w + UB * u, a, ts << 5, split_end, rows_left, gi0, lane, tb,
-                                         rfilter, idv, margin);
+                                         rfilter, idv, margin, rt CRH_TRIP_ARG);
         }
     };
     auto body = [&](auto Pc, int j, int s_cur, int s_nxt, int s_fill) __attribute__((always_inline)) {
@@ -762,6 +793,8 @@
                     const unsigned tb = has_bits ? tbits[((ts >> 6) & 1) * 64 + (ts & 63)] : 0u;
                     int idv = 0;
                     if constexpr (CM) idv = (int)tbits[((j - 1) & (IDS_SLOTS - 1)) * 32 + (lane & 31)];
+                    bool rt = false;
+                    if constexpr (CM) rt = (__builtin_amdgcn_readfirstlane(rtiles[(int)((ts >> 9) & 1) * 64 + (int)((ts >> 3) & 63)]) >> (4 * (int)(ts & 7) + wave)) & 1u;
                     const int64_t rl64 = split_end - (ts << 5);
                     const int rows_left = rl64 < 32 ? (int)rl64 : 32;
                     const int gi0 = (int)(a.item_base + (ts << 5));
@@ -769,10 +802,10 @@
                     for (int u = 0; u < NU; ++u)
                         if ((M16 && !DMA_EVENT_REBALLOT) ? hitb[u] != 0ull : __ballot(m[u] > tau[u]) != 0ull) {
                             if constexpr (M16)
-                                event16(acc[Q][u], tau[u], u, ts, rows_left, gi0, tb, idv);
+                                event16(acc[Q][u], tau[u], u, ts, rows_left, gi0, tb, idv, rt);
                             else
                                 tile_slow_path_dma<sizeof(T) == 4 && DMA_ONE_TRIP_F32, CM, MG>(acc[Q][u], tau[u], ls, li, cnt, K, 32 * u, slot0w + 32 * u, a,
-                                                                                                ts << 5, split_end, lane, tb, rfilter, idv, margin);
+                                                                                                ts << 5, split_end, lane, tb, rfilter, idv, margin, rt CRH_TRIP_ARG);
                         }
                     __builtin_amdgcn_s_waitcnt(0xc07f);
 #ifdef CRH_PROFILE
@@ -906,6 +939,8 @@
                     const unsigned tb = has_bits ? tbits[((ts >> 6) & 1) * 64 + (ts & 63)] : 0u;
                     int idv = 0;
                     if constexpr (CM) idv = (int)tbits[((j - 1) & (IDS_SLOTS - 1)) * 32 + (lane & 31)];
+                    bool rt = false;
+                    if constexpr (CM) rt = (__builtin_amdgcn_readfirstlane(rtiles[(int)((ts >> 9) & 1) * 64 + (int)((ts >> 3) & 63)]) >> (4 * (int)(ts & 7) + wave)) & 1u;
                     const int64_t rl64 = split_end - (ts << 5);
                     const int rows_left = rl64 < 32 ? (int)rl64 : 32;
                     const int gi0 = (int)(a.item_base + (ts << 5));
@@ -913,7 +948,7 @@
                     for (int u = 0; u < NU; ++u)
                         if (!DMA_EVENT_REBALLOT ? hitb[u] != 0ull : __ballot(m[u] > tau[u]) != 0ull)
                             if constexpr (M16)
-                                event16(acc[Q][u], tau[u], u, ts, rows_left, gi0, tb, idv);
+                                event16(acc[Q][u], tau[u], u, ts, rows_left, gi0, tb, idv, rt);
                     __builtin_amdgcn_s_waitcnt(0xc07f);
 #ifdef CRH_PROFILE
                     if (a.wave_clock != nullptr) {
@@ -933,6 +968,12 @@
         if constexpr (CM) {
             dma_ids(0);
             dma_ids(2);
+            if (rt_fetch) {
+                dma_rtiles(t0 >> 9);
+                dma_rtiles((t0 >> 9) + 1);
+            } else {
+                for (int q = lane; q < RT_B / 4; q += 64) rtiles[q] = a.rated_rowptr != nullptr ? ~0u : 0u;
+            }
         } else {
             dma_tbits(t0 >> 6);
             dma_tbits((t0 >> 6) + 1);
@@ -956,6 +997,11 @@
             if (win_steps < 2) win_steps = 2;
             next_sync = 0;
         }
+        [[maybe_unused]] int next_win = next_sync, next_rt = n_steps + 4;
+        if constexpr (CM) {
+            if (rt_fetch && wave == 0) next_rt = (int)(((((t0 >> 9) + 1) << 9) + 64) - t0);
+            next_sync = next_win < next_rt ? next_win : next_rt;
+        }
 #ifdef CRH_PROFILE
         unsigned long long t_prev = 0;
 #endif
@@ -971,16 +1017,28 @@
                 t_prev = t_now;
             }
 #endif
-            if (due) {
+            auto window = [&](int& nxt) __attribute__((always_inline)) {
                 const int win = j / win_steps;
                 if (xcd_window_sync(sync_cnt, win, lane)) {
-                    next_sync += win_steps;
+                    nxt += win_steps;
                 } else {
-                    next_sync = n_steps + 4;
+                    nxt = n_steps + 4;
                     const int n_win = (n_steps + win_steps - 1) / win_steps;
                     if (lane == 0)
                         for (int wdw = win; wdw < n_win; ++wdw)
                             __hip_atomic_fetch_add(sync_cnt + 1 + wdw, 1u, __ATOMIC_RELAXED, __HIP_MEMORY_SCOPE_AGENT);
+                }
+            };
+            if (due) {
+                if constexpr (CM) {
+                    if (j >= next_rt) {
+                        dma_rtiles(((t0 + j) >> 9) + 1);
+                        next_rt += 512;
+                    }
+                    if (j >= next_win) window(next_win);
+                    next_sync = next_win < next_rt ? next_win : next_rt;
+                } else {
+                    window(next_sync);
                 }
             }
         };
@@ -1016,6 +1074,8 @@
     if (a.wave_clock != nullptr && blockIdx.x < 16 && lane == 0) {
         a.wave_clock[(size_t)16 * 4 * 64 + ((size_t)blockIdx.x * 4 + wave) * 2] = ev_ticks;
         a.wave_clock[(size_t)16 * 4 * 64 + ((size_t)blockIdx.x * 4 + wave) * 2 + 1] = ev_count;
+        a.wave_clock[(size_t)16 * 4 * 66 + ((size_t)blockIdx.x * 4 + wave) * 2] = tp.ticks;
+        a.wave_clock[(size_t)16 * 4 * 66 + ((size_t)blockIdx.x * 4 + wave) * 2 + 1] = tp.count;
     }
 #endif
     if (live) {
@@ -1050,7 +1110,7 @@
 }
 
 size_t score_dma_lds_bytes(int row_bytes, int k, int ring_slots, bool flags, bool compact) {
-    return (size_t)ring_slots * (row_bytes / 32) * 1024 + (compact ? IDS_B : TBITS_B) + (flags ? FLAGS_B : 0) + DMA_NW * dma_wave_lds_bytes(k);
+    return (size_t)ring_slots * (row_bytes / 32) * 1024 + (compact ? IDS_B + RT_B : TBITS_B) + (flags ? FLAGS_B : 0) + DMA_NW * dma_wave_lds_bytes(k);
 }
 
 int score_dma_ring_slots(int esz, int d, int k, int mode) {
diff --git a/coldrec_amd/ops.py b/coldrec_amd/ops.py
--- a/coldrec_amd/ops.py
+++ b/coldrec_amd/ops.py
@@ -230,6 +230,30 @@
                                               _lib.current_stream())
     _lib.check(rc, "crh_score_topk_screen_map")
     return out_map[:count.value], out_keys[:count.value]
+
+
+def score_topk_screen_rated_tiles(n_users: int, n_items: int, d: int, k: int, has_bitmap: bool = True, has_rated: bool = True) -> bool:
+    L = _lib.lib()
+    ws_bytes = L.crh_score_topk_workspace_bytes(n_users, n_items, d, k)
+    return bool(L.crh_score_topk_screen_rated_tiles(n_users, n_items, ws_bytes, 1 if has_bitmap else 0, 1 if has_rated else 0))
+
+
+def score_topk_screen_flags(cand_bitmap: torch.Tensor, item_emb: torch.Tensor, rated_rowptr: torch.Tensor, rated_col: torch.Tensor,
+                            item_base: int = 0, prefix: int = 0, ordered: bool = True) -> torch.Tensor:
+    _need_cuda(cand_bitmap, item_emb, rated_rowptr, rated_col)
+    assert cand_bitmap.dtype == torch.int32 and item_emb.dtype == torch.float32 and item_emb.shape[1] == 128
+    assert rated_rowptr.dtype == torch.int64 and rated_col.dtype == torch.int32
+    item_emb = item_emb.contiguous()
+    n_users, n_main = rated_rowptr.shape[0] - 1, item_emb.shape[0] - prefix
+    L = _lib.lib()
+    groups = ((n_users + 127) // 128 + 3) // 4
+    words = int(L.crh_score_topk_screen_flags_bytes(n_users, n_main)) // 4
+    out = torch.empty((groups, words // groups), dtype=torch.int32, device=item_emb.device)
+    rc = L.crh_score_topk_screen_flags(_lib.ptr(cand_bitmap), _lib.ptr(item_emb), item_emb.shape[0], item_base, prefix,
+                                       1 if ordered else 0, _lib.ptr(rated_rowptr), _lib.ptr(rated_col), n_users, _lib.ptr(out),
+                                       _lib.current_stream())
+    _lib.check(rc, "crh_score_topk_screen_flags")
+    return out
 
 
 def score_topk_uncertified(device=None) -> int:
diff --git a/include/coldrec_hip.h b/include/coldrec_hip.h
--- a/include/coldrec_hip.h
+++ b/include/coldrec_hip.h
@@ -36,6 +36,11 @@
 int crh_score_topk_screen_ordered(int64_t n_users, int64_t n_items, size_t workspace_bytes, int has_bitmap);
 int crh_score_topk_screen_map(const uint32_t* bitmap, const float* item_emb, int64_t n_items, int64_t item_base, int64_t prefix,
                               int ordered, int32_t* map_out, int32_t* keys_out, int64_t* count, void* stream);
+int crh_score_topk_screen_rated_tiles(int64_t n_users, int64_t n_items, size_t workspace_bytes, int has_bitmap, int has_rated);
+size_t crh_score_topk_screen_flags_bytes(int64_t n_users, int64_t n_main);
+int crh_score_topk_screen_flags(const uint32_t* bitmap, const float* item_emb, int64_t n_items, int64_t item_base, int64_t prefix,
+                                int ordered, const int64_t* rated_rowptr, const int32_t* rated_col, int64_t n_users,
+                                uint32_t* flags_out, void* stream);
 int crh_score_topk_screened(int elem_bytes, int64_t n_users, int64_t n_items, int d, int k, size_t workspace_bytes,
                             int has_bitmap, int n_splits);
 int64_t crh_score_topk_uncertified(const void* workspace, void* stream);
```

New measurement: 6842 billion items/s, median of 6. 1.01x the previous value.
